# alibaba/VideoMV

Hardware: AMD Instinct MI355X
Metric: denoise-steps/sec, t2v 320x512x24 (latent 24x40x64), CFG 9.0, 50-step DDIM schedule (higher is better)
Workload: dtype fp16; 1 GPU; t2v_infer.yaml UNetSD_T2VBase 1.413B, 24 views, latent 40x64, 77 ctx tokens, 1 sample per GPU (cond+uncond batched); parallelism=replicas x1

## Files before the change

include/vmv.h:

```cpp
#ifndef VMV_H
#define VMV_H
#include <stdint.h>
#include <stddef.h>

#ifdef __cplusplus
extern "C" {
#endif

#define VMV_OK            0
#define VMV_EINVAL       -1
#define VMV_EALIGN       -2
#define VMV_ENULL        -3
#define VMV_ERANGE       -4
#define VMV_ECOMM        -5

#define VMV_ABI_VERSION   12
int vmv_abi_version(void);
#define VMV_ELEM_F16      0
#define VMV_ELEM_BF16     1
int vmv_elem_type(void);
int vmv_has_experiments(void);
int vmv_sizeof(int which);
const char* vmv_error_string(int code);

#define VMV_MAX_SEGS 24
#define VMV_SEG_LINEAR   0
#define VMV_SEG_SPATIAL  1
#define VMV_SEG_TEMPORAL 2

typedef struct {
    const void* src;
    int32_t ld;
    int32_t k;
    int32_t mode;
    int32_t d0, d1;
    int32_t _pad;
} VmvGemmSeg;

#define VMV_EPI_NONE   0
#define VMV_EPI_GEGLU  1
#define VMV_EPI_TATTN  2
#define VMV_ACT_NONE   0
#define VMV_ACT_SILU   1
#define VMV_ACT_GELU   2

typedef struct {
    int32_t M, N;
    int32_t nseg;
    int32_t ktot;
    VmvGemmSeg seg[VMV_MAX_SEGS];
    const void* W;
    const float* bias;
    const float* rowvec;
    int32_t rowvec_div, rowvec_ld;
    const void* residual;
    int32_t ldr;
    int32_t epilogue;
    int32_t act;
    int32_t out_fp32;
    void* out;
    int32_t ldo;
    int32_t OH, OW, IH, IW, stride, ups;
    int32_t F, P;
    int32_t ksplit;
    float* workspace;
    int32_t tile;
    float res_scale;
    const float* rowstat;
    const float* colsum;
    float ln_eps;
    int32_t wgroup_rows;
    int64_t wgroup_stride;
    const float* gn_table;
    int32_t gn_rows_per_stat;
    int32_t gn_silu;
    float epi_scale;
    int32_t phased;
} VmvGemmParams;

#define VMV_TILE_AUTO     0
#define VMV_TILE_128x128  1
#define VMV_TILE_128x160  2
#define VMV_TILE_128x64   3
#define VMV_TILE_64x64    4
#define VMV_TILE_256x128  5
#define VMV_TILE_256x160  6
#define VMV_TILE_G128x128 7
#define VMV_TILE_G128x160 8
#define VMV_TILE_P256x128 9
#define VMV_TILE_P256x160 10
#define VMV_TILE_PP256x128 11
#define VMV_TILE_PP256x160 12
#define VMV_TILE_Q128x128 13
#define VMV_TILE_Q96x160  14
#define VMV_TILE_S256x128 15
#define VMV_TILE_S192x160 16
#define VMV_TILE_S256x160 17
#define VMV_TILE_A128x160 18
#define VMV_TILE_A128x128 19
#define VMV_TILE_X256x320 20
#define VMV_TILE_X256x256 21
#define VMV_TILE_X256x128 22
#define VMV_TILE_RS       23
#define VMV_TILE_RS512    24
#define VMV_TILE_RS256    25
#define VMV_TILE_HALO     26
#define VMV_TILE_TFR      27

#define VMV_TILE_TQA      28
#define VMV_TILE_W256x256 29

#define VMV_TILE_X512x128 30
#define VMV_TILE_Y256x128 31

#define VMV_TILE_TRS      32

int vmv_gemm(const VmvGemmParams* p, void* stream);
int vmv_gemm_tqa_ok(const VmvGemmParams* p);
int vmv_gemm_up4_ok(const VmvGemmParams* p);
int vmv_gemm_ln_inline_ok(const VmvGemmParams* p);
int vmv_gemm_rs_ok(const VmvGemmParams* p);
int vmv_gemm_tfr_ok(const VmvGemmParams* p);
int vmv_gemm_trs_ok(const VmvGemmParams* p);
int vmv_gemm_trs_blocks(const VmvGemmParams* p, int max_blocks, void* stream);
int vmv_gemm_pick_tile(const VmvGemmParams* p);
int vmv_gemm_validate(const VmvGemmParams* p);
int vmv_gemm_served_tile(const VmvGemmParams* p);
int vmv_gemm_tile_map(int bid, int tiles_m, int tiles_n, int gm, int* tile_m, int* tile_n);
int vmv_gemm_group_m(int tiles_m, int tiles_n, int BM, int BN, int conc);

typedef struct {
    int32_t M, C;
    const void* x; int32_t ldx;
    int32_t _pad0;
    const void* w1;
    const float* b1;
    const void* w2;
    const float* b2;
    const void* residual; int32_t ldr;
    float ln_eps;
    void* out; int32_t ldo;
    int32_t _pad1;
} VmvFfParams;
int vmv_ff_fused(const VmvFfParams* p, void* stream);
int vmv_ff_fused_ok(const VmvFfParams* p);

typedef struct {
    const void* x;
    const void* x1;
    int32_t ld, ld1;
    int32_t C0, C1;
    int32_t rows, rows_per_stat;
    int32_t chunk_rows;
    float* partial;
    const float* gamma;
    const float* beta;
    float eps;
    int32_t silu;
    void* y;
    int32_t ldy;
    int32_t fold_ranks;
    int64_t* totals;
    int64_t* totals_clear;
    int32_t clear_count;
    int32_t _pad;
} VmvGroupNormParams;

#define VMV_GN_REC 8
#define VMV_GN_NREP 8
int vmv_groupnorm_stats(const VmvGroupNormParams* p, void* stream);
int vmv_groupnorm_table(const VmvGroupNormParams* p, void* stream);
int vmv_groupnorm_apply(const VmvGroupNormParams* p, void* stream);
#define VMV_GN_FUSED_BYTES 131072
int vmv_groupnorm_fused(const VmvGroupNormParams* p, int32_t cols, void* stream);

typedef struct {
    const void* x; int32_t ldx;
    void* y; int32_t ldy;
    const float* gamma; const float* beta;
    int32_t rows, C;
    float eps;
    int32_t _pad;
    float* stats_out;
} VmvLayerNormParams;
int vmv_layernorm(const VmvLayerNormParams* p, void* stream);

typedef struct {
    const float* s; int32_t lds;
    void* p; int32_t ldp;
    int32_t rows, n;
    float scale;
    int32_t _pad;
} VmvSoftmaxParams;
int vmv_softmax_rows(const VmvSoftmaxParams* p, void* stream);

typedef struct {
    int64_t s_outer, s_inner, s_row;
    int32_t inner; int32_t _pad;
} VmvSeqMap;

typedef struct {
    const void* q; const void* k; const void* v; void* o;
    VmvSeqMap qm, km, vm, om;
    int32_t n_outer;
    int32_t kv_div;
    int32_t heads;
    int32_t Nq, Nk;
    float scale;
    int32_t head_dim;
    int32_t causal;
} VmvAttnParams;
int vmv_attention(const VmvAttnParams* p, void* stream);
#define VMV_ATTN_SHORT    1
#define VMV_ATTN_WAVE     2
#define VMV_ATTN_Q128     3
#define VMV_ATTN_Q256     4
#define VMV_ATTN_CAUSAL   5
#define VMV_ATTN_D32      6
#define VMV_ATTN_D128     7
int vmv_attention_served_kernel(const VmvAttnParams* p);

int vmv_latent_to_rows(const float* x, void* rows, int nb_src, int C, int F, int H, int W, int Cpad, int nrep,
                       void* stream);
int vmv_latent_to_rows_keep(const float* x, void* rows, int nb, int C, int F, int H, int W, int ld, int nrep, void* stream);
int vmv_rows_to_nchw(const void* rows, int rows_fp32, int ld, float* out, int n, int C, int HW, void* stream);

typedef struct {
    const float* eps_rows;
    int32_t ld;
    int32_t C, F, HW;
    float guide_scale;
    float c_recip, c_recipm1;
    float c_sqrt_ac, c_sqrt_1mac;
    float a_prev;
    int32_t v_pred;
    float* xt;
    float* x0_out;
    float clamp;
    float sigma;
    const float* noise;
} VmvDdimParams;
int vmv_cfg_ddim_step(const VmvDdimParams* p, void* stream);

int vmv_posterior_sample(const float* moments_rows, int ld, const float* noise, float* z, int n, int zc, int HW, float scale,
                         void* stream);
int vmv_emb_combine_silu(const float* temb, const float* cam, void* out, int rows, int C, int rows_per_t,
                         int cam_rows, void* stream);
int vmv_sinusoidal(const float* t, void* out_elem, int n, int dim, void* stream);

int vmv_i2v_temporal_adapter(const void* in, int ld_in, void* out, int ld_out, const float* w, int F, int HW, int nrep,
                             float scale, void* stream);
int vmv_adaptive_avgpool_rows(const void* in, int ld, void* out, int ldo, int n, int C, int IH, int IW, int OH, int OW,
                              void* stream);

int vmv_lgm_x0_views(const float* eps_rows, int ld, int branch, const float* xt, int C, int F, int HW, const int32_t* idx4,
                     float c_recip, float c_recipm1, float inv_scale, float* out, void* stream);
int vmv_lgm_pack_input(const float* decoded, const float* rays, float* out, int nviews, int HW, void* stream);
int vmv_lgm_render_to_vae(const float* images, float* out, int nviews, int S_in, int S, void* stream);
int vmv_ddim_x0_step(const float* x0_cond, const float* x0_uncond, float* xt, long n, float guide, float c_recip,
                     float c_recipm1, float a_prev, float clamp, float sigma, const float* noise, void* stream);

int vmv_gaussian_activation(const float* raw, int ld, float* out, int n, float* workspace, void* stream);

typedef struct {
    const float* gaussians;
    int32_t N;
    int32_t size;
    const float* view;
    const float* view_proj;
    float tan_half_fov;
    float bg[3];
    float* depth;
    float* xy;
    float* conic_opacity;
    int32_t* rect;
    uint32_t* tiles_touched;
    uint32_t* offsets;
    void* scan_temp; size_t scan_temp_bytes;
    uint64_t* keys; uint64_t* keys_sorted;
    uint32_t* vals; uint32_t* vals_sorted;
    int32_t num_rendered; int32_t _pad;
    void* sort_temp; size_t sort_temp_bytes;
    uint32_t* ranges;
    float* out_color; float* out_alpha;
} VmvGsParams;
int vmv_gs_workspace_bytes(int n_gaussians, int n_instances, size_t* scan_bytes, size_t* sort_bytes);
int vmv_gs_preprocess(const VmvGsParams* p, void* stream);
int vmv_gs_render(const VmvGsParams* p, void* stream);

typedef struct {
    const float* gaussians;
    int32_t B, N, V, size;
    const float* views;
    const float* view_projs;
    float tan_half_fov;
    float bg[3];
    float* depth;
    float* xy;
    float* conic_opacity;
    int32_t* rect;
    uint32_t* tiles_touched;
    uint32_t* offsets;
    void* scan_temp; size_t scan_temp_bytes;
    uint64_t* keys; uint64_t* keys_sorted;
    uint32_t* vals; uint32_t* vals_sorted;
    int32_t num_rendered; int32_t _pad;
    void* sort_temp; size_t sort_temp_bytes;
    uint32_t* ranges;
    float* out_color;
    float* out_alpha;
} VmvGsBatchParams;
int vmv_gs_batch_key_bits(int n_views, int size);
int vmv_gs_batch_workspace_bytes(int n_view_gaussians, int n_instances, int key_bits, size_t* scan_bytes, size_t* sort_bytes);
int vmv_gs_batch_preprocess(const VmvGsBatchParams* p, void* stream);
int vmv_gs_batch_render(const VmvGsBatchParams* p, void* stream);

typedef struct {
    VmvGsBatchParams pass;
    float* out_depth;
    float* out_median_depth;
} VmvGsDepthParams;
int vmv_gs_batch_render_depth(const VmvGsDepthParams* p, void* stream);

typedef struct {
    VmvGsBatchParams pass;
    float* final_T;
    int32_t* n_contrib;
    const float* dL_dimage;
    float* grad2d;
    float* grad_view;
    float* grad;
} VmvGsBackwardParams;
int vmv_gs_batch_render_state(const VmvGsBackwardParams* p, void* stream);
int vmv_gs_batch_backward(const VmvGsBackwardParams* p, void* stream);
int vmv_gs_image_loss(const float* image, const float* target, long n, float* dL_dimage, float* loss, float* workspace, void* stream);
typedef struct {
    float* params;
    float* m; float* v;
    const float* grad;
    float* gaussians;
    int32_t n; int32_t step;
    float lr[5];
    float beta1, beta2, eps;
} VmvGsAdamParams;
int vmv_gs_adam_step(const VmvGsAdamParams* p, void* stream);

typedef struct {
    const float* image;
    const float* target;
    int32_t planes, height, width;
    float lambda_dssim;
    float* dL_dimage;
    float* loss;
    float* workspace;
    size_t workspace_bytes;
} VmvGsSsimLossParams;
int vmv_gs_ssim_loss_workspace_bytes(int planes, int height, int width, size_t* bytes);
int vmv_gs_ssim_loss(const VmvGsSsimLossParams* p, void* stream);

typedef struct {
    const float* depth;
    const float* colour;
    const float* views;
    int   n_views, size;
    float tan_half_fov;
    int   res;
    float origin[3];
    float voxel, trunc, z_min;
    int   carve;
    float* acc;
    long  plane_stride;
} VmvGsTsdfParams;
int vmv_gs_tsdf_integrate(const VmvGsTsdfParams* p, void* stream);

typedef struct {
    const int64_t* faces;
    int64_t  face_stride;
    int64_t  n_faces;
    int64_t  n_vertices;
    int32_t* label;
    int32_t* face_count;
    int32_t* status;
} VmvGsMeshComponentsParams;
int vmv_gs_mesh_components(const VmvGsMeshComponentsParams* p, void* stream);

typedef struct {
    const float*   verts;
    const float*   vert_colours;
    const int64_t* faces;
    int64_t  face_stride;
    int64_t  n_faces;
    int64_t  n_vertices;
    const float* depth;
    const float* colour;
    const float* views;
    int32_t  n_views, size;
    float    tan_half_fov;
    float    z_min, depth_tol;
    float    cos_min;
    int32_t  patch;
    int32_t  tex_size;
    float*   out;
    int64_t  plane_stride;
    int32_t* status;
} VmvGsMeshBakeParams;
int vmv_gs_mesh_bake(const VmvGsMeshBakeParams* p, void* stream);

typedef struct {
    const void* src;
    void* dst;
    int32_t n0, n1, n2;
    int32_t inner16;
    int64_t ss0, ss1, ss2;
} VmvCopyParams;
int vmv_permute_copy(const VmvCopyParams* p, void* stream);

#define VMV_COMM_ALL_TO_ALL 0
#define VMV_COMM_ALL_GATHER 1
#define VMV_COMM_ID_BYTES   128
typedef struct VmvComm VmvComm;
typedef struct {
    const VmvComm* comm;
    int32_t kind;
    int32_t _pad;
    const void* send;
    void* recv;
    int64_t bytes;
} VmvCommParams;
int      vmv_comm_load(const char* rccl_path);
int      vmv_comm_loaded(void);
int      vmv_comm_unique_id(void* id128);
VmvComm* vmv_comm_create(const void* id128, int world, int rank);
VmvComm* vmv_comm_create_sim(int world, int rank);
void     vmv_comm_destroy(VmvComm* comm);
int      vmv_comm_world(const VmvComm* comm);
int      vmv_comm_rank(const VmvComm* comm);
int      vmv_comm_is_sim(const VmvComm* comm);
int      vmv_comm_run(const VmvCommParams* p, void* stream);

typedef struct VmvPlan VmvPlan;
#define VMV_OP_GEMM        1
#define VMV_OP_GN_STATS    2
#define VMV_OP_GN_APPLY    3
#define VMV_OP_LAYERNORM   4
#define VMV_OP_ATTENTION   5
#define VMV_OP_SOFTMAX     6
#define VMV_OP_COPY        7
#define VMV_OP_GN_FUSED    8
#define VMV_OP_FF          9
#define VMV_OP_GN_TABLE    10
#define VMV_OP_COMM        11
VmvPlan* vmv_plan_create(void);
void     vmv_plan_destroy(VmvPlan* plan);
int      vmv_plan_add(VmvPlan* plan, int op, const void* params, size_t nbytes);
int      vmv_plan_size(const VmvPlan* plan);
int      vmv_plan_run(const VmvPlan* plan, void* stream);
int      vmv_plan_run_range(const VmvPlan* plan, int first, int last, void* stream);
typedef struct VmvGraph VmvGraph;
VmvGraph* vmv_plan_capture(const VmvPlan* plan, void* stream);
int       vmv_graph_launch(const VmvGraph* graph, void* stream);
int       vmv_graph_nodes(const VmvGraph* graph);
void      vmv_graph_destroy(VmvGraph* graph);

#ifdef __cplusplus
}
#endif
#endif
```

videomv_amd/_lib.py:

```python
import ctypes as C
import os

_HERE = os.path.dirname(os.path.abspath(__file__))
_ELEM_NAMES = {"fp16": "f16", "f16": "f16", "float16": "f16", "half": "f16", "bf16": "bf16", "bfloat16": "bf16"}
_elem = _ELEM_NAMES[os.environ.get("VMV_DTYPE", "fp16").lower()]
ELEM_F16, ELEM_BF16 = 0, 1


def set_elem(name: str):
    global _elem
    new = _ELEM_NAMES[str(name).lower()]
    if _lib is not None and new != _elem:
        raise RuntimeError(f"the {_elem} kernels are already loaded; set VMV_DTYPE / call set_elem() before first use")
    _elem = new


def elem_name() -> str:
    return "fp16" if _elem == "f16" else "bf16"


def elem():
    import torch
    return torch.float16 if _elem == "f16" else torch.bfloat16


def lib_path() -> str:
    return os.path.join(os.environ.get("VMV_LIB_DIR") or os.path.join(_HERE, "lib"), f"libvmv_hip_{_elem}.so")

VMV_MAX_SEGS = 24
SEG_LINEAR, SEG_SPATIAL, SEG_TEMPORAL = 0, 1, 2
EPI_NONE, EPI_GEGLU, EPI_TATTN = 0, 1, 2
ACT_NONE, ACT_SILU, ACT_GELU = 0, 1, 2
TILE_AUTO, TILE_128x128, TILE_128x160, TILE_128x64, TILE_64x64, TILE_256x128, TILE_256x160 = 0, 1, 2, 3, 4, 5, 6
TILE_G128x128, TILE_G128x160, TILE_P256x128, TILE_P256x160, TILE_PP256x128, TILE_PP256x160 = 7, 8, 9, 10, 11, 12
TILE_Q128x128, TILE_Q96x160 = 13, 14
TILE_S256x128, TILE_S192x160, TILE_S256x160 = 15, 16, 17
TILE_A128x160, TILE_A128x128 = 18, 19
TILE_X256x320, TILE_X256x256, TILE_X256x128 = 20, 21, 22
TILE_RS, TILE_RS512, TILE_RS256, TILE_HALO, TILE_TFR, TILE_TQA, TILE_W256x256, TILE_X512x128, TILE_Y256x128 = 23, 24, 25, 26, 27, 28, 29, 30, 31
TRS_TILE = 32
OP_GEMM, OP_GN_STATS, OP_GN_APPLY, OP_LAYERNORM, OP_ATTENTION, OP_SOFTMAX, OP_COPY, OP_GN_FUSED, OP_FF, OP_GN_TABLE, OP_COMM = 1, 2, 3, 4, 5, 6, 7, 8, 9, 10, 11
COMM_ALL_TO_ALL, COMM_ALL_GATHER, COMM_ID_BYTES = 0, 1, 128
ABI_VERSION = 12
ATTN_SHORT, ATTN_WAVE, ATTN_Q128, ATTN_Q256, ATTN_CAUSAL, ATTN_D32, ATTN_D128 = 1, 2, 3, 4, 5, 6, 7
GN_FUSED_BYTES = 131072


class GemmSeg(C.Structure):
    _fields_ = [("src", C.c_void_p), ("ld", C.c_int32), ("k", C.c_int32), ("mode", C.c_int32),
                ("d0", C.c_int32), ("d1", C.c_int32), ("_pad", C.c_int32)]


class GemmParams(C.Structure):
    _fields_ = [("M", C.c_int32), ("N", C.c_int32), ("nseg", C.c_int32), ("ktot", C.c_int32),
                ("seg", GemmSeg * VMV_MAX_SEGS),
                ("W", C.c_void_p), ("bias", C.c_void_p), ("rowvec", C.c_void_p),
                ("rowvec_div", C.c_int32), ("rowvec_ld", C.c_int32),
                ("residual", C.c_void_p), ("ldr", C.c_int32),
                ("epilogue", C.c_int32), ("act", C.c_int32), ("out_fp32", C.c_int32),
                ("out", C.c_void_p), ("ldo", C.c_int32),
                ("OH", C.c_int32), ("OW", C.c_int32), ("IH", C.c_int32), ("IW", C.c_int32),
                ("stride", C.c_int32), ("ups", C.c_int32),
                ("F", C.c_int32), ("P", C.c_int32),
                ("ksplit", C.c_int32), ("workspace", C.c_void_p),
                ("tile", C.c_int32), ("res_scale", C.c_float), ("rowstat", C.c_void_p), ("colsum", C.c_void_p),
                ("ln_eps", C.c_float), ("wgroup_rows", C.c_int32), ("wgroup_stride", C.c_int64),
                ("gn_table", C.c_void_p), ("gn_rows_per_stat", C.c_int32), ("gn_silu", C.c_int32), ("epi_scale", C.c_float),
                ("phased", C.c_int32)]


class GroupNormParams(C.Structure):
    _fields_ = [("x", C.c_void_p), ("x1", C.c_void_p), ("ld", C.c_int32), ("ld1", C.c_int32),
                ("C0", C.c_int32), ("C1", C.c_int32), ("rows", C.c_int32), ("rows_per_stat", C.c_int32),
                ("chunk_rows", C.c_int32), ("partial", C.c_void_p), ("gamma", C.c_void_p), ("beta", C.c_void_p),
                ("eps", C.c_float), ("silu", C.c_int32), ("y", C.c_void_p), ("ldy", C.c_int32), ("fold_ranks", C.c_int32),
                ("totals", C.c_void_p), ("totals_clear", C.c_void_p), ("clear_count", C.c_int32), ("_pad", C.c_int32)]


class FfParams(C.Structure):
    _fields_ = [("M", C.c_int32), ("C", C.c_int32), ("x", C.c_void_p), ("ldx", C.c_int32), ("_pad0", C.c_int32),
                ("w1", C.c_void_p), ("b1", C.c_void_p), ("w2", C.c_void_p), ("b2", C.c_void_p),
                ("residual", C.c_void_p), ("ldr", C.c_int32), ("ln_eps", C.c_float),
                ("out", C.c_void_p), ("ldo", C.c_int32), ("_pad1", C.c_int32)]


class GsParams(C.Structure):
    _fields_ = [("gaussians", C.c_void_p), ("N", C.c_int32), ("size", C.c_int32), ("view", C.c_void_p),
                ("view_proj", C.c_void_p), ("tan_half_fov", C.c_float), ("bg", C.c_float * 3),
                ("depth", C.c_void_p), ("xy", C.c_void_p), ("conic_opacity", C.c_void_p), ("rect", C.c_void_p),
                ("tiles_touched", C.c_void_p), ("offsets", C.c_void_p), ("scan_temp", C.c_void_p),
                ("scan_temp_bytes", C.c_size_t), ("keys", C.c_void_p), ("keys_sorted", C.c_void_p), ("vals", C.c_void_p),
                ("vals_sorted", C.c_void_p), ("num_rendered", C.c_int32), ("_pad", C.c_int32), ("sort_temp", C.c_void_p),
                ("sort_temp_bytes", C.c_size_t), ("ranges", C.c_void_p), ("out_color", C.c_void_p), ("out_alpha", C.c_void_p)]


class GsBatchParams(C.Structure):
    _fields_ = [("gaussians", C.c_void_p), ("B", C.c_int32), ("N", C.c_int32), ("V", C.c_int32), ("size", C.c_int32),
                ("views", C.c_void_p), ("view_projs", C.c_void_p), ("tan_half_fov", C.c_float), ("bg", C.c_float * 3),
                ("depth", C.c_void_p), ("xy", C.c_void_p), ("conic_opacity", C.c_void_p), ("rect", C.c_void_p),
                ("tiles_touched", C.c_void_p), ("offsets", C.c_void_p), ("scan_temp", C.c_void_p),
                ("scan_temp_bytes", C.c_size_t), ("keys", C.c_void_p), ("keys_sorted", C.c_void_p), ("vals", C.c_void_p),
                ("vals_sorted", C.c_void_p), ("num_rendered", C.c_int32), ("_pad", C.c_int32), ("sort_temp", C.c_void_p),
                ("sort_temp_bytes", C.c_size_t), ("ranges", C.c_void_p), ("out_color", C.c_void_p), ("out_alpha", C.c_void_p)]


class GsBackwardParams(C.Structure):
    _fields_ = [("pass_", GsBatchParams), ("final_T", C.c_void_p), ("n_contrib", C.c_void_p), ("dL_dimage", C.c_void_p),
                ("grad2d", C.c_void_p), ("grad_view", C.c_void_p), ("grad", C.c_void_p)]


class GsDepthParams(C.Structure):
    _fields_ = [("pass_", GsBatchParams), ("out_depth", C.c_void_p), ("out_median_depth", C.c_void_p)]


class GsAdamParams(C.Structure):
    _fields_ = [("params", C.c_void_p), ("m", C.c_void_p), ("v", C.c_void_p), ("grad", C.c_void_p), ("gaussians", C.c_void_p),
                ("n", C.c_int32), ("step", C.c_int32), ("lr", C.c_float * 5), ("beta1", C.c_float), ("beta2", C.c_float),
                ("eps", C.c_float)]


class GsSsimLossParams(C.Structure):
    _fields_ = [("image", C.c_void_p), ("target", C.c_void_p), ("planes", C.c_int32), ("height", C.c_int32), ("width", C.c_int32),
                ("lambda_dssim", C.c_float), ("dL_dimage", C.c_void_p), ("loss", C.c_void_p), ("workspace", C.c_void_p),
                ("workspace_bytes", C.c_size_t)]


class GsTsdfParams(C.Structure):
    _fields_ = [("depth", C.c_void_p), ("colour", C.c_void_p), ("views", C.c_void_p), ("n_views", C.c_int), ("size", C.c_int),
                ("tan_half_fov", C.c_float), ("res", C.c_int), ("origin", C.c_float * 3), ("voxel", C.c_float), ("trunc", C.c_float),
                ("z_min", C.c_float), ("carve", C.c_int), ("acc", C.c_void_p), ("plane_stride", C.c_long)]


class GsMeshComponentsParams(C.Structure):
    _fields_ = [("faces", C.c_void_p), ("face_stride", C.c_int64), ("n_faces", C.c_int64), ("n_vertices", C.c_int64),
                ("label", C.c_void_p), ("face_count", C.c_void_p), ("status", C.c_void_p)]


class GsMeshBakeParams(C.Structure):
    _fields_ = [("verts", C.c_void_p), ("vert_colours", C.c_void_p), ("faces", C.c_void_p), ("face_stride", C.c_int64),
                ("n_faces", C.c_int64), ("n_vertices", C.c_int64), ("depth", C.c_void_p), ("colour", C.c_void_p), ("views", C.c_void_p),
                ("n_views", C.c_int32), ("size", C.c_int32), ("tan_half_fov", C.c_float), ("z_min", C.c_float), ("depth_tol", C.c_float),
                ("cos_min", C.c_float), ("patch", C.c_int32), ("tex_size", C.c_int32), ("out", C.c_void_p), ("plane_stride", C.c_int64),
                ("status", C.c_void_p)]


MESH_STATUS_RANGE, MESH_STATUS_GAVE_UP = 1, 2


class CopyParams(C.Structure):
    _fields_ = [("src", C.c_void_p), ("dst", C.c_void_p), ("n0", C.c_int32), ("n1", C.c_int32), ("n2", C.c_int32),
                ("inner16", C.c_int32), ("ss0", C.c_int64), ("ss1", C.c_int64), ("ss2", C.c_int64)]


class CommParams(C.Structure):
    _fields_ = [("comm", C.c_void_p), ("kind", C.c_int32), ("_pad", C.c_int32), ("send", C.c_void_p), ("recv", C.c_void_p),
                ("bytes", C.c_int64)]


class LayerNormParams(C.Structure):
    _fields_ = [("x", C.c_void_p), ("ldx", C.c_int32), ("y", C.c_void_p), ("ldy", C.c_int32),
                ("gamma", C.c_void_p), ("beta", C.c_void_p), ("rows", C.c_int32), ("C", C.c_int32),
                ("eps", C.c_float), ("_pad", C.c_int32), ("stats_out", C.c_void_p)]


class SeqMap(C.Structure):
    _fields_ = [("s_outer", C.c_int64), ("s_inner", C.c_int64), ("s_row", C.c_int64),
                ("inner", C.c_int32), ("_pad", C.c_int32)]


class AttnParams(C.Structure):
    _fields_ = [("q", C.c_void_p), ("k", C.c_void_p), ("v", C.c_void_p), ("o", C.c_void_p),
                ("qm", SeqMap), ("km", SeqMap), ("vm", SeqMap), ("om", SeqMap),
                ("n_outer", C.c_int32), ("kv_div", C.c_int32), ("heads", C.c_int32),
                ("Nq", C.c_int32), ("Nk", C.c_int32), ("scale", C.c_float), ("head_dim", C.c_int32), ("causal", C.c_int32)]


class SoftmaxParams(C.Structure):
    _fields_ = [("s", C.c_void_p), ("lds", C.c_int32), ("p", C.c_void_p), ("ldp", C.c_int32),
                ("rows", C.c_int32), ("n", C.c_int32), ("scale", C.c_float), ("_pad", C.c_int32)]


class DdimParams(C.Structure):
    _fields_ = [("eps_rows", C.c_void_p), ("ld", C.c_int32), ("C", C.c_int32), ("F", C.c_int32), ("HW", C.c_int32),
                ("guide_scale", C.c_float), ("c_recip", C.c_float), ("c_recipm1", C.c_float),
                ("c_sqrt_ac", C.c_float), ("c_sqrt_1mac", C.c_float), ("a_prev", C.c_float),
                ("v_pred", C.c_int32), ("xt", C.c_void_p), ("x0_out", C.c_void_p),
                ("clamp", C.c_float), ("sigma", C.c_float), ("noise", C.c_void_p)]


_P = C.c_void_p
SYMBOLS = {
    "vmv_abi_version": (C.c_int, []),
    "vmv_elem_type": (C.c_int, []),
    "vmv_sizeof": (C.c_int, [C.c_int]),
    "vmv_error_string": (C.c_char_p, [C.c_int]),
    "vmv_gemm": (C.c_int, [C.POINTER(GemmParams), _P]),
    "vmv_gemm_ln_inline_ok": (C.c_int, [C.POINTER(GemmParams)]),
    "vmv_gemm_rs_ok": (C.c_int, [C.POINTER(GemmParams)]),
    "vmv_gemm_tfr_ok": (C.c_int, [C.POINTER(GemmParams)]),
    "vmv_gemm_tqa_ok": (C.c_int, [C.POINTER(GemmParams)]),
    "vmv_gemm_trs_ok": (C.c_int, [C.POINTER(GemmParams)]),
    "vmv_gemm_trs_blocks": (C.c_int, [C.POINTER(GemmParams), C.c_int, _P]),
    "vmv_gemm_up4_ok": (C.c_int, [C.POINTER(GemmParams)]),
    "vmv_has_experiments": (C.c_int, []),
    "vmv_ff_fused": (C.c_int, [C.POINTER(FfParams), _P]),
    "vmv_ff_fused_ok": (C.c_int, [C.POINTER(FfParams)]),
    "vmv_gemm_pick_tile": (C.c_int, [C.POINTER(GemmParams)]),
    "vmv_gemm_validate": (C.c_int, [C.POINTER(GemmParams)]),
    "vmv_gemm_served_tile": (C.c_int, [C.POINTER(GemmParams)]),
    "vmv_gemm_tile_map": (C.c_int, [C.c_int, C.c_int, C.c_int, C.c_int, C.POINTER(C.c_int), C.POINTER(C.c_int)]),
    "vmv_gemm_group_m": (C.c_int, [C.c_int, C.c_int, C.c_int, C.c_int, C.c_int]),
    "vmv_groupnorm_stats": (C.c_int, [C.POINTER(GroupNormParams), _P]),
    "vmv_groupnorm_apply": (C.c_int, [C.POINTER(GroupNormParams), _P]),
    "vmv_groupnorm_table": (C.c_int, [C.POINTER(GroupNormParams), _P]),
    "vmv_groupnorm_fused": (C.c_int, [C.POINTER(GroupNormParams), C.c_int32, _P]),
    "vmv_layernorm": (C.c_int, [C.POINTER(LayerNormParams), _P]),
    "vmv_attention": (C.c_int, [C.POINTER(AttnParams), _P]),
    "vmv_attention_served_kernel": (C.c_int, [C.POINTER(AttnParams)]),
    "vmv_softmax_rows": (C.c_int, [C.POINTER(SoftmaxParams), _P]),
    "vmv_permute_copy": (C.c_int, [C.POINTER(CopyParams), _P]),
    "vmv_gaussian_activation": (C.c_int, [_P, C.c_int, _P, C.c_int, _P, _P]),
    "vmv_lgm_x0_views": (C.c_int, [_P, C.c_int, C.c_int, _P, C.c_int, C.c_int, C.c_int, _P, C.c_float, C.c_float, C.c_float, _P, _P]),
    "vmv_lgm_pack_input": (C.c_int, [_P, _P, _P, C.c_int, C.c_int, _P]),
    "vmv_lgm_render_to_vae": (C.c_int, [_P, _P, C.c_int, C.c_int, C.c_int, _P]),
    "vmv_ddim_x0_step": (C.c_int, [_P, _P, _P, C.c_long, C.c_float, C.c_float, C.c_float, C.c_float, C.c_float, C.c_float, _P, _P]),
    "vmv_gs_workspace_bytes": (C.c_int, [C.c_int, C.c_int, C.POINTER(C.c_size_t), C.POINTER(C.c_size_t)]),
    "vmv_gs_preprocess": (C.c_int, [C.POINTER(GsParams), _P]),
    "vmv_gs_render": (C.c_int, [C.POINTER(GsParams), _P]),
    "vmv_gs_batch_key_bits": (C.c_int, [C.c_int, C.c_int]),
    "vmv_gs_batch_workspace_bytes": (C.c_int, [C.c_int, C.c_int, C.c_int, C.POINTER(C.c_size_t), C.POINTER(C.c_size_t)]),
    "vmv_gs_batch_preprocess": (C.c_int, [C.POINTER(GsBatchParams), _P]),
    "vmv_gs_batch_render": (C.c_int, [C.POINTER(GsBatchParams), _P]),
    "vmv_gs_batch_render_depth": (C.c_int, [C.POINTER(GsDepthParams), _P]),
    "vmv_gs_batch_render_state": (C.c_int, [C.POINTER(GsBackwardParams), _P]),
    "vmv_gs_batch_backward": (C.c_int, [C.POINTER(GsBackwardParams), _P]),
    "vmv_gs_image_loss": (C.c_int, [_P, _P, C.c_long, _P, _P, _P, _P]),
    "vmv_gs_adam_step": (C.c_int, [C.POINTER(GsAdamParams), _P]),
    "vmv_gs_ssim_loss_workspace_bytes": (C.c_int, [C.c_int, C.c_int, C.c_int, C.POINTER(C.c_size_t)]),
    "vmv_gs_ssim_loss": (C.c_int, [C.POINTER(GsSsimLossParams), _P]),
    "vmv_gs_tsdf_integrate": (C.c_int, [C.POINTER(GsTsdfParams), _P]),
    "vmv_gs_mesh_components": (C.c_int, [C.POINTER(GsMeshComponentsParams), _P]),
    "vmv_gs_mesh_bake": (C.c_int, [C.POINTER(GsMeshBakeParams), _P]),
    "vmv_latent_to_rows": (C.c_int, [_P, _P, C.c_int, C.c_int, C.c_int, C.c_int, C.c_int, C.c_int, C.c_int, _P]),
    "vmv_latent_to_rows_keep": (C.c_int, [_P, _P, C.c_int, C.c_int, C.c_int, C.c_int, C.c_int, C.c_int, C.c_int, _P]),
    "vmv_i2v_temporal_adapter": (C.c_int, [_P, C.c_int, _P, C.c_int, _P, C.c_int, C.c_int, C.c_int, C.c_float, _P]),
    "vmv_adaptive_avgpool_rows": (C.c_int, [_P, C.c_int, _P, C.c_int, C.c_int, C.c_int, C.c_int, C.c_int, C.c_int, C.c_int, _P]),
    "vmv_rows_to_nchw": (C.c_int, [_P, C.c_int, C.c_int, _P, C.c_int, C.c_int, C.c_int, _P]),
    "vmv_cfg_ddim_step": (C.c_int, [C.POINTER(DdimParams), _P]),
    "vmv_posterior_sample": (C.c_int, [_P, C.c_int, _P, _P, C.c_int, C.c_int, C.c_int, C.c_float, _P]),
    "vmv_emb_combine_silu": (C.c_int, [_P, _P, _P, C.c_int, C.c_int, C.c_int, C.c_int, _P]),
    "vmv_sinusoidal": (C.c_int, [_P, _P, C.c_int, C.c_int, _P]),
    "vmv_plan_create": (_P, []),
    "vmv_plan_destroy": (None, [_P]),
    "vmv_plan_add": (C.c_int, [_P, C.c_int, _P, C.c_size_t]),
    "vmv_plan_size": (C.c_int, [_P]),
    "vmv_plan_run": (C.c_int, [_P, _P]),
    "vmv_plan_run_range": (C.c_int, [_P, C.c_int, C.c_int, _P]),
    "vmv_plan_capture": (_P, [_P, _P]),
    "vmv_graph_launch": (C.c_int, [_P, _P]),
    "vmv_graph_nodes": (C.c_int, [_P]),
    "vmv_graph_destroy": (None, [_P]),
    "vmv_comm_load": (C.c_int, [C.c_char_p]),
    "vmv_comm_loaded": (C.c_int, []),
    "vmv_comm_unique_id": (C.c_int, [_P]),
    "vmv_comm_create": (_P, [_P, C.c_int, C.c_int]),
    "vmv_comm_create_sim": (_P, [C.c_int, C.c_int]),
    "vmv_comm_destroy": (None, [_P]),
    "vmv_comm_world": (C.c_int, [_P]),
    "vmv_comm_rank": (C.c_int, [_P]),
    "vmv_comm_is_sim": (C.c_int, [_P]),
    "vmv_comm_run": (C.c_int, [C.POINTER(CommParams), _P]),
}

_lib = None


def load():
    global _lib
    if _lib is not None:
        return _lib
    LIB_PATH = lib_path()
    if not os.path.exists(LIB_PATH):
        raise RuntimeError(
            f"{LIB_PATH} is missing: build the HIP extension first (python -c 'import __graft_entry__ as g; "
            f"g.build()' or make -C videomv_amd/csrc).  There is no CPU fallback for the hot path.")
    lib = C.CDLL(LIB_PATH)
    for name, (res, args) in SYMBOLS.items():
        fn = getattr(lib, name)
        fn.restype = res
        fn.argtypes = args
    if lib.vmv_abi_version() != ABI_VERSION:
        raise RuntimeError(f"{LIB_PATH}: ABI version mismatch")
    if lib.vmv_elem_type() != (ELEM_F16 if _elem == "f16" else ELEM_BF16):
        raise RuntimeError(f"{LIB_PATH} was built for another element type")
    for which, st in ((OP_GEMM, GemmParams), (OP_GN_STATS, GroupNormParams), (OP_LAYERNORM, LayerNormParams),
                      (OP_ATTENTION, AttnParams), (OP_SOFTMAX, SoftmaxParams), (OP_COPY, CopyParams), (OP_FF, FfParams), (OP_COMM, CommParams), (103, GsParams), (104, GsBatchParams), (105, GsBackwardParams), (106, GsAdamParams), (107, GsSsimLossParams), (108, GsDepthParams), (109, GsTsdfParams), (110, GsMeshComponentsParams), (111, GsMeshBakeParams), (100, DdimParams), (101, GemmSeg), (102, SeqMap)):
        if lib.vmv_sizeof(which) != C.sizeof(st):
            raise RuntimeError(f"struct layout drift for {st.__name__}: C {lib.vmv_sizeof(which)} vs ctypes "
                               f"{C.sizeof(st)}")
    _lib = lib
    return lib


class VmvError(RuntimeError):
    pass


def check(rc, what=""):
    if rc != 0:
        msg = load().vmv_error_string(rc)
        raise VmvError(f"{what}: rc={rc} ({msg.decode() if msg else '?'})")
```

videomv_amd/csrc/gemm.hip:

```cpp
#include "gemm_common.h"

using namespace vmvg;

int vmv_gemm_glds_launch(const VmvGemmParams& p, int total_steps, int tile, hipStream_t st);
int vmv_gemm_pglds_launch(const VmvGemmParams& p, int total_steps, int tile, hipStream_t st);
bool vmv_gemm_pglds_supported(const VmvGemmParams& p);
int vmv_gemm_xglds_launch(const VmvGemmParams& p, int total_steps, int tile, hipStream_t st);
int vmv_gemm_xglds_epi_ok(const VmvGemmParams& p, int tile);
int vmv_gemm_rs_launch(const VmvGemmParams& p, int tile, hipStream_t st);
bool vmv_gemm_rs_supported(const VmvGemmParams& p);
int vmv_conv_halo_launch(const VmvGemmParams& p, hipStream_t st);
bool vmv_conv_halo_supported(const VmvGemmParams& p);
bool vmv_gemm_rs_preferred(const VmvGemmParams& p);
int vmv_gemm_tfr_launch(const VmvGemmParams& p, hipStream_t st);
bool vmv_gemm_tfr_supported(const VmvGemmParams& p);
bool vmv_gemm_tfr_preferred(const VmvGemmParams& p);
int vmv_gemm_tqa_launch(const VmvGemmParams& p, hipStream_t st);
bool vmv_gemm_tqa_supported(const VmvGemmParams& p);
bool vmv_gemm_tqa_preferred(const VmvGemmParams& p);
int vmv_gemm_trs_launch(const VmvGemmParams& p, int max_blocks, hipStream_t st);
bool vmv_gemm_trs_supported(const VmvGemmParams& p);
bool vmv_gemm_trs_preferred(const VmvGemmParams& p);
namespace {

template <int WM, int WN>
struct GemmCfg {
    static constexpr int BM = 32 * WM;
    static constexpr int BN = 32 * WN;
    static constexpr int LDS_BYTES = 2 * (BM + BN) * BK * 2;
};

template <int WM, int WN>
__global__ __launch_bounds__(256) void gemm_kernel(const VmvGemmParams p, const int tiles_m, const int tiles_n,
                                                   const int total_steps, const int steps_per_split) {
    VMV_KERNEL_ENTER();
    using Cfg = GemmCfg<WM, WN>;
    constexpr int BM = Cfg::BM, BN = Cfg::BN;
    extern __shared__ __attribute__((aligned(16))) unsigned char smem_raw[];
    u32x4_t* const lds = reinterpret_cast<u32x4_t*>(smem_raw);
    constexpr int A_U = BM * 8, W_U = BN * 8;

    const int tid = threadIdx.x;
    const int lane = tid & 63;
    const int wave = tid >> 6;
    const int wave_m = wave >> 1, wave_n = wave & 1;

    int tile_m, tile_n;
    tile_of_block(blockIdx.x, tiles_m, tiles_n, 1, tile_m, tile_n);
    const int m0 = tile_m * BM, n0 = tile_n * BN;
    const int split = blockIdx.y;
    const int step_begin = split * steps_per_split;
    const int step_end = min(total_steps, step_begin + steps_per_split);

    const int srow = tid >> 3, sslot = tid & 7;
    const int sw_slot = sslot ^ ((srow >> 1) & 7);

    RowInfo rinfo[WM];
#pragma unroll
    for (int i = 0; i < WM; ++i) {
        const int m = m0 + srow + 32 * i;
        RowInfo r;
        r.m = (m < p.M) ? m : -1;
        r.nb = 0; r.oy = 0; r.ox = 0; r.fr = 0;
        if (p.OH > 0) {
            const int hw = p.OH * p.OW;
            const int n = m / hw, rem = m - n * hw;
            r.nb = n * p.IH * p.IW;
            r.oy = rem / p.OW;
            r.ox = rem - r.oy * p.OW;
        }
        if (p.P > 0) r.fr = (m / p.P) % p.F;
        rinfo[i] = r;
    }
    const uint16_t* wrow[WN];
    bool wvalid[WN];
#pragma unroll
    for (int j = 0; j < WN; ++j) {
        const int n = n0 + srow + 32 * j;
        wvalid[j] = n < p.N;
        wrow[j] = reinterpret_cast<const uint16_t*>(p.W) + (size_t)(wvalid[j] ? n : 0) * p.ktot + sslot * 8 +
                  (p.wgroup_rows > 0 ? (long)(m0 / p.wgroup_rows) * p.wgroup_stride : 0L);
    }

    int s = 0, kc = 0, koff = 0;
    {
        int skip = step_begin;
        while (s < p.nseg) {
            const int nch = (p.seg[s].k + BK - 1) / BK;
            if (skip < nch) { kc = skip * BK; break; }
            skip -= nch; koff += p.seg[s].k; ++s;
        }
    }
    int aoff[WM];
    auto enter_segment = [&]() {
#pragma unroll
        for (int i = 0; i < WM; ++i) aoff[i] = seg_row_offset(p, p.seg[s], rinfo[i]);
    };
    if (s < p.nseg) enter_segment();

    u32x4_t ra[WM], rw[WN];
    auto load_chunk = [&]() {
        const VmvGemmSeg& sg = p.seg[s];
        const int kk = kc + sslot * 8;
        const bool kvalid = kk < sg.k;
        const uint16_t* src = reinterpret_cast<const uint16_t*>(sg.src) + kk;
#pragma unroll
        for (int i = 0; i < WM; ++i) {
            u32x4_t v = {0u, 0u, 0u, 0u};
            if (kvalid && aoff[i] >= 0) v = *reinterpret_cast<const u32x4_t*>(src + aoff[i]);
            ra[i] = v;
        }
#pragma unroll
        for (int j = 0; j < WN; ++j) {
            u32x4_t v = {0u, 0u, 0u, 0u};
            if (kvalid && wvalid[j]) v = *reinterpret_cast<const u32x4_t*>(wrow[j] + koff + kc);
            rw[j] = v;
        }
    };
    auto advance = [&]() {
        kc += BK;
        if (kc >= p.seg[s].k) {
            koff += p.seg[s].k; ++s; kc = 0;
            if (s < p.nseg) enter_segment();
        }
    };
    auto store_chunk = [&](int buf) {
        u32x4_t* a = lds + buf * A_U;
        u32x4_t* w = lds + 2 * A_U + buf * W_U;
#pragma unroll
        for (int i = 0; i < WM; ++i) a[(srow + 32 * i) * 8 + sw_slot] = ra[i];
#pragma unroll
        for (int j = 0; j < WN; ++j) w[(srow + 32 * j) * 8 + sw_slot] = rw[j];
    };

    f32x4_t acc[WN][WM];
#pragma unroll
    for (int j = 0; j < WN; ++j)
#pragma unroll
        for (int i = 0; i < WM; ++i) acc[j][i] = f32x4_t{0.f, 0.f, 0.f, 0.f};

    const int frow = lane & 15;
    const int fgrp = lane >> 4;
    const int fswz = (frow >> 1) & 7;

    const int nsteps = step_end - step_begin;
    if (nsteps > 0) {
        load_chunk();
        advance();
        store_chunk(0);
    }
    __syncthreads();
    int cur = 0;
    for (int t = 0; t < nsteps; ++t) {
        const bool more = (t + 1) < nsteps;
        if (more) { load_chunk(); advance(); }
        const u32x4_t* a = lds + cur * A_U + (wave_m * 16 * WM + frow) * 8;
        const u32x4_t* w = lds + 2 * A_U + cur * W_U + (wave_n * 16 * WN + frow) * 8;
#pragma unroll
        for (int kk = 0; kk < 2; ++kk) {
            const int slot = (kk * 4 + fgrp) ^ fswz;
            elem8_t af[WM], wf[WN];
#pragma unroll
            for (int i = 0; i < WM; ++i) af[i] = __builtin_bit_cast(elem8_t, a[i * 16 * 8 + slot]);
#pragma unroll
            for (int j = 0; j < WN; ++j) wf[j] = __builtin_bit_cast(elem8_t, w[j * 16 * 8 + slot]);
#pragma unroll
            for (int j = 0; j < WN; ++j)
#pragma unroll
                for (int i = 0; i < WM; ++i)
                    acc[j][i] = VMV_MFMA16(wf[j], af[i], acc[j][i], 0, 0, 0);
        }
        if (more) store_chunk(cur ^ 1);
        __syncthreads();
        cur ^= 1;
    }

    const int mbase = m0 + wave_m * 16 * WM + frow;
    const int nbase = n0 + wave_n * 16 * WN + 4 * fgrp;
    if (p.ksplit > 1) {
        float* ws = p.workspace + (size_t)split * p.M * p.N;
#pragma unroll
        for (int j = 0; j < WN; ++j)
#pragma unroll
            for (int i = 0; i < WM; ++i) {
                const int m = mbase + 16 * i, n = nbase + 16 * j;
                if (m < p.M && n < p.N) *reinterpret_cast<f32x4_t*>(ws + (size_t)m * p.N + n) = acc[j][i];
            }
        return;
    }
    if (p.epilogue == VMV_EPI_GEGLU) {
        if constexpr ((WN & 1) == 0) {
#pragma unroll
            for (int j = 0; j < WN; j += 2)
#pragma unroll
                for (int i = 0; i < WM; ++i) epilogue_store(p, mbase + 16 * i, nbase + 16 * j, acc[j][i], acc[j + 1][i]);
        }
    } else {
#pragma unroll
        for (int j = 0; j < WN; ++j)
#pragma unroll
            for (int i = 0; i < WM; ++i) epilogue_store(p, mbase + 16 * i, nbase + 16 * j, acc[j][i], acc[j][i]);
    }
}

__global__ __launch_bounds__(256) void gemm_splitk_reduce(const VmvGemmParams p) {
    VMV_KERNEL_ENTER();
    const int geglu = p.epilogue == VMV_EPI_GEGLU;
    const int nq = geglu ? (p.N / 32) * 4 : p.N / 4;
    const long total = (long)p.M * nq;
    for (long idx = (long)blockIdx.x * blockDim.x + threadIdx.x; idx < total; idx += (long)gridDim.x * blockDim.x) {
        const int m = (int)(idx / nq);
        const int qi = (int)(idx - (long)m * nq);
        const int n = geglu ? (qi >> 2) * 32 + (qi & 3) * 4 : qi * 4;
        f32x4_t v = {0.f, 0.f, 0.f, 0.f}, g = {0.f, 0.f, 0.f, 0.f};
        for (int s = 0; s < p.ksplit; ++s) {
            const float* ws = p.workspace + ((size_t)s * p.M + m) * p.N + n;
            v += *reinterpret_cast<const f32x4_t*>(ws);
            if (geglu) g += *reinterpret_cast<const f32x4_t*>(ws + 16);
        }
        epilogue_store(p, m, n, v, g);
    }
}

template <int WM, int WN>
int launch_cfg(const VmvGemmParams& p, int total_steps, hipStream_t st) {
    using Cfg = GemmCfg<WM, WN>;
    const int tiles_m = (p.M + Cfg::BM - 1) / Cfg::BM;
    const int tiles_n = (p.N + Cfg::BN - 1) / Cfg::BN;
    const int ks = p.ksplit > 1 ? p.ksplit : 1;
    const int sps = (total_steps + ks - 1) / ks;
    static std::atomic<unsigned long long> attr_set{0};
    if (const int rc_attr = vmv_lds_attr_once(attr_set, reinterpret_cast<const void*>(&gemm_kernel<WM, WN>), Cfg::LDS_BYTES)) return rc_attr;
    dim3 grid(tiles_m * tiles_n, ks, 1);
    VMV_LAUNCH((gemm_kernel<WM, WN>), grid, dim3(256), Cfg::LDS_BYTES, st, p, tiles_m, tiles_n, total_steps, sps);
    return vmv_launch_status();
}

int pick_tile(const VmvGemmParams& p, int total_steps) {
    if (p.epilogue == VMV_EPI_TATTN) return VMV_TILE_TQA;
    if (p.tile != VMV_TILE_AUTO) return p.tile;
    const int geglu = p.epilogue == VMV_EPI_GEGLU;
    if (vmv_gemm_rs_preferred(p)) return VMV_TILE_RS;
    if (vmv_conv_halo_supported(p)) return VMV_TILE_HALO;
    if (vmv_gemm_tfr_preferred(p)) return VMV_TILE_TFR;
    if (vmv_gemm_trs_preferred(p)) return VMV_TILE_TRS;
    if (p.gn_table && p.nseg == 3 && p.seg[0].mode == VMV_SEG_TEMPORAL) return VMV_TILE_TFR;
    if (p.gn_table) return VMV_TILE_RS;
    if (!geglu && p.ksplit <= 1 && !p.rowstat && !vmv_gemm_ln_inline(p) && total_steps >= 12 && (p.N % 320 == 0 || p.N % 256 == 0)) {
        bool any_gather = false;
        for (int i = 0; i < p.nseg; ++i) any_gather = any_gather || p.seg[i].mode != VMV_SEG_LINEAR;
        const int bx = p.N % 320 == 0 ? 320 : 256;
        const long tm = (p.M + 255) / 256;
        const long rounds_x = (tm * (p.N / bx) + 255) / 256, rounds_g = (tm * (p.N / (bx / 2)) + 255) / 256;
        if ((any_gather || total_steps >= 32) && 20 * rounds_x <= 11 * rounds_g) return bx == 320 ? VMV_TILE_X256x320 : VMV_TILE_X256x256;
    }
    if (!geglu && p.ksplit <= 1 && !p.rowstat && !vmv_gemm_ln_inline(p) && p.N == 128 && total_steps >= 12 && p.wgroup_rows == 0 &&
        !p.out_fp32 && (long)p.M >= 2L * 256 * 512) {
        bool any_gather = false;
        for (int i = 0; i < p.nseg; ++i) any_gather = any_gather || p.seg[i].mode != VMV_SEG_LINEAR;
        if (any_gather) return VMV_TILE_X512x128;
    }
    if ((geglu || p.rowstat) && p.ksplit <= 1 && !vmv_gemm_ln_inline(p) && total_steps >= 20 && p.N % 256 == 0 && p.wgroup_rows == 0 &&
        !p.out_fp32 && !p.rowvec && vmv_gemm_xglds_epi_ok(p, VMV_TILE_X256x256)) {
        bool lin = true;
        for (int i = 0; i < p.nseg; ++i) lin = lin && p.seg[i].mode == VMV_SEG_LINEAR;
        const long tiles = (long)((p.M + 255) / 256) * (p.N / 256);
        const long rounds = (tiles + 255) / 256;
        if (lin && tiles >= 400 && (double)tiles / (double)(rounds * 256) >= 0.85) return VMV_TILE_X256x256;
    }
    auto padded = [&](int bn) { return ((p.N + bn - 1) / bn) * bn; };
    int best = VMV_TILE_128x128, best_pad = padded(128);
    if (!geglu && padded(160) <= best_pad) { best = VMV_TILE_128x160; best_pad = padded(160); }
    if (padded(64) < best_pad) { best = VMV_TILE_128x64; best_pad = padded(64); }
    if (p.M <= 64 && best == VMV_TILE_128x64) best = VMV_TILE_64x64;
    if (p.ksplit > 1 && p.M > 64 && (best == VMV_TILE_128x128 || best == VMV_TILE_128x160)) {
        const int bn = best == VMV_TILE_128x128 ? 128 : 160;
        best = best == VMV_TILE_128x128 ? VMV_TILE_G128x128 : VMV_TILE_G128x160;
        const long blocks256 = (long)((p.M + 255) / 256) * ((p.N + bn - 1) / bn) * p.ksplit;
        if (p.M >= 1024 && blocks256 >= 192 && blocks256 <= 272)
            best = bn == 128 ? VMV_TILE_256x128 : VMV_TILE_256x160;
    }
    if (p.ksplit <= 1 && (best == VMV_TILE_128x128 || best == VMV_TILE_128x160)) {
        const int bn = best == VMV_TILE_128x128 ? 128 : 160;
        const long tiles = (long)((p.M + 255) / 256) * ((p.N + bn - 1) / bn);
        const long waves = (tiles + 255) / 256;
        const bool big = tiles >= 240 && (double)tiles / (double)(waves * 256) >= 0.8;
        bool linear = true;
        for (int i = 0; i < p.nseg; ++i) linear = linear && p.seg[i].mode == VMV_SEG_LINEAR;
        const bool p160 = best == VMV_TILE_128x160;
        const long ptiles = (long)((p.M + (p160 ? 191 : 255)) / (p160 ? 192 : 256)) * ((p.N + bn - 1) / bn);
        if (linear && total_steps <= 24 && ptiles >= 2 * 256)
            best = p160 ? VMV_TILE_P256x160 : VMV_TILE_P256x128;
        else if (big)
            best = best == VMV_TILE_128x128 ? VMV_TILE_256x128 : VMV_TILE_256x160;
        else if (p.M > 64)
            best = best == VMV_TILE_128x128 ? VMV_TILE_G128x128 : VMV_TILE_G128x160;
    }
    return best;
}

bool retired_tile(int t) {
    return t == VMV_TILE_S256x128 || t == VMV_TILE_S192x160 || t == VMV_TILE_S256x160 || t == VMV_TILE_A128x160 || t == VMV_TILE_A128x128 ||
           t == VMV_TILE_W256x256 || t == VMV_TILE_Y256x128;
}

int final_tile(const VmvGemmParams& p, int total_steps) {
    int picked = pick_tile(p, total_steps);
    if (retired_tile(picked)) return VMV_EINVAL;
    if (p.phased) {
        const bool x = picked == VMV_TILE_X256x320 || picked == VMV_TILE_X256x256 || picked == VMV_TILE_X256x128;
        if (x) return picked;
        if (p.tile != VMV_TILE_AUTO) return VMV_EINVAL;
        const long tm = 4L * ((p.M / 4 + 255) / 256);
        if (p.N % 320 == 0 && tm * (p.N / 320) >= 256) return VMV_TILE_X256x320;
        if (p.N % 256 == 0 && tm * (p.N / 256) >= 256) return VMV_TILE_X256x256;
        return VMV_TILE_X256x128;
    }
    if (picked == VMV_TILE_HALO) return vmv_conv_halo_supported(p) ? picked : VMV_EINVAL;
    if (picked == VMV_TILE_TFR) return vmv_gemm_tfr_supported(p) ? picked : VMV_EINVAL;
    if (picked == VMV_TILE_TRS) return vmv_gemm_trs_supported(p) ? picked : VMV_EINVAL;
    if (picked == VMV_TILE_TQA) return vmv_gemm_tqa_supported(p) && (p.tile == VMV_TILE_AUTO || p.tile == VMV_TILE_TQA) ? picked : VMV_EINVAL;
    const bool rs_tile = picked == VMV_TILE_RS || picked == VMV_TILE_RS512 || picked == VMV_TILE_RS256;
    if (rs_tile) return vmv_gemm_rs_supported(p) ? picked : VMV_EINVAL;
    if (p.gn_table) return VMV_EINVAL;
    if (vmv_gemm_ln_inline(p) && p.tile == VMV_TILE_AUTO)
        picked = vmv_gemm_rs_supported(p) ? VMV_TILE_RS
                                          : (p.epilogue != VMV_EPI_GEGLU && p.N % 160 == 0) ? VMV_TILE_P256x160 : VMV_TILE_P256x128;
    if (picked == VMV_TILE_RS) return picked;
    if (p.wgroup_rows > 0) {
        const bool ok = picked == VMV_TILE_128x128 || picked == VMV_TILE_128x64 || picked == VMV_TILE_64x64 || picked == VMV_TILE_256x128 ||
                        picked == VMV_TILE_G128x128 || picked == VMV_TILE_P256x128;
        if (p.tile != VMV_TILE_AUTO) {
            if (!ok) return VMV_EINVAL;
        } else if (picked == VMV_TILE_P256x160 || picked == VMV_TILE_X256x320 || picked == VMV_TILE_X256x256 || picked == VMV_TILE_X512x128) picked = VMV_TILE_P256x128;
        else if (picked == VMV_TILE_256x160) picked = VMV_TILE_256x128;
        else if (!ok) picked = VMV_TILE_G128x128;
    }
    if (p.rowstat && !(picked == VMV_TILE_X256x256 && vmv_gemm_xglds_epi_ok(p, picked)) && picked != VMV_TILE_P256x128 && picked != VMV_TILE_P256x160 &&
        picked != VMV_TILE_Q128x128 && picked != VMV_TILE_Q96x160 && picked != VMV_TILE_128x128 && picked != VMV_TILE_128x160 &&
        picked != VMV_TILE_128x64 && picked != VMV_TILE_64x64)
        picked = (p.epilogue != VMV_EPI_GEGLU && p.N % 160 == 0) ? VMV_TILE_P256x160 : VMV_TILE_P256x128;
    return picked;
}

bool up4_valid(const VmvGemmParams& p) {
    if (p.phased != 1 || p.ups != 1 || p.stride != 1 || p.out_fp32 || p.nseg != 4 || p.ksplit > 1) return false;
    if (p.residual || p.rowvec || p.rowstat || p.colsum || p.gn_table || p.gn_silu || p.wgroup_rows != 0 || p.epilogue != VMV_EPI_NONE) return false;
    static const int taps[4][2] = {{-1, -1}, {-1, 0}, {0, -1}, {0, 0}};
    for (int s = 0; s < 4; ++s) {
        const VmvGemmSeg& sg = p.seg[s];
        if (sg.mode != VMV_SEG_SPATIAL || sg.src != p.seg[0].src || sg.ld != p.seg[0].ld || sg.k != p.seg[0].k) return false;
        if (sg.d0 != taps[s][0] || sg.d1 != taps[s][1]) return false;
    }
    if (p.ktot != 4 * p.seg[0].k || p.OH != 2 * p.IH || p.OW != 2 * p.IW) return false;
    const long hw = (long)p.IH * p.IW;
    if ((p.M & 3) || (p.M / 4) % hw != 0) return false;
    return true;
}

bool ln_inline_ok(const VmvGemmParams& p) {
    if (!p.W || !p.out || !p.colsum || p.nseg != 1 || p.seg[0].mode != VMV_SEG_LINEAR || p.seg[0].k != p.ktot) return false;
    if (p.ksplit > 1 || p.out_fp32 || p.rowvec || p.residual) return false;
    if (p.epilogue == VMV_EPI_TATTN) return (p.tile == VMV_TILE_AUTO || p.tile == VMV_TILE_TQA) && vmv_gemm_tqa_supported(p);
    const bool rs_forced = p.tile == VMV_TILE_RS || p.tile == VMV_TILE_RS512 || p.tile == VMV_TILE_RS256;
    if (p.tile != VMV_TILE_AUTO && p.tile != VMV_TILE_P256x128 && p.tile != VMV_TILE_P256x160 && !rs_forced) return false;
    const int n_out = p.epilogue == VMV_EPI_GEGLU ? p.N / 2 : p.N;
    if ((p.ldo & 7) || (n_out & 7) || !vmv_aligned16(p.out)) return false;
    if (rs_forced) return vmv_gemm_rs_supported(p);
    return vmv_gemm_rs_supported(p) || vmv_gemm_pglds_supported(p);
}

}

extern "C" int vmv_has_experiments(void) { return 0; }

extern "C" int vmv_gemm_ln_inline_ok(const VmvGemmParams* pp) { return pp && ln_inline_ok(*pp) ? 1 : 0; }

extern "C" int vmv_gemm_rs_ok(const VmvGemmParams* pp) {
    if (!pp || pp->tile != VMV_TILE_AUTO || pp->nseg <= 0 || pp->nseg > VMV_MAX_SEGS) return 0;
    return vmv_gemm_rs_preferred(*pp) ? 1 : 0;
}

extern "C" int vmv_gemm_tfr_ok(const VmvGemmParams* pp) {
    if (!pp || pp->tile != VMV_TILE_AUTO || pp->nseg <= 0 || pp->nseg > VMV_MAX_SEGS) return 0;
    return vmv_gemm_tfr_preferred(*pp) ? 1 : 0;
}

extern "C" int vmv_gemm_trs_ok(const VmvGemmParams* pp) {
    if (!pp || pp->tile != VMV_TILE_AUTO || pp->nseg <= 0 || pp->nseg > VMV_MAX_SEGS) return 0;
    return vmv_gemm_trs_preferred(*pp) && vmv_gemm_validate(pp) == VMV_OK ? 1 : 0;
}

extern "C" int vmv_gemm_tqa_ok(const VmvGemmParams* pp) {
    if (!pp || pp->tile != VMV_TILE_AUTO || pp->nseg <= 0 || pp->nseg > VMV_MAX_SEGS) return 0;
    return vmv_gemm_tqa_preferred(*pp) ? 1 : 0;
}

extern "C" int vmv_gemm_up4_ok(const VmvGemmParams* pp) {
    if (!pp || pp->tile != VMV_TILE_AUTO || !pp->phased) return 0;
    const char* e = getenv("VMV_UP4_MIN_ROWS");
    const long min_rows = e ? atol(e) : 769;
    if (pp->M / 4 < min_rows) return 0;
    return vmv_gemm_validate(pp) == VMV_OK ? 1 : 0;
}

extern "C" int vmv_gemm_pick_tile(const VmvGemmParams* pp) {
    if (!pp || pp->nseg <= 0 || pp->nseg > VMV_MAX_SEGS) return VMV_EINVAL;
    int total_steps = 0;
    for (int s = 0; s < pp->nseg; ++s) total_steps += (pp->seg[s].k + BK - 1) / BK;
    return final_tile(*pp, total_steps);
}

thread_local int vmv_dry_run = 0;
extern "C" int vmv_gemm_validate(const VmvGemmParams* pp) {
    vmv_dry_run = 1;
    const int rc = vmv_gemm(pp, nullptr);
    vmv_dry_run = 0;
    return rc;
}

static thread_local int vmv_served_note = 0;
static inline int served(int rc, int tile) {
    if (vmv_dry_run && rc != VMV_GLDS_UNSUPPORTED) vmv_served_note = tile;
    return rc;
}
extern "C" int vmv_gemm_served_tile(const VmvGemmParams* pp) {
    vmv_served_note = 0;
    const int rc = vmv_gemm_validate(pp);
    if (rc != VMV_OK) return rc < 0 ? rc : VMV_EINVAL;
    return vmv_served_note > 0 ? vmv_served_note : VMV_EINVAL;
}

extern "C" int vmv_gemm_trs_blocks(const VmvGemmParams* pp, int max_blocks, void* stream) {
    if (!pp || pp->tile != VMV_TILE_TRS || max_blocks < 1) return VMV_EINVAL;
    if (const int rc = vmv_gemm_validate(pp)) return rc;
    const int rc = vmv_gemm_trs_launch(*pp, max_blocks, reinterpret_cast<hipStream_t>(stream));
    return rc == VMV_GLDS_UNSUPPORTED ? VMV_EINVAL : rc;
}

extern "C" int vmv_gemm_tile_map(int bid, int tiles_m, int tiles_n, int gm, int* tile_m, int* tile_n) {
    if (!tile_m || !tile_n) return VMV_ENULL;
    if (tiles_m <= 0 || tiles_n <= 0 || gm < 1 || bid < 0 || (long)bid >= (long)tiles_m * tiles_n) return VMV_EINVAL;
    tile_of_block(bid, tiles_m, tiles_n, gm, *tile_m, *tile_n);
    return VMV_OK;
}
extern "C" int vmv_gemm_group_m(int tiles_m, int tiles_n, int BM, int BN, int conc) { return gemm_group_m(tiles_m, tiles_n, BM, BN, conc); }

extern "C" int vmv_gemm(const VmvGemmParams* pp, void* stream) {
    if (!pp) return VMV_ENULL;
    const VmvGemmParams& p = *pp;
    if (!p.W || !p.out) return VMV_ENULL;
    if (p.M <= 0 || p.N <= 0 || (p.N & 3) || p.nseg <= 0 || p.nseg > VMV_MAX_SEGS) return VMV_EINVAL;
    if (!vmv_aligned16(p.W) || !vmv_aligned16(p.out) || (p.ktot & 7)) return VMV_EALIGN;
    if (p.bias && !vmv_aligned16(p.bias)) return VMV_EALIGN;
    if (p.ldo & 3) return VMV_EALIGN;
    int ksum = 0, total_steps = 0, maxld = p.ldo;
    for (int s = 0; s < p.nseg; ++s) {
        const VmvGemmSeg& sg = p.seg[s];
        if (!sg.src) return VMV_ENULL;
        if (!vmv_aligned16(sg.src) || (sg.ld & 7) || (sg.k & 7) || sg.k <= 0) return VMV_EALIGN;
        if (sg.mode == VMV_SEG_SPATIAL && (p.OH <= 0 || p.OW <= 0 || p.IH <= 0 || p.IW <= 0 || p.stride <= 0)) return VMV_EINVAL;
        if (sg.mode == VMV_SEG_TEMPORAL && (p.F <= 0 || p.P <= 0)) return VMV_EINVAL;
        if (sg.mode < 0 || sg.mode > 2) return VMV_EINVAL;
        ksum += sg.k;
        if (sg.ld > maxld) maxld = sg.ld;
        total_steps += (sg.k + BK - 1) / BK;
    }
    if (ksum != p.ktot) return VMV_EINVAL;
    if (p.epilogue == VMV_EPI_GEGLU && (p.N & 31)) return VMV_EINVAL;
    if (p.epilogue < VMV_EPI_NONE || p.epilogue > VMV_EPI_TATTN) return VMV_EINVAL;
    if (p.epilogue == VMV_EPI_TATTN && !vmv_gemm_tqa_supported(p)) return VMV_EINVAL;
    if (p.rowvec && (p.rowvec_div <= 0 || (p.rowvec_ld & 3) || !vmv_aligned16(p.rowvec))) return VMV_EINVAL;
    if (p.residual && ((p.ldr & 3) || (((uintptr_t)p.residual) & 7))) return VMV_EALIGN;
    if (p.ksplit > 1 && (!p.workspace || !vmv_aligned16(p.workspace))) return VMV_ENULL;
    if ((long)p.M * (long)maxld >= (1L << 31) || (long)p.N * (long)p.ktot >= (1L << 31)) return VMV_ERANGE;
    if (p.phased) {
        if (!up4_valid(p)) return VMV_EINVAL;
        if (4L * p.N * (long)p.ktot >= (1L << 31)) return VMV_ERANGE;
    }
    hipStream_t st = reinterpret_cast<hipStream_t>(stream);
    int rc;
    if (p.rowstat) {
        if (!p.colsum) return VMV_ENULL;
        if ((((uintptr_t)p.rowstat) & 7) || !vmv_aligned16(p.colsum)) return VMV_EALIGN;
        if (p.ksplit > 1) return VMV_EINVAL;
        for (int s = 0; s < p.nseg; ++s) if (p.seg[s].mode != VMV_SEG_LINEAR) return VMV_EINVAL;
    }
    if (p.wgroup_rows != 0) {
        if (p.wgroup_rows < 0 || (p.wgroup_rows & 255) || p.wgroup_stride < 0 || (p.wgroup_stride & 7) || p.ksplit > 1) return VMV_EINVAL;
        const long groups = ((long)p.M + p.wgroup_rows - 1) / p.wgroup_rows;
        if (!vmv_span32(1, (groups - 1) * p.wgroup_stride + (long)p.N * p.ktot)) return VMV_ERANGE;
    }
    if (p.gn_table && !vmv_gemm_rs_supported(p) && !vmv_gemm_tfr_supported(p) && !vmv_gemm_trs_supported(p)) return VMV_EINVAL;
    if (p.gn_silu && !(p.gn_table && (vmv_gemm_tfr_supported(p) || vmv_gemm_trs_supported(p)))) return VMV_EINVAL;
    const bool ln_inline = vmv_gemm_ln_inline(p);
    if (ln_inline) {
        if (!ln_inline_ok(p)) return VMV_EINVAL;
        if (!vmv_aligned16(p.colsum)) return VMV_EALIGN;
    }
    const int picked = final_tile(p, total_steps);
    if (picked < 0) return picked;
    switch (picked) {
        case VMV_TILE_128x128: rc = served(launch_cfg<4, 4>(p, total_steps, st), VMV_TILE_128x128); break;
        case VMV_TILE_128x160:
            if (p.epilogue == VMV_EPI_GEGLU) return VMV_EINVAL;
            rc = served(launch_cfg<4, 5>(p, total_steps, st), VMV_TILE_128x160); break;
        case VMV_TILE_128x64: rc = served(launch_cfg<4, 2>(p, total_steps, st), VMV_TILE_128x64); break;
        case VMV_TILE_64x64: rc = served(launch_cfg<2, 2>(p, total_steps, st), VMV_TILE_64x64); break;
        case VMV_TILE_256x128:
            rc = served(vmv_gemm_glds_launch(p, total_steps, VMV_TILE_256x128, st), VMV_TILE_256x128);
            if (rc == VMV_GLDS_UNSUPPORTED) rc = served(launch_cfg<4, 4>(p, total_steps, st), VMV_TILE_128x128);
            break;
        case VMV_TILE_256x160:
            rc = served(vmv_gemm_glds_launch(p, total_steps, VMV_TILE_256x160, st), VMV_TILE_256x160);
            if (rc == VMV_GLDS_UNSUPPORTED) rc = served(launch_cfg<4, 5>(p, total_steps, st), VMV_TILE_128x160);
            break;
        case VMV_TILE_X256x320:
        case VMV_TILE_X256x256:
        case VMV_TILE_X256x128:
        case VMV_TILE_X512x128:
            rc = served(vmv_gemm_xglds_launch(p, total_steps, picked, st), picked);
            if (rc == VMV_GLDS_UNSUPPORTED && p.phased) return VMV_EINVAL;
            if (rc == VMV_GLDS_UNSUPPORTED && (p.rowstat || p.epilogue == VMV_EPI_GEGLU)) {
                if (p.tile != VMV_TILE_AUTO) return VMV_EINVAL;
                rc = served(vmv_gemm_pglds_launch(p, total_steps, VMV_TILE_P256x128, st), VMV_TILE_P256x128);
                if (rc == VMV_GLDS_UNSUPPORTED) rc = served(launch_cfg<4, 4>(p, total_steps, st), VMV_TILE_128x128);
                break;
            }
            if (rc == VMV_GLDS_UNSUPPORTED) {
                if (p.tile != VMV_TILE_AUTO) return VMV_EINVAL;
                rc = served(vmv_gemm_glds_launch(p, total_steps, p.N % 160 == 0 ? VMV_TILE_256x160 : VMV_TILE_256x128, st), p.N % 160 == 0 ? VMV_TILE_256x160 : VMV_TILE_256x128);
                if (rc == VMV_GLDS_UNSUPPORTED) rc = p.N % 160 == 0 ? served(launch_cfg<4, 5>(p, total_steps, st), VMV_TILE_128x160) : served(launch_cfg<4, 4>(p, total_steps, st), VMV_TILE_128x128);
            }
            break;
        case VMV_TILE_TFR:
            rc = served(vmv_gemm_tfr_launch(p, st), VMV_TILE_TFR);
            if (rc == VMV_GLDS_UNSUPPORTED) return VMV_EINVAL;
            break;
        case VMV_TILE_TRS:
            rc = served(vmv_gemm_trs_launch(p, 0, st), VMV_TILE_TRS);
            if (rc == VMV_GLDS_UNSUPPORTED) return VMV_EINVAL;
            break;
        case VMV_TILE_TQA:
            rc = served(vmv_gemm_tqa_launch(p, st), VMV_TILE_TQA);
            if (rc == VMV_GLDS_UNSUPPORTED) return VMV_EINVAL;
            break;
        case VMV_TILE_HALO:
            rc = served(vmv_conv_halo_launch(p, st), VMV_TILE_HALO);
            if (rc == VMV_GLDS_UNSUPPORTED) return VMV_EINVAL;
            break;
        case VMV_TILE_RS:
        case VMV_TILE_RS512:
        case VMV_TILE_RS256:
            rc = served(vmv_gemm_rs_launch(p, picked, st), picked);
            if (rc == VMV_GLDS_UNSUPPORTED) return VMV_EINVAL;
            break;
        case VMV_TILE_Q128x128:
            rc = served(vmv_gemm_pglds_launch(p, total_steps, VMV_TILE_Q128x128, st), VMV_TILE_Q128x128);
            if (rc == VMV_GLDS_UNSUPPORTED && !p.rowstat) rc = served(vmv_gemm_glds_launch(p, total_steps, VMV_TILE_256x128, st), VMV_TILE_256x128);
            if (rc == VMV_GLDS_UNSUPPORTED) rc = served(launch_cfg<4, 4>(p, total_steps, st), VMV_TILE_128x128);
            break;
        case VMV_TILE_Q96x160:
            rc = served(vmv_gemm_pglds_launch(p, total_steps, VMV_TILE_Q96x160, st), VMV_TILE_Q96x160);
            if (rc == VMV_GLDS_UNSUPPORTED && !p.rowstat) rc = served(vmv_gemm_glds_launch(p, total_steps, VMV_TILE_256x160, st), VMV_TILE_256x160);
            if (rc == VMV_GLDS_UNSUPPORTED) rc = served(launch_cfg<4, 5>(p, total_steps, st), VMV_TILE_128x160);
            break;
        case VMV_TILE_P256x128:
            rc = served(vmv_gemm_pglds_launch(p, total_steps, VMV_TILE_P256x128, st), VMV_TILE_P256x128);
            if (rc == VMV_GLDS_UNSUPPORTED && ln_inline) return VMV_EINVAL;
            if (rc == VMV_GLDS_UNSUPPORTED && !p.rowstat) rc = served(vmv_gemm_glds_launch(p, total_steps, VMV_TILE_256x128, st), VMV_TILE_256x128);
            if (rc == VMV_GLDS_UNSUPPORTED) rc = served(launch_cfg<4, 4>(p, total_steps, st), VMV_TILE_128x128);
            break;
        case VMV_TILE_P256x160:
            rc = served(vmv_gemm_pglds_launch(p, total_steps, VMV_TILE_P256x160, st), VMV_TILE_P256x160);
            if (rc == VMV_GLDS_UNSUPPORTED && ln_inline) return VMV_EINVAL;
            if (rc == VMV_GLDS_UNSUPPORTED && !p.rowstat) rc = served(vmv_gemm_glds_launch(p, total_steps, VMV_TILE_256x160, st), VMV_TILE_256x160);
            if (rc == VMV_GLDS_UNSUPPORTED) rc = served(launch_cfg<4, 5>(p, total_steps, st), VMV_TILE_128x160);
            break;
        case VMV_TILE_PP256x128:
            rc = served(vmv_gemm_glds_launch(p, total_steps, VMV_TILE_PP256x128, st), VMV_TILE_PP256x128);
            if (rc == VMV_GLDS_UNSUPPORTED) rc = served(launch_cfg<4, 4>(p, total_steps, st), VMV_TILE_128x128);
            break;
        case VMV_TILE_PP256x160:
            rc = served(vmv_gemm_glds_launch(p, total_steps, VMV_TILE_PP256x160, st), VMV_TILE_PP256x160);
            if (rc == VMV_GLDS_UNSUPPORTED) rc = served(launch_cfg<4, 5>(p, total_steps, st), VMV_TILE_128x160);
            break;
        case VMV_TILE_G128x128:
            rc = served(vmv_gemm_glds_launch(p, total_steps, VMV_TILE_G128x128, st), VMV_TILE_G128x128);
            if (rc == VMV_GLDS_UNSUPPORTED) rc = served(launch_cfg<4, 4>(p, total_steps, st), VMV_TILE_128x128);
            break;
        case VMV_TILE_G128x160:
            rc = served(vmv_gemm_glds_launch(p, total_steps, VMV_TILE_G128x160, st), VMV_TILE_G128x160);
            if (rc == VMV_GLDS_UNSUPPORTED) rc = served(launch_cfg<4, 5>(p, total_steps, st), VMV_TILE_128x160);
            break;
        default: return VMV_EINVAL;
    }
    if (rc != VMV_OK) return rc;
    if (p.ksplit > 1) {
        const long items = (long)p.M * (p.N / 4);
        int blocks = (int)((items + 255) / 256);
        if (blocks > 4096) blocks = 4096;
        VMV_LAUNCH(gemm_splitk_reduce, dim3(blocks), dim3(256), 0, st, p);
        rc = vmv_launch_status();
    }
    return rc;
}
```

videomv_amd/csrc/gemm_rs.hip:

```cpp
#include "gemm_rs_common.h"
#include <type_traits>

using namespace vmvg;

namespace {

template <int RT, int KS>
struct RsCfg : RsRing<KS> {
    using Ring = RsRing<KS>;
    static constexpr int BM = Ring::NW * RT * 16;
    static constexpr int MAX_COLS = 5120;
    static constexpr int TAB_BYTES = 2 * 2 * Ring::K * 4;
    static constexpr int LDS_BYTES = Ring::STAGES * Ring::CHUNK_BYTES + MAX_COLS * 4 + TAB_BYTES;
    static_assert(LDS_BYTES <= 160 * 1024, "LDS budget");
};

constexpr int RS_GEGLU = 1, RS_LN = 2, RS_RES = 4, RS_GN = 8;

template <int RT, int KS, int MODE>
__global__ __launch_bounds__(512, 1) void gemm_rs_kernel(const VmvGemmParams p, const int tiles_m, const int nsplit, const int cols_per_split) {
    VMV_KERNEL_ENTER();
    using Cfg = RsCfg<RT, KS>;
    constexpr bool GEGLU = (MODE & RS_GEGLU) != 0, LN = (MODE & RS_LN) != 0, RES = (MODE & RS_RES) != 0, GN = (MODE & RS_GN) != 0;
    constexpr int RB = Cfg::RB, G = Cfg::G, P = Cfg::PIECES;
    extern __shared__ __attribute__((aligned(16))) unsigned char smem[];

    const int tid = threadIdx.x;
    const int lane = tid & 63;
    const int wave = __builtin_amdgcn_readfirstlane(tid >> 6);
    const int frow = lane & 15, fgrp = lane >> 4;

    const int nblk = tiles_m * nsplit;
    const int logical = xcd_logical(blockIdx.x, nblk);
    const int mt = logical / nsplit, ns = logical - mt * nsplit;
    const int m_wave = mt * Cfg::BM + wave * (16 * RT);
    const int n_begin = ns * cols_per_split;
    const int ncols = (p.N - n_begin) < cols_per_split ? (p.N - n_begin) : cols_per_split;
    const int NC = ncols / Cfg::CROWS;

    const VmvGemmSeg& sg = p.seg[0];
    const __amdgpu_buffer_rsrc_t a_rsrc = __builtin_amdgcn_make_buffer_rsrc(const_cast<void*>(sg.src), 0, (uint32_t)p.M * (uint32_t)sg.ld * 2u, SRD_FLAGS);
    u32x4_t a[RT][KS];
#pragma unroll
    for (int i = 0; i < RT; ++i) {
        const uint32_t vo = (uint32_t)((m_wave + 16 * i + frow) * sg.ld + 8 * fgrp) * 2u;
#pragma unroll
        for (int kk = 0; kk < KS; ++kk) a[i][kk] = __builtin_amdgcn_raw_buffer_load_b128(a_rsrc, vo + (uint32_t)(kk * 64), 0, 0);
    }

    float* bias_lds = reinterpret_cast<float*>(smem + Cfg::STAGES * Cfg::CHUNK_BYTES);
    {
        const __amdgpu_buffer_rsrc_t b_rsrc = __builtin_amdgcn_make_buffer_rsrc(const_cast<float*>(p.bias), 0, p.bias ? (uint32_t)p.N * 4u : 0u, SRD_FLAGS);
        for (int q = wave; q * 256 < ncols; q += Cfg::NW)
            blds16(b_rsrc, reinterpret_cast<unsigned char*>(bias_lds) + q * 1024, (uint32_t)(n_begin + q * 256 + 4 * lane) * 4u, 0);
    }
    float* tab_lds = bias_lds + Cfg::MAX_COLS;
    int gn_first = 0;
    if constexpr (GN) {
        gn_first = (mt * Cfg::BM) / p.gn_rows_per_stat;
        const uint32_t nstat = (uint32_t)((p.M + p.gn_rows_per_stat - 1) / p.gn_rows_per_stat);
        const __amdgpu_buffer_rsrc_t t_rsrc = __builtin_amdgcn_make_buffer_rsrc(const_cast<float*>(p.gn_table), 0, nstat * (uint32_t)(2 * Cfg::K * 4), SRD_FLAGS);
        for (int q = wave; q * 1024 < Cfg::TAB_BYTES; q += Cfg::NW)
            blds16(t_rsrc, reinterpret_cast<unsigned char*>(tab_lds) + q * 1024, (uint32_t)(gn_first * 2 * Cfg::K * 4 + q * 1024 + 16 * lane), 0);
    }
    const __amdgpu_buffer_rsrc_t w_rsrc = __builtin_amdgcn_make_buffer_rsrc(const_cast<void*>(p.W), 0, (uint32_t)p.N * (uint32_t)p.ktot * 2u, SRD_FLAGS);
    auto issue_chunk = [&](int c, int slot) {
        unsigned char* base = Cfg::wave_base(smem + slot * Cfg::CHUNK_BYTES, wave);
        const uint32_t so = (uint32_t)((n_begin + c * Cfg::CROWS) * p.ktot) * 2u;
        rs_issue_rows<Cfg>(w_rsrc, base, wave, lane, so, [&](const int r) { return r * p.ktot; });
    };
    const int pro = NC < Cfg::STAGES ? NC : Cfg::STAGES;
    for (int c = 0; c < pro; ++c) issue_chunk(c, c);

    if constexpr (GN) {
        wait_vmcnt_rt(pro * P);
        __syncthreads();
        const float* tbase[RT];
#pragma unroll
        for (int i = 0; i < RT; ++i) {
            const int l = __builtin_amdgcn_readfirstlane((m_wave + 16 * i) / p.gn_rows_per_stat - gn_first);
            tbase[i] = tab_lds + (l ? 2 * Cfg::K : 0) + 8 * fgrp;
        }
        constexpr int GPF = 1, GNB = GPF + 1;
        f32x4_t tv[GNB][4];
        int chain = 0;
        auto rd = [&](int idx, f32x4_t (&t)[4]) {
            const float* tb = tbase[idx / KS] + (idx % KS) * 32 + chain;
            t[0] = *reinterpret_cast<const f32x4_t*>(tb); t[1] = *reinterpret_cast<const f32x4_t*>(tb + 4);
            t[2] = *reinterpret_cast<const f32x4_t*>(tb + Cfg::K); t[3] = *reinterpret_cast<const f32x4_t*>(tb + Cfg::K + 4);
        };
#pragma unroll
        for (int idx = 0; idx < GPF; ++idx) rd(idx, tv[idx % GNB]);
#pragma unroll
        for (int idx = 0; idx < RT * KS; ++idx) {
            if (idx + GPF < RT * KS) rd(idx + GPF, tv[(idx + GPF) % GNB]);
            __builtin_amdgcn_sched_barrier(0);
            const f32x4_t sc0 = tv[idx % GNB][0], sc1 = tv[idx % GNB][1], sh0 = tv[idx % GNB][2], sh1 = tv[idx % GNB][3];
            u32x4_t v = a[idx / KS][idx % KS];
            v.x = pack_elem2(fmaf(elem_lo(v.x), sc0.x, sh0.x), fmaf(elem_hi(v.x), sc0.y, sh0.y));
            v.y = pack_elem2(fmaf(elem_lo(v.y), sc0.z, sh0.z), fmaf(elem_hi(v.y), sc0.w, sh0.w));
            v.z = pack_elem2(fmaf(elem_lo(v.z), sc1.x, sh1.x), fmaf(elem_hi(v.z), sc1.y, sh1.y));
            v.w = pack_elem2(fmaf(elem_lo(v.w), sc1.z, sh1.z), fmaf(elem_hi(v.w), sc1.w, sh1.w));
            a[idx / KS][idx % KS] = v;
            asm volatile("" : "+v"(chain) : "v"(v.x), "v"(v.y), "v"(v.z), "v"(v.w));
            __builtin_amdgcn_sched_barrier(0);
        }
    }

    if constexpr (LN) rs_layernorm_rows(a, p.ln_eps);

    const int lanecol = (fgrp & 1) * 16 + (fgrp >> 1) * 8;
    const __amdgpu_buffer_rsrc_t out_rsrc = __builtin_amdgcn_make_buffer_rsrc(p.out, 0, SRD_RECORDS, SRD_FLAGS);
    const __amdgpu_buffer_rsrc_t res_rsrc = __builtin_amdgcn_make_buffer_rsrc(const_cast<void*>(p.residual), 0, SRD_RECORDS, SRD_FLAGS);
    const uint32_t ovo = (uint32_t)(frow * p.ldo + lanecol) * 2u;
    const uint32_t ovo_g = (uint32_t)((frow + 16 * (fgrp & 1)) * p.ldo + (fgrp >> 1) * 8) * 2u;
    const uint32_t rvo = (uint32_t)(frow * p.ldr + lanecol) * 2u;
    const float rs = p.res_scale != 0.f ? p.res_scale : 1.f;
    auto row_ok = [&](int i) { return m_wave + 16 * i + frow < p.M; };

    if (pro >= 3) wait_vmcnt_rt(2 * P); else if (pro == 2) wait_vmcnt_rt(P); else wait_vmcnt_rt(0);
    __builtin_amdgcn_s_barrier();
    asm volatile("" ::: "memory");

    const int fsw = KS == 10 ? ((frow >> 1) & 7) : frow;
    constexpr int NB = KS == 10 ? 2 : 4;
    int foff[Cfg::NB];
#pragma unroll
    for (int r = 0; r < NB; ++r) foff[r] = frow * RB + (fgrp ^ (fsw & 3)) * 16 + ((r ^ (fsw >> 2)) - r) * 64;
    constexpr int PFD = (RES && RT == 4) ? 0 : 1;
    auto mma_pair = [&](const unsigned char* sbase, const int q, f32x4_t (&c0)[RT], f32x4_t (&c1)[RT]) {
        rs_mma_pair<false, PFD, Cfg>(a, sbase, q, foff, c0, c1);
    };
    auto load_res = [&](const int ocol, u32x4_t (&rv)[RT]) {
#pragma unroll
        for (int i = 0; i < RT; ++i)
            rv[i] = __builtin_amdgcn_raw_buffer_load_b128(res_rsrc, row_ok(i) ? rvo : OOB, (uint32_t)((m_wave + 16 * i) * p.ldr + ocol) * 2u, 0);
    };
    auto store_pair = [&](const int ocol, const int i, u32x4_t o) {
        rs_store16(rs_swap16(o), out_rsrc, row_ok(i) ? ovo : OOB, (uint32_t)((m_wave + 16 * i) * p.ldo + ocol) * 2u);
    };

    const int nbody = ncols / 64;
    int c = 0, slot = 0;
    auto chunk_end = [&](const int stores) { rs_ring_step<Cfg>(c, slot, NC, stores, issue_chunk); };
    for (int b = 0; b < nbody; ++b) {
#pragma unroll
        for (int h = 0; h < 2; ++h) {
            const unsigned char* sbase = smem + slot * Cfg::CHUNK_BYTES;
            const int q = G == 4 ? h : 0;
            const int nrel = 64 * b + 32 * h;
            const int ocol = GEGLU ? (n_begin + nrel) / 2 : n_begin + nrel;
            f32x4_t c0[RT], c1[RT];
            u32x4_t rv[RT];
            if constexpr (RES) load_res(ocol, rv);
            mma_pair(sbase, q, c0, c1);
            const bool cend = G == 2 || h == 1;
            constexpr int SP = GEGLU ? RT / 2 : RT;
            const f32x4_t b0 = *reinterpret_cast<const f32x4_t*>(bias_lds + nrel + 4 * fgrp);
            const f32x4_t b1 = *reinterpret_cast<const f32x4_t*>(bias_lds + nrel + 16 + 4 * fgrp);
            if constexpr (GEGLU) {
                u32x2_t hp[RT];
#pragma unroll
                for (int i = 0; i < RT; ++i) {
                    f32x4_t v = c0[i] + b0;
                    const f32x4_t gt = c1[i] + b1;
                    v.x *= gelu_erf_f(gt.x); v.y *= gelu_erf_f(gt.y); v.z *= gelu_erf_f(gt.z); v.w *= gelu_erf_f(gt.w);
                    hp[i].x = pack_elem2(v.x, v.y); hp[i].y = pack_elem2(v.z, v.w);
                    if (i & 1) {
                        const u32x4_t o = rs_swap16(u32x4_t{hp[i - 1].x, hp[i - 1].y, hp[i].x, hp[i].y});
                        const bool ok = m_wave + 16 * (i - 1 + (fgrp & 1)) + frow < p.M;
                        rs_store16(o, out_rsrc, ok ? ovo_g : OOB, (uint32_t)((m_wave + 16 * (i - 1)) * p.ldo + ocol) * 2u);
                    }
                    __builtin_amdgcn_sched_barrier(0);
                }
            } else {
#pragma unroll
                for (int i = 0; i < RT; ++i) {
                    f32x4_t v0 = c0[i] + b0, v1 = c1[i] + b1;
                    if constexpr (RES) {
                        const u32x4_t r = rs_swap16(rv[i]);
                        v0.x += rs * elem_lo(r.x); v0.y += rs * elem_hi(r.x); v0.z += rs * elem_lo(r.y); v0.w += rs * elem_hi(r.y);
                        v1.x += rs * elem_lo(r.z); v1.y += rs * elem_hi(r.z); v1.z += rs * elem_lo(r.w); v1.w += rs * elem_hi(r.w);
                    }
                    u32x4_t o;
                    o.x = pack_elem2(v0.x, v0.y); o.y = pack_elem2(v0.z, v0.w);
                    o.z = pack_elem2(v1.x, v1.y); o.w = pack_elem2(v1.z, v1.w);
                    store_pair(ocol, i, o);
                }
            }
            if (cend) chunk_end(c == 0 ? SP * (G / 2) : 2 * SP * (G / 2));
        }
    }
}

struct RsPlan { int rt, nsplit, cols; };

bool rs_plan(const VmvGemmParams& p, int force_rt, RsPlan& best, int ncu) {
    const int K = p.ktot;
    bool found = false;
    double best_cost = 0;
    for (int rt = 4; rt >= 2; rt -= 2) {
        if (force_rt && rt != force_rt) continue;
        if ((K == 640 || K == 512) && rt != 2) continue;
        const int bm = 128 * rt;
        const long tm = (p.M + bm - 1) / bm;
        for (int ns = 1; ns <= 8; ns *= 2) {
            if (p.N % (64 * ns)) continue;
            const int cols = p.N / ns;
            if (cols > 5120) continue;
            const long blocks = tm * ns;
            const long rounds = (blocks + ncu - 1) / ncu;
            const double cost = (double)rounds * ((double)bm * cols + 24.0 * bm * K / 32.0);
            if (!found || cost < best_cost * 0.999) { found = true; best_cost = cost; best = RsPlan{rt, ns, cols}; }
        }
    }
    return found;
}

template <int RT, int KS, int MODE>
int launch_rs(const VmvGemmParams& p, const RsPlan& pl, hipStream_t st) {
    using Cfg = RsCfg<RT, KS>;
    const int tiles_m = (p.M + Cfg::BM - 1) / Cfg::BM;
    static std::atomic<unsigned long long> attr{0};
    if (const int rc_attr = vmv_lds_attr_once(attr, reinterpret_cast<const void*>(&gemm_rs_kernel<RT, KS, MODE>), Cfg::LDS_BYTES)) return rc_attr;
    VMV_LAUNCH((gemm_rs_kernel<RT, KS, MODE>), dim3(tiles_m * pl.nsplit), dim3(Cfg::NT), Cfg::LDS_BYTES, st, p, tiles_m, pl.nsplit, pl.cols);
    return vmv_launch_status();
}

template <int RT, int KS>
int launch_rs_mode(const VmvGemmParams& p, const RsPlan& pl, int mode, hipStream_t st) {
    switch (mode) {
        case 0: return launch_rs<RT, KS, 0>(p, pl, st);
        case RS_GEGLU: return launch_rs<RT, KS, RS_GEGLU>(p, pl, st);
        case RS_LN: return launch_rs<RT, KS, RS_LN>(p, pl, st);
        case RS_LN | RS_GEGLU: return launch_rs<RT, KS, RS_LN | RS_GEGLU>(p, pl, st);
        case RS_RES: return launch_rs<RT, KS, RS_RES>(p, pl, st);
        case RS_GN: return launch_rs<RT, KS, RS_GN>(p, pl, st);
        default: return VMV_GLDS_UNSUPPORTED;
    }
}

}

bool vmv_gemm_rs_supported(const VmvGemmParams& p) {
    if (p.nseg != 1 || p.seg[0].mode != VMV_SEG_LINEAR || p.seg[0].k != p.ktot) return false;
    if (p.ktot != 320 && p.ktot != 640 && p.ktot != 512) return false;
    if (p.ksplit > 1 || p.out_fp32 || p.rowvec || p.act != VMV_ACT_NONE || p.wgroup_rows != 0) return false;
    if (p.N % 64) return false;
    const bool geglu = p.epilogue == VMV_EPI_GEGLU;
    const bool ln = p.colsum != nullptr;
    if (ln && !(p.ln_eps > 0.f)) return false;
    if (ln && p.residual) return false;
    if (geglu && p.residual) return false;
    if (p.gn_table) {
        if (ln || geglu || p.residual) return false;
        if (p.gn_rows_per_stat < 512 || (p.gn_rows_per_stat & 15) || (((uintptr_t)p.gn_table) & 15)) return false;
    }
    const int n_out = geglu ? p.N / 2 : p.N;
    if ((p.ldo & 7) || (n_out & 7) || !vmv_aligned16(p.out)) return false;
    if (p.residual && ((p.ldr & 7) || !vmv_aligned16(p.residual))) return false;
    if (!vmv_gemm_spans32(p, p.M + 512, 0, p.M + 512, p.M + 512)) return false;
    RsPlan pl;
    return rs_plan(p, 0, pl, 256);
}

bool vmv_gemm_rs_preferred(const VmvGemmParams& p) {
    if (!vmv_gemm_rs_supported(p)) return false;
    RsPlan pl;
    if (!rs_plan(p, 0, pl, 256)) return false;
    const long blocks = (long)((p.M + 128 * pl.rt - 1) / (128 * pl.rt)) * pl.nsplit;
    return blocks >= 160;
}

int vmv_gemm_rs_launch(const VmvGemmParams& p, int tile, hipStream_t st) {
    if (!vmv_gemm_rs_supported(p)) return VMV_GLDS_UNSUPPORTED;
    RsPlan pl;
    const int force_rt = tile == VMV_TILE_RS512 ? 4 : tile == VMV_TILE_RS256 ? 2 : 0;
    if (!rs_plan(p, force_rt, pl, rs_ncu_whole_xcds())) return VMV_GLDS_UNSUPPORTED;
    const int mode = (p.epilogue == VMV_EPI_GEGLU ? RS_GEGLU : 0) | (p.colsum ? RS_LN : 0) | (p.residual ? RS_RES : 0) | (p.gn_table ? RS_GN : 0);
    if (p.ktot == 320) return pl.rt == 4 ? launch_rs_mode<4, 10>(p, pl, mode, st) : launch_rs_mode<2, 10>(p, pl, mode, st);
    if (p.ktot == 512) return launch_rs_mode<2, 16>(p, pl, mode, st);
    return launch_rs_mode<2, 20>(p, pl, mode, st);
}
```

videomv_amd/csrc/gemm_trs.hip:

```cpp
#include "gemm_rs_common.h"
#include <cstdlib>
#include <type_traits>

using namespace vmvg;

bool vmv_gemm_tfr_preferred(const VmvGemmParams& p);

namespace {

using TrRing = RsRing<10>;
constexpr int TR_RT = 3, TR_KS = TrRing::KS, TR_K = TrRing::K;
constexpr int TR_ROWS = 16 * TR_RT;
constexpr int TR_RB = TrRing::RB, TR_CHUNK = TrRing::CHUNK_BYTES, TR_STAGES = TrRing::STAGES;
constexpr int TR_MAXCOLS = 1280;
constexpr int TR_MAXSAMP = 8;
constexpr int TR_TAB = TR_MAXSAMP * 2 * TR_K * 4;
constexpr int TR_OFF_BIAS = TR_STAGES * TR_CHUNK, TR_OFF_TAB = TR_OFF_BIAS + TR_MAXCOLS * 4;
constexpr int TR_LDS = TR_OFF_TAB + TR_TAB;
static_assert(TrRing::CROWS == 64 && (TR_TAB % 1024) == 0 && TR_LDS <= 160 * 1024, "chunk geometry");

constexpr int DPP_ROW_SHL = 0x100, DPP_ROW_SHR = 0x110, DPP_ROW_ROR = 0x120;
template <int CTRL>
VMV_DEV float tr_dpp(float old, float v) {
#if defined(__HIP_DEVICE_COMPILE__)
    return __builtin_bit_cast(float, __builtin_amdgcn_update_dpp(__builtin_bit_cast(int, old), __builtin_bit_cast(int, v), CTRL, 0xf, 0xf, false));
#else
    return old + v;
#endif
}
template <int S>
VMV_DEV void tr_shift_down(const f32x4_t (&y)[TR_RT], f32x4_t (&o)[TR_RT]) {
#pragma unroll
    for (int i = 0; i < TR_RT; ++i)
#pragma unroll
        for (int r = 0; r < 4; ++r) {
            const float carry = i > 0 ? tr_dpp<DPP_ROW_ROR + S>(0.f, y[i - 1][r]) : 0.f;
            o[i][r] = tr_dpp<DPP_ROW_SHR + S>(carry, y[i][r]);
        }
}
template <int S>
VMV_DEV void tr_shift_up_add(const f32x4_t (&y)[TR_RT], f32x4_t (&o)[TR_RT]) {
#pragma unroll
    for (int i = 0; i < TR_RT; ++i)
#pragma unroll
        for (int r = 0; r < 4; ++r) {
            const float carry = i + 1 < TR_RT ? tr_dpp<DPP_ROW_ROR + 16 - S>(0.f, y[i + 1][r]) : 0.f;
            o[i][r] += tr_dpp<DPP_ROW_SHL + S>(carry, y[i][r]);
        }
}

template <bool GN, bool RES, int S>
__global__ __launch_bounds__(512, 1) void gemm_trs_kernel(const VmvGemmParams p, const int ntiles, const int ngroups, const int npix) {
    VMV_KERNEL_ENTER();
    constexpr int RT = TR_RT, KS = TR_KS, RB = TR_RB, P = TrRing::PIECES, PPW = S, F = TR_ROWS / S;
    extern __shared__ __attribute__((aligned(16))) unsigned char smem[];
    const int tid = threadIdx.x;
    const int lane = tid & 63;
    const int wave = __builtin_amdgcn_readfirstlane(tid >> 6);
    const int frow = lane & 15, fgrp = lane >> 4;
    const int PX = p.P;

    const int nblk = gridDim.x;
    const int logical = xcd_logical(blockIdx.x, nblk);
    const long nitems = (long)ntiles * ngroups;
    const int i0 = (int)(((long)logical * nitems) / nblk), i1 = (int)(((long)(logical + 1) * nitems) / nblk);
    const int nit = i1 - i0;

    const VmvGemmSeg& sg = p.seg[0];
    const int lanecol = (fgrp & 1) * 16 + (fgrp >> 1) * 8;
    int mrow[RT];
    uint32_t tabo[RT];
    const __amdgpu_buffer_rsrc_t a_rsrc = __builtin_amdgcn_make_buffer_rsrc(const_cast<void*>(sg.src), 0, (uint32_t)p.M * (uint32_t)sg.ld * 2u, SRD_FLAGS);
    u32x4_t a[RT][KS];
    auto load_tile = [&](const int tile) __attribute__((always_inline)) {
        const int gp0 = (tile * TrRing::NW + wave) * PPW;
        rs_load_rows(a, a_rsrc, sg.ld, gp0, frow, fgrp, F, PX, npix, [&](const int tr, int& f, int& px) { f = tr / PPW; px = tr - f * PPW; },
                     [&](const int i, const bool ok, const int b, const long m, const int) {
                         mrow[i] = ok ? (int)m : -1;
                         tabo[i] = (uint32_t)(TR_OFF_TAB + ((ok ? b : 0) * 2 * TR_K + 8 * fgrp) * 4);
                     });
    };
    int cur_tile = i0 / ngroups;
    load_tile(cur_tile);

    float* bias_lds = reinterpret_cast<float*>(smem + TR_OFF_BIAS);
    {
        const __amdgpu_buffer_rsrc_t b_rsrc = __builtin_amdgcn_make_buffer_rsrc(const_cast<float*>(p.bias), 0, p.bias ? (uint32_t)p.N * 4u : 0u, SRD_FLAGS);
        for (int q = wave; q * 256 < TR_MAXCOLS; q += TrRing::NW)
            blds16(b_rsrc, reinterpret_cast<unsigned char*>(bias_lds) + q * 1024, (uint32_t)(q * 256 + 4 * lane) * 4u, 0);
    }
    if constexpr (GN) {
        const uint32_t tbytes = (uint32_t)(p.M / (F * PX)) * (uint32_t)(2 * TR_K * 4);
        const __amdgpu_buffer_rsrc_t t_rsrc = __builtin_amdgcn_make_buffer_rsrc(const_cast<float*>(p.gn_table), 0, tbytes, SRD_FLAGS);
        for (int q = wave; q * 1024 < (int)tbytes; q += TrRing::NW)
            blds16(t_rsrc, smem + TR_OFF_TAB + q * 1024, (uint32_t)(q * 1024 + 16 * lane), 0);
    }
    const __amdgpu_buffer_rsrc_t w_rsrc = __builtin_amdgcn_make_buffer_rsrc(const_cast<void*>(p.W), 0, (uint32_t)p.N * (uint32_t)p.ktot * 2u, SRD_FLAGS);
    auto issue_chunk = [&](int c, int slot) {
        unsigned char* base = TrRing::wave_base(smem + slot * TR_CHUNK, wave);
        const int it = c / 3, cc = c - 3 * it;
        const int n0 = 64 * ((i0 + it) % ngroups);
        rs_issue_rows<TrRing>(w_rsrc, base, wave, lane, 0, [&](const int r) {
            const int hh = 2 * cc + (r >> 5);
            const int pr = hh >= 3 ? 1 : 0, tp = hh - 3 * pr;
            const int n = n0 + 32 * pr + (r & 31);
            return n * p.ktot + tp * TR_K;
        });
    };
    const int NC = 3 * nit;
    for (int c = 0; c < TR_STAGES; ++c) issue_chunk(c, c);

    const bool silu = p.gn_silu != 0;
    auto fold_rows = [&]() __attribute__((always_inline)) {
        if constexpr (GN) {
            f32x4_t tv[2][4];
            int chain = 0;
            auto rd = [&](int idx, f32x4_t (&t)[4]) {
                const float* tb = reinterpret_cast<const float*>(smem + tabo[idx / KS]) + (idx % KS) * 32 + chain;
                t[0] = *reinterpret_cast<const f32x4_t*>(tb); t[1] = *reinterpret_cast<const f32x4_t*>(tb + 4);
                t[2] = *reinterpret_cast<const f32x4_t*>(tb + TR_K); t[3] = *reinterpret_cast<const f32x4_t*>(tb + TR_K + 4);
            };
            rd(0, tv[0]);
#pragma unroll
            for (int idx = 0; idx < RT * KS; ++idx) {
                if (idx + 1 < RT * KS) rd(idx + 1, tv[(idx + 1) & 1]);
                __builtin_amdgcn_sched_barrier(0);
                const f32x4_t sc0 = tv[idx & 1][0], sc1 = tv[idx & 1][1], sh0 = tv[idx & 1][2], sh1 = tv[idx & 1][3];
                u32x4_t v = a[idx / KS][idx % KS];
                float x0 = fmaf(elem_lo(v.x), sc0.x, sh0.x), x1 = fmaf(elem_hi(v.x), sc0.y, sh0.y);
                float x2 = fmaf(elem_lo(v.y), sc0.z, sh0.z), x3 = fmaf(elem_hi(v.y), sc0.w, sh0.w);
                float x4 = fmaf(elem_lo(v.z), sc1.x, sh1.x), x5 = fmaf(elem_hi(v.z), sc1.y, sh1.y);
                float x6 = fmaf(elem_lo(v.w), sc1.z, sh1.z), x7 = fmaf(elem_hi(v.w), sc1.w, sh1.w);
                if (silu) {
                    x0 = silu_f(x0); x1 = silu_f(x1); x2 = silu_f(x2); x3 = silu_f(x3);
                    x4 = silu_f(x4); x5 = silu_f(x5); x6 = silu_f(x6); x7 = silu_f(x7);
                }
                v.x = pack_elem2(x0, x1); v.y = pack_elem2(x2, x3); v.z = pack_elem2(x4, x5); v.w = pack_elem2(x6, x7);
                a[idx / KS][idx % KS] = v;
                asm volatile("" : "+v"(chain) : "v"(v.x), "v"(v.y), "v"(v.z), "v"(v.w));
                __builtin_amdgcn_sched_barrier(0);
            }
        }
    };
    if constexpr (GN) {
        wait_vmcnt_rt(TR_STAGES * P);
        __syncthreads();
    }
    fold_rows();

    const __amdgpu_buffer_rsrc_t out_rsrc = __builtin_amdgcn_make_buffer_rsrc(p.out, 0, SRD_RECORDS, SRD_FLAGS);
    const __amdgpu_buffer_rsrc_t res_rsrc = __builtin_amdgcn_make_buffer_rsrc(const_cast<void*>(p.residual), 0, SRD_RECORDS, SRD_FLAGS);
    const float rs = p.res_scale != 0.f ? p.res_scale : 1.f;

    wait_vmcnt_rt(2 * P);
    __builtin_amdgcn_s_barrier();
    asm volatile("" ::: "memory");

    const int fsw = (frow >> 1) & 7;
    int foff[2];
#pragma unroll
    for (int r = 0; r < 2; ++r) foff[r] = frow * RB + (fgrp ^ (fsw & 3)) * 16 + ((r ^ (fsw >> 2)) - r) * 64;
    auto mma_pair = [&](const unsigned char* sbase, const int q, f32x4_t (&c0)[RT], f32x4_t (&c1)[RT]) {
        rs_mma_pair<false, 1, TrRing>(a, sbase, q, foff, c0, c1);
    };

    int c = 0, slot = 0;
    auto chunk_end = [&](const int extra) { rs_ring_step<TrRing>(c, slot, NC, extra, issue_chunk); };
    constexpr int NVM = RES ? 2 * RT : RT;

    for (int it = 0; it < nit; ++it) {
        const int tile = (i0 + it) / ngroups, g = (i0 + it) - tile * ngroups;
        if (tile != cur_tile) {
            cur_tile = tile;
            load_tile(tile);
            fold_rows();
        }
        f32x4_t o0[RT], o1[RT];
#pragma unroll
        for (int h = 0; h < 6; ++h) {
            const int pr = h / 3, tap = h - 3 * pr;
            const int ocol = 64 * g + 32 * pr;
            const unsigned char* sbase = smem + slot * TR_CHUNK;
            const bool col_ok = ocol < p.N;
            u32x4_t rv[RT];
            if constexpr (RES) {
                if (tap == 2) {
#pragma unroll
                    for (int i = 0; i < RT; ++i)
                        rv[i] = __builtin_amdgcn_raw_buffer_load_b128(res_rsrc, col_ok && mrow[i] >= 0 ? (uint32_t)(mrow[i] * p.ldr + lanecol) * 2u : OOB, (uint32_t)ocol * 2u, 0);
                }
            }
            f32x4_t c0[RT], c1[RT];
            mma_pair(sbase, h & 1, c0, c1);
            if (tap == 0) {
                tr_shift_down<S>(c0, o0); tr_shift_down<S>(c1, o1);
            } else if (tap == 1) {
#pragma unroll
                for (int i = 0; i < RT; ++i) { o0[i] += c0[i]; o1[i] += c1[i]; }
            } else {
                tr_shift_up_add<S>(c0, o0); tr_shift_up_add<S>(c1, o1);
                const f32x4_t b0 = *reinterpret_cast<const f32x4_t*>(bias_lds + ocol + 4 * fgrp);
                const f32x4_t b1 = *reinterpret_cast<const f32x4_t*>(bias_lds + ocol + 16 + 4 * fgrp);
#pragma unroll
                for (int i = 0; i < RT; ++i) {
                    f32x4_t v0 = o0[i] + b0, v1 = o1[i] + b1;
                    act_apply(v0, p.act); act_apply(v1, p.act);
                    if constexpr (RES) {
                        const u32x4_t r = rs_swap16(rv[i]);
                        v0.x += rs * elem_lo(r.x); v0.y += rs * elem_hi(r.x); v0.z += rs * elem_lo(r.y); v0.w += rs * elem_hi(r.y);
                        v1.x += rs * elem_lo(r.z); v1.y += rs * elem_hi(r.z); v1.z += rs * elem_lo(r.w); v1.w += rs * elem_hi(r.w);
                    }
                    const u32x4_t ov = u32x4_t{pack_elem2(v0.x, v0.y), pack_elem2(v0.z, v0.w), pack_elem2(v1.x, v1.y), pack_elem2(v1.z, v1.w)};
                    rs_store16(rs_swap16(ov), out_rsrc, col_ok && mrow[i] >= 0 ? (uint32_t)(mrow[i] * p.ldo + lanecol) * 2u : OOB, (uint32_t)ocol * 2u);
                    __builtin_amdgcn_sched_barrier(0);
                }
            }
            if (h == 1) chunk_end(it > 0 ? NVM : 0);
            else if (h == 3) chunk_end(NVM);
            else if (h == 5) chunk_end(2 * NVM);
        }
    }
}

long trs_items(const VmvGemmParams& p) {
    return (long)rs_pixel_tiles(p, TR_ROWS).ntiles * ((p.N + 63) / 64);
}

}

bool vmv_gemm_trs_supported(const VmvGemmParams& p) {
    if (p.nseg != 3 || (p.F != 12 && p.F != 16 && p.F != 24) || p.P <= 0) return false;
    const VmvGemmSeg& s0 = p.seg[0];
    for (int i = 0; i < 3; ++i) {
        const VmvGemmSeg& sg = p.seg[i];
        if (sg.mode != VMV_SEG_TEMPORAL || sg.d0 != i - 1 || sg.src != s0.src || sg.ld != s0.ld || sg.k != s0.k) return false;
    }
    if (s0.k != TR_K || p.ktot != 3 * TR_K || (p.N % 32) || p.N > TR_MAXCOLS) return false;
    if ((long)p.M % ((long)p.F * p.P)) return false;
    if (p.epilogue != VMV_EPI_NONE || p.rowvec || p.rowstat || p.colsum || p.ln_eps > 0.f || p.wgroup_rows || p.ksplit > 1 || p.out_fp32 || p.phased) return false;
    if ((p.ldo & 7) || !vmv_aligned16(p.out) || (p.residual && ((p.ldr & 7) || !vmv_aligned16(p.residual)))) return false;
    if (p.gn_table && (p.gn_rows_per_stat != p.F * p.P || !vmv_aligned16(p.gn_table) || p.M / ((long)p.F * p.P) > TR_MAXSAMP)) return false;
    if (p.gn_silu && !p.gn_table) return false;
    if (!vmv_gemm_spans32(p, p.M, 64, p.M, p.M)) return false;
    return true;
}

bool vmv_gemm_trs_preferred(const VmvGemmParams& p) {
    if (!p.gn_table || !vmv_gemm_trs_supported(p) || vmv_gemm_tfr_preferred(p)) return false;
    const char* e = getenv("VMV_TRS_MIN_ITEMS");
    return trs_items(p) >= (e ? atol(e) : 128);
}

int vmv_gemm_trs_launch(const VmvGemmParams& p, int max_blocks, hipStream_t st) {
    if (!vmv_gemm_trs_supported(p)) return VMV_GLDS_UNSUPPORTED;
    const int npix = rs_pixel_tiles(p, TR_ROWS).npix, ntiles = rs_pixel_tiles(p, TR_ROWS).ntiles;
    const int ngroups = (p.N + 63) / 64;
    const long nitems = trs_items(p);
    int nblk = (int)(nitems < rs_ncu_whole_xcds() ? nitems : rs_ncu_whole_xcds());
    if (max_blocks > 0 && nblk > max_blocks) nblk = max_blocks;
    const bool gn = p.gn_table != nullptr, res = p.residual != nullptr;
#define TR_LAUNCH1(GNV, RESV, SV)                                                                                                               \
    do {                                                                                                                                 \
        static std::atomic<unsigned long long> attr{0};                                                                                  \
        if (const int rc = vmv_lds_attr_once(attr, reinterpret_cast<const void*>(&gemm_trs_kernel<GNV, RESV, SV>), TR_LDS)) return rc;         \
        VMV_LAUNCH((gemm_trs_kernel<GNV, RESV, SV>), dim3(nblk), dim3(TrRing::NT), TR_LDS, st, p, ntiles, ngroups, npix);                           \
    } while (0)
#define TR_LAUNCH(SV)                                                                                                                    \
    do {                                                                                                                                 \
        if (gn) { if (res) TR_LAUNCH1(true, true, SV); else TR_LAUNCH1(true, false, SV); }                                               \
        else { if (res) TR_LAUNCH1(false, true, SV); else TR_LAUNCH1(false, false, SV); }                                                \
    } while (0)
    if (p.F == 24) TR_LAUNCH(2); else if (p.F == 16) TR_LAUNCH(3); else TR_LAUNCH(4);
#undef TR_LAUNCH
#undef TR_LAUNCH1
    return vmv_launch_status();
}
```

videomv_amd/csrc/norm.hip:

```cpp
#include "common.h"
#include <type_traits>

namespace {

constexpr float GN_LO = 1099511627776.0f;

VMV_DEV void gn_add2(unsigned long long* rec, int which, float v) {
    const float fl = floorf(v);
    atomicAdd(rec + which, (unsigned long long)(long long)fl);
    atomicAdd(rec + 2 + which, (unsigned long long)(long long)((v - fl) * GN_LO));
}

struct GnSlots {
    int TPR, RPP;
    __host__ __device__ explicit GnSlots(int slots) : TPR(slots < 256 ? slots : 256), RPP(256 / TPR) {}
};
struct GnLane : GnSlots {
    int rl, cl;
    bool active;
    __device__ explicit GnLane(int slots) : GnSlots(slots), rl((int)threadIdx.x / TPR), cl((int)threadIdx.x - rl * TPR), active(rl < RPP) {}
};
struct GnSrc { const uint16_t* base; long ld; };
VMV_DEV GnSrc gn_src(const VmvGroupNormParams& p, int c) {
    const bool first = c < p.C0;
    return {first ? reinterpret_cast<const uint16_t*>(p.x) + c : reinterpret_cast<const uint16_t*>(p.x1) + (c - p.C0),
            first ? p.ld : p.ld1};
}
VMV_DEV float gn_pilot(const VmvGroupNormParams& p, long row, int c) {
    const GnSrc s = gn_src(p, c);
    return elem_to_f32(s.base[row * s.ld]);
}
template <int U, typename F>
VMV_DEV void gn_walk(const uint16_t* base, long ld, long& r, long row_end, int RPP, F f) {
    for (; r + (long)(U - 1) * RPP < row_end; r += (long)U * RPP) {
        u32x4_t v[U];
#pragma unroll
        for (int k = 0; k < U; ++k) v[k] = *reinterpret_cast<const u32x4_t*>(base + (r + (long)k * RPP) * ld);
#pragma unroll
        for (int k = 0; k < U; ++k) f(v[k], r + (long)k * RPP);
    }
}
VMV_DEV void gn_scale_shift(float* scale, float* shift, const float* s_mean, const float* s_rstd, const VmvGroupNormParams& p,
                            int c0, int n, int cpg) {
    for (int c = threadIdx.x; c < n; c += 256) {
        const int g = c / cpg;
        const float sc = s_rstd[g] * p.gamma[c0 + c];
        scale[c] = sc;
        shift[c] = p.beta[c0 + c] - s_mean[g] * sc;
    }
}
struct GnAffine {
    float a[8], b[8];
    VMV_DEV GnAffine(const float* scale, const float* shift) {
#pragma unroll
        for (int e = 0; e < 8; ++e) { a[e] = scale[e]; b[e] = shift[e]; }
    }
    template <bool SILU>
    VMV_DEV u32x4_t apply(const u32x4_t& v) const {
        float f[8];
        unpack8(v, f);
#pragma unroll
        for (int e = 0; e < 8; ++e) {
            f[e] = f[e] * a[e] + b[e];
            if constexpr (SILU) f[e] = silu_f(f[e]);
        }
        return pack8(f);
    }
};

__global__ __launch_bounds__(256) void gn_stats_kernel(const VmvGroupNormParams p, const int nchunk) {
    VMV_KERNEL_ENTER();
    extern __shared__ __attribute__((aligned(16))) float sh[];
    const int C = p.C0 + p.C1;
    const int CS = C >> 3;
    const GnLane L(CS);
    const int RPP = L.RPP, rl = L.rl;
    const int tid = threadIdx.x;
    const int stat = blockIdx.y, chunk = blockIdx.x;
    const long row0 = (long)stat * p.rows_per_stat + (long)chunk * p.chunk_rows;
    long row_end = row0 + p.chunk_rows;
    const long stat_end = (long)(stat + 1) * p.rows_per_stat;
    if (row_end > stat_end) row_end = stat_end;
    float* lsum = sh;
    float* lsq = sh + RPP * C;
    float* pil = sh + 2 * RPP * C;
    const int cpg_ = C >> 5;
    if (tid < 32) pil[tid] = gn_pilot(p, (long)stat * p.rows_per_stat, tid * cpg_);
    __syncthreads();
    for (int cs = L.cl; cs < CS; cs += L.TPR) {
        float s[8], q[8], pl[8];
#pragma unroll
        for (int e = 0; e < 8; ++e) { s[e] = 0.f; q[e] = 0.f; pl[e] = pil[(cs * 8 + e) / cpg_]; }
        if (L.active) {
            const GnSrc src = gn_src(p, cs * 8);
            auto add = [&](const u32x4_t& v, long) {
                float f[8];
                unpack8(v, f);
#pragma unroll
                for (int e = 0; e < 8; ++e) { const float d = f[e] - pl[e]; s[e] += d; q[e] += d * d; }
            };
            long r = row0 + rl;
            gn_walk<8>(src.base, src.ld, r, row_end, RPP, add);
            gn_walk<4>(src.base, src.ld, r, row_end, RPP, add);
            gn_walk<1>(src.base, src.ld, r, row_end, RPP, add);
#pragma unroll
            for (int e = 0; e < 8; ++e) { lsum[rl * C + cs * 8 + e] = s[e]; lsq[rl * C + cs * 8 + e] = q[e]; }
        }
    }
    __syncthreads();
    if (tid < 32) {
        const int cpg = C >> 5;
        float s = 0.f, q = 0.f;
        for (int r = 0; r < RPP; ++r)
            for (int c = tid * cpg; c < (tid + 1) * cpg; ++c) { s += lsum[r * C + c]; q += lsq[r * C + c]; }
        if (p.totals) {
            unsigned long long* rec = reinterpret_cast<unsigned long long*>(p.totals) +
                                      (((long)stat * 32 + tid) * VMV_GN_NREP + (chunk & (VMV_GN_NREP - 1))) * VMV_GN_REC;
            gn_add2(rec, 0, s);
            gn_add2(rec, 1, q);
            if (chunk == 0) rec[4] = (unsigned long long)__float_as_uint(pil[tid]);
        } else {
            float* out = p.partial + (((long)stat * nchunk + chunk) * 32 + tid) * 2;
            out[0] = s; out[1] = q;
        }
    }
}

__global__ __launch_bounds__(256) void gn_apply_kernel(const VmvGroupNormParams p, const int nchunk,
                                                       const int apply_rows, const int nstat, float* const table) {
    VMV_KERNEL_ENTER();
    extern __shared__ __attribute__((aligned(16))) float sh[];
    const int C = p.C0 + p.C1;
    const int CS = C >> 3;
    const int cpg = C >> 5;
    const int tid = threadIdx.x;
    const int stat = blockIdx.y;
    float* scale = sh;
    float* shift = sh + C;
    float* s_mean = sh + 2 * C;
    float* s_rstd = s_mean + 32;
    {
        const int g = tid >> 3, sub = tid & 7;
        float s = 0.f, q = 0.f;
        const int R = p.fold_ranks > 1 ? p.fold_ranks : 1;
        if (p.totals) {
            static_assert(VMV_GN_NREP == 8, "one replica per sub-lane");
            const double nr = (double)p.rows_per_stat * (double)cpg;
            double S = 0.0, Q = 0.0, P0 = 0.0;
            for (int r = 0; r < R; ++r) {
                const long long* rec = reinterpret_cast<const long long*>(p.totals) +
                                       ((((long)r * nstat + stat) * 32 + g) * VMV_GN_NREP + sub) * VMV_GN_REC;
                long long l0 = rec[0], l1 = rec[1], l2 = rec[2], l3 = rec[3];
                const long long pb = __shfl(rec[4], tid & 56, 64);
#pragma unroll
                for (int o = 1; o < 8; o <<= 1) {
                    l0 += __shfl_xor(l0, o, 64); l1 += __shfl_xor(l1, o, 64);
                    l2 += __shfl_xor(l2, o, 64); l3 += __shfl_xor(l3, o, 64);
                }
                const double sr = (double)l0 + (double)l2 * (1.0 / (double)GN_LO);
                const double qr = (double)l1 + (double)l3 * (1.0 / (double)GN_LO);
                const double P = (double)__uint_as_float((uint32_t)pb);
                if (r == 0) P0 = P;
                const double d = P - P0;
                S += sr + nr * d;
                Q += qr + 2.0 * d * sr + nr * d * d;
            }
            if (sub == 0) {
                const double n = nr * (double)R;
                const double m = S / n;
                double var = Q / n - m * m;
                var = var < 0.0 ? 0.0 : var;
                s_mean[g] = (float)(P0 + m);
                s_rstd[g] = (float)(1.0 / sqrt(var + (double)p.eps));
            }
        } else {
            const float* pp = p.partial + ((long)stat * nchunk * 32 + g) * 2;
            for (int c = sub; c < nchunk; c += 8) { s += pp[(long)c * 64]; q += pp[(long)c * 64 + 1]; }
#pragma unroll
            for (int o = 1; o < 8; o <<= 1) { s += __shfl_xor(s, o, 64); q += __shfl_xor(q, o, 64); }
            if (sub == 0) {
                const float n = (float)p.rows_per_stat * (float)cpg;
                const float m = s / n;
                float var = q / n - m * m;
                var = var < 0.f ? 0.f : var;
                s_mean[g] = gn_pilot(p, (long)stat * p.rows_per_stat, g * cpg) + m;
                s_rstd[g] = rsqrtf(var + p.eps);
            }
        }
    }
    __syncthreads();
    if (p.totals_clear && blockIdx.x == 0 && blockIdx.y == 0)
        for (int i = tid; i < p.clear_count; i += 256) p.totals_clear[i] = 0;
    gn_scale_shift(scale, shift, s_mean, s_rstd, p, 0, C, cpg);
    __syncthreads();
    if (table) {
        for (int c = tid; c < C; c += 256) {
            table[((long)stat * 2 + 0) * C + c] = scale[c];
            table[((long)stat * 2 + 1) * C + c] = shift[c];
        }
        return;
    }
    const long row0 = (long)stat * p.rows_per_stat + (long)blockIdx.x * apply_rows;
    long row_end = row0 + apply_rows;
    const long stat_end = (long)(stat + 1) * p.rows_per_stat;
    if (row_end > stat_end) row_end = stat_end;
    const GnLane L(CS);
    uint16_t* y = reinterpret_cast<uint16_t*>(p.y);
    if (L.active) {
        for (int cs = L.cl; cs < CS; cs += L.TPR) {
            const int c = cs * 8;
            const GnAffine af(scale + c, shift + c);
            const GnSrc src = gn_src(p, c);
            uint16_t* dst = y + c;
            auto stream = [&](auto silu_tag) {
                auto put = [&](const u32x4_t& v, long row) {
                    *reinterpret_cast<u32x4_t*>(dst + row * p.ldy) = af.apply<decltype(silu_tag)::value>(v);
                };
                long r = row0 + L.rl;
                gn_walk<4>(src.base, src.ld, r, row_end, L.RPP, put);
                gn_walk<1>(src.base, src.ld, r, row_end, L.RPP, put);
            };
            if (p.silu) stream(std::true_type{}); else stream(std::false_type{});
        }
    }
}

constexpr int GNF_UNR = 4;
__global__ __launch_bounds__(256) void gn_fused_kernel(const VmvGroupNormParams p, const int CW) {
    VMV_KERNEL_ENTER();
    extern __shared__ __attribute__((aligned(16))) float sh[];
    const int C = p.C0 + p.C1;
    const int cpg = C >> 5;
    const int G = CW / cpg;
    const int SW = CW >> 3;
    const GnLane L(SW);
    const int TPR = L.TPR, RPP = L.RPP, rl = L.rl, cl = L.cl;
    const bool active = L.active;
    const int tid = threadIdx.x;
    const int stat = blockIdx.y, c0 = blockIdx.x * CW;
    const int rows = p.rows_per_stat;
    const long row0 = (long)stat * rows;
    u32x4_t* stage = reinterpret_cast<u32x4_t*>(sh);
    float* red = sh + (size_t)rows * SW * 4;
    float* scale = red + RPP * CW;
    float* shift = scale + CW;
    float* s_mean = shift + CW;
    float* s_rstd = s_mean + 32;
    for (int cs = cl; cs < SW; cs += TPR) {
        float s[8];
#pragma unroll
        for (int e = 0; e < 8; ++e) s[e] = 0.f;
        if (active) {
            const GnSrc src = gn_src(p, c0 + cs * 8);
            const uint16_t* base = src.base;
            const long ld = src.ld;
            int r = rl;
            for (; r + (GNF_UNR - 1) * RPP < rows; r += GNF_UNR * RPP) {
                u32x4_t v[GNF_UNR];
#pragma unroll
                for (int k = 0; k < GNF_UNR; ++k) v[k] = *reinterpret_cast<const u32x4_t*>(base + (row0 + r + k * RPP) * ld);
#pragma unroll
                for (int k = 0; k < GNF_UNR; ++k) {
                    stage[(size_t)(r + k * RPP) * SW + cs] = v[k];
                    float f[8];
                    unpack8(v[k], f);
#pragma unroll
                    for (int e = 0; e < 8; ++e) s[e] += f[e];
                }
            }
            for (; r < rows; r += RPP) {
                const u32x4_t v = *reinterpret_cast<const u32x4_t*>(base + (row0 + r) * ld);
                stage[(size_t)r * SW + cs] = v;
                float f[8];
                unpack8(v, f);
#pragma unroll
                for (int e = 0; e < 8; ++e) s[e] += f[e];
            }
#pragma unroll
            for (int e = 0; e < 8; ++e) red[rl * CW + cs * 8 + e] = s[e];
        }
    }
    __syncthreads();
    const float n = (float)rows * (float)cpg;
    auto group_totals = [&](float* dst, auto finish) {
        float cs = 0.f;
        if (tid < CW)
            for (int r = 0; r < RPP; ++r) cs += red[r * CW + tid];
        __syncthreads();
        if (tid < CW) red[tid] = cs;
        __syncthreads();
        const int wv = tid >> 6, ln = tid & 63;
        for (int g = wv; g < G; g += 4) {
            float s = 0.f;
            for (int c = ln; c < cpg; c += 64) s += red[g * cpg + c];
            s = wave_sum(s);
            if (ln == 0) dst[g] = finish(s);
        }
        __syncthreads();
    };
    group_totals(s_mean, [&](float s) { return s / n; });
    for (int cs = cl; cs < SW; cs += TPR) {
        if (active) {
            float mu[8], q[8];
#pragma unroll
            for (int e = 0; e < 8; ++e) { mu[e] = s_mean[(cs * 8 + e) / cpg]; q[e] = 0.f; }
            for (int r = rl; r < rows; r += RPP) {
                float f[8];
                unpack8(stage[(size_t)r * SW + cs], f);
#pragma unroll
                for (int e = 0; e < 8; ++e) { const float d = f[e] - mu[e]; q[e] += d * d; }
            }
#pragma unroll
            for (int e = 0; e < 8; ++e) red[rl * CW + cs * 8 + e] = q[e];
        }
    }
    __syncthreads();
    group_totals(s_rstd, [&](float q) { return rsqrtf(q / n + p.eps); });
    gn_scale_shift(scale, shift, s_mean, s_rstd, p, c0, CW, cpg);
    __syncthreads();
    uint16_t* y = reinterpret_cast<uint16_t*>(p.y);
    if (active) {
        for (int cs = cl; cs < SW; cs += TPR) {
            const GnAffine af(scale + cs * 8, shift + cs * 8);
            uint16_t* dst = y + c0 + cs * 8;
            auto run = [&](auto silu_tag) {
                for (int r = rl; r < rows; r += RPP)
                    *reinterpret_cast<u32x4_t*>(dst + (row0 + r) * p.ldy) = af.apply<decltype(silu_tag)::value>(stage[(size_t)r * SW + cs]);
            };
            if (p.silu) run(std::true_type{}); else run(std::false_type{});
        }
    }
}

constexpr int LN_MAX_IT = 5;
template <int LPR>
__global__ __launch_bounds__(256) void layernorm_kernel(const VmvLayerNormParams p) {
    VMV_KERNEL_ENTER();
    constexpr int RPW = 64 / LPR;
    const int lane = threadIdx.x & 63;
    const int sub = lane % LPR;
    const long row = ((long)blockIdx.x * 4 + (threadIdx.x >> 6)) * RPW + lane / LPR;
    const bool live = row < p.rows;
    const int CS = p.C >> 3;
    const uint16_t* x = reinterpret_cast<const uint16_t*>(p.x) + (live ? row : 0) * p.ldx;
    float f[LN_MAX_IT][8];
    float s = 0.f;
#pragma unroll
    for (int it = 0; it < LN_MAX_IT; ++it) {
        const int cs = sub + it * LPR;
        if (cs < CS) {
            unpack8(*reinterpret_cast<const u32x4_t*>(x + cs * 8), f[it]);
#pragma unroll
            for (int e = 0; e < 8; ++e) s += f[it][e];
        }
    }
#pragma unroll
    for (int o = LPR / 2; o > 0; o >>= 1) s += __shfl_xor(s, o, 64);
    const float mean = s / (float)p.C;
    float q = 0.f;
#pragma unroll
    for (int it = 0; it < LN_MAX_IT; ++it) {
        const int cs = sub + it * LPR;
        if (cs < CS) {
#pragma unroll
            for (int e = 0; e < 8; ++e) { const float d = f[it][e] - mean; q += d * d; }
        }
    }
#pragma unroll
    for (int o = LPR / 2; o > 0; o >>= 1) q += __shfl_xor(q, o, 64);
    const float rstd = rsqrtf(q / (float)p.C + p.eps);
    if (!live) return;
    if (p.stats_out) {
        if (sub == 0) *reinterpret_cast<float2*>(p.stats_out + row * 2) = make_float2(mean, rstd);
        return;
    }
    uint16_t* y = reinterpret_cast<uint16_t*>(p.y) + row * p.ldy;
#pragma unroll
    for (int it = 0; it < LN_MAX_IT; ++it) {
        const int cs = sub + it * LPR;
        if (cs < CS) {
            const int c = cs * 8;
            const f32x4_t g0 = *reinterpret_cast<const f32x4_t*>(p.gamma + c);
            const f32x4_t g1 = *reinterpret_cast<const f32x4_t*>(p.gamma + c + 4);
            const f32x4_t b0 = *reinterpret_cast<const f32x4_t*>(p.beta + c);
            const f32x4_t b1 = *reinterpret_cast<const f32x4_t*>(p.beta + c + 4);
            float o[8];
            o[0] = (f[it][0] - mean) * rstd * g0.x + b0.x; o[1] = (f[it][1] - mean) * rstd * g0.y + b0.y;
            o[2] = (f[it][2] - mean) * rstd * g0.z + b0.z; o[3] = (f[it][3] - mean) * rstd * g0.w + b0.w;
            o[4] = (f[it][4] - mean) * rstd * g1.x + b1.x; o[5] = (f[it][5] - mean) * rstd * g1.y + b1.y;
            o[6] = (f[it][6] - mean) * rstd * g1.z + b1.z; o[7] = (f[it][7] - mean) * rstd * g1.w + b1.w;
            *reinterpret_cast<u32x4_t*>(y + c) = pack8(o);
        }
    }
}

__global__ __launch_bounds__(256) void softmax_rows_kernel(const VmvSoftmaxParams p) {
    VMV_KERNEL_ENTER();
    const int lane = threadIdx.x & 63;
    const long row = (long)blockIdx.x * 4 + (threadIdx.x >> 6);
    if (row >= p.rows) return;
    const float* s = p.s + row * p.lds;
    const float sc = p.scale * 1.44269504088896341f;
    const int n4 = p.n >> 2;
    float mx = -3.0e38f;
    for (int i = lane; i < n4; i += 64) {
        const f32x4_t v = *reinterpret_cast<const f32x4_t*>(s + 4 * i);
        mx = fmaxf(fmaxf(fmaxf(mx, v.x), fmaxf(v.y, v.z)), v.w);
    }
#pragma unroll
    for (int o = 32; o > 0; o >>= 1) mx = fmaxf(mx, __shfl_xor(mx, o, 64));
    const float m2 = mx * sc;
    float sum = 0.f;
    for (int i = lane; i < n4; i += 64) {
        const f32x4_t v = *reinterpret_cast<const f32x4_t*>(s + 4 * i);
        sum += __builtin_amdgcn_exp2f(v.x * sc - m2) + __builtin_amdgcn_exp2f(v.y * sc - m2) +
               __builtin_amdgcn_exp2f(v.z * sc - m2) + __builtin_amdgcn_exp2f(v.w * sc - m2);
    }
    const float inv = 1.0f / wave_sum(sum);
    uint16_t* out = reinterpret_cast<uint16_t*>(p.p) + row * p.ldp;
    for (int i = lane; i < n4; i += 64) {
        const f32x4_t v = *reinterpret_cast<const f32x4_t*>(s + 4 * i);
        u32x2_t w;
        w.x = pack_elem2(__builtin_amdgcn_exp2f(v.x * sc - m2) * inv, __builtin_amdgcn_exp2f(v.y * sc - m2) * inv);
        w.y = pack_elem2(__builtin_amdgcn_exp2f(v.z * sc - m2) * inv, __builtin_amdgcn_exp2f(v.w * sc - m2) * inv);
        *reinterpret_cast<u32x2_t*>(out + 4 * i) = w;
    }
}

int gn_check(const VmvGroupNormParams& p, bool ws) {
    if (!p.x || (ws && !p.partial && !p.totals)) return VMV_ENULL;
    const int C = p.C0 + p.C1;
    if (C <= 0 || (C & 31) || (p.C0 & 7) || (p.C1 & 7)) return VMV_EINVAL;
    if (p.C1 > 0 && !p.x1) return VMV_ENULL;
    if (p.rows <= 0 || p.rows_per_stat <= 0 || (p.rows % p.rows_per_stat) || (ws && p.chunk_rows <= 0)) return VMV_EINVAL;
    if (!vmv_aligned16(p.x) || (p.ld & 7) || (p.C1 > 0 && (!vmv_aligned16(p.x1) || (p.ld1 & 7)))) return VMV_EALIGN;
    if (C > 4096) return VMV_ERANGE;
    return VMV_OK;
}
int gn_check_out(const VmvGroupNormParams& p, bool table) {
    if (!p.y || !p.gamma || !p.beta) return VMV_ENULL;
    if (table && p.silu) return VMV_EINVAL;
    if (!vmv_aligned16(p.y) || (!table && (p.ldy & 7)) || !vmv_aligned16(p.gamma) || !vmv_aligned16(p.beta)) return VMV_EALIGN;
    return VMV_OK;
}
struct GnGrid { int nstat, nchunk; };
GnGrid gn_grid(const VmvGroupNormParams& p) { return {p.rows / p.rows_per_stat, (p.rows_per_stat + p.chunk_rows - 1) / p.chunk_rows}; }

int gn_apply_launch(const VmvGroupNormParams* pp, void* stream, bool table) {
    if (!pp) return VMV_ENULL;
    const VmvGroupNormParams& p = *pp;
    if (const int rc = gn_check(p, true)) return rc;
    if (const int rc = gn_check_out(p, table)) return rc;
    if (p.fold_ranks > 1 && !p.totals) return VMV_EINVAL;
    const int C = p.C0 + p.C1;
    const GnGrid g = gn_grid(p);
    int apply_rows = (65536 / (C * 2));
    if (apply_rows < 1 || table) apply_rows = 1;
    const int nblk = table ? 1 : (p.rows_per_stat + apply_rows - 1) / apply_rows;
    hipLaunchKernelGGL(gn_apply_kernel, dim3(nblk, g.nstat), dim3(256), (size_t)(2 * C + 64) * sizeof(float),
                       reinterpret_cast<hipStream_t>(stream), p, g.nchunk, apply_rows, g.nstat, table ? reinterpret_cast<float*>(p.y) : nullptr);
    return vmv_launch_status();
}

}

extern "C" int vmv_groupnorm_stats(const VmvGroupNormParams* pp, void* stream) {
    if (!pp) return VMV_ENULL;
    const VmvGroupNormParams& p = *pp;
    if (const int rc = gn_check(p, true)) return rc;
    const int C = p.C0 + p.C1;
    const GnGrid g = gn_grid(p);
    const size_t shbytes = ((size_t)2 * GnSlots(C >> 3).RPP * C + 32) * sizeof(float);
    if (p.totals && (((uintptr_t)p.totals) & 7)) return VMV_EALIGN;
    hipLaunchKernelGGL(gn_stats_kernel, dim3(g.nchunk, g.nstat), dim3(256), shbytes, reinterpret_cast<hipStream_t>(stream), p, g.nchunk);
    return vmv_launch_status();
}

extern "C" int vmv_groupnorm_apply(const VmvGroupNormParams* pp, void* stream) { return gn_apply_launch(pp, stream, false); }
extern "C" int vmv_groupnorm_table(const VmvGroupNormParams* pp, void* stream) { return gn_apply_launch(pp, stream, true); }

extern "C" int vmv_groupnorm_fused(const VmvGroupNormParams* pp, int32_t cols, void* stream) {
    if (!pp) return VMV_ENULL;
    const VmvGroupNormParams& p = *pp;
    if (const int rc = gn_check(p, false)) return rc;
    if (const int rc = gn_check_out(p, false)) return rc;
    const int C = p.C0 + p.C1, cpg = C >> 5;
    if (cols <= 0 || (cols & 7) || (cols % cpg) || (C % cols)) return VMV_EINVAL;
    if (cols > 256) return VMV_ERANGE;
    if (p.fold_ranks > 1) return VMV_EINVAL;
    if ((long)p.rows_per_stat * cols * 2 > VMV_GN_FUSED_BYTES) return VMV_ERANGE;
    const size_t shbytes = (size_t)p.rows_per_stat * cols * 2 + (size_t)(GnSlots(cols >> 3).RPP * cols + 2 * cols + 64) * sizeof(float);
    if (shbytes > 160 * 1024) return VMV_ERANGE;
    static std::atomic<unsigned long long> attr{0};
    if (const int rc_attr = vmv_lds_attr_once(attr, reinterpret_cast<const void*>(&gn_fused_kernel), 160 * 1024)) return rc_attr;
    hipLaunchKernelGGL(gn_fused_kernel, dim3(C / cols, p.rows / p.rows_per_stat), dim3(256), shbytes,
                       reinterpret_cast<hipStream_t>(stream), p, cols);
    return vmv_launch_status();
}

extern "C" int vmv_layernorm(const VmvLayerNormParams* pp, void* stream) {
    if (!pp) return VMV_ENULL;
    const VmvLayerNormParams& p = *pp;
    if (!p.x) return VMV_ENULL;
    if (!p.stats_out && (!p.y || !p.gamma || !p.beta)) return VMV_ENULL;
    if (p.rows <= 0 || p.C <= 0 || (p.C & 7)) return VMV_EINVAL;
    if (p.C > LN_MAX_IT * 64 * 8) return VMV_ERANGE;
    if (!vmv_aligned16(p.x) || (p.ldx & 7)) return VMV_EALIGN;
    if (p.stats_out) { if (((uintptr_t)p.stats_out) & 7) return VMV_EALIGN; }
    else if (!vmv_aligned16(p.y) || (p.ldy & 7) || !vmv_aligned16(p.gamma) || !vmv_aligned16(p.beta)) return VMV_EALIGN;
    const int CS = p.C >> 3;
    hipStream_t st = reinterpret_cast<hipStream_t>(stream);
    auto go = [&](auto lpr_tag) {
        constexpr int LPR = decltype(lpr_tag)::value;
        const int rows_per_block = 4 * (64 / LPR);
        const int blocks = (p.rows + rows_per_block - 1) / rows_per_block;
        hipLaunchKernelGGL(layernorm_kernel<LPR>, dim3(blocks), dim3(256), 0, st, p);
    };
    if (CS <= 8 * LN_MAX_IT) go(std::integral_constant<int, 8>{});
    else if (CS <= 16 * LN_MAX_IT) go(std::integral_constant<int, 16>{});
    else if (CS <= 32 * LN_MAX_IT) go(std::integral_constant<int, 32>{});
    else go(std::integral_constant<int, 64>{});
    return vmv_launch_status();
}

extern "C" int vmv_softmax_rows(const VmvSoftmaxParams* pp, void* stream) {
    if (!pp) return VMV_ENULL;
    const VmvSoftmaxParams& p = *pp;
    if (!p.s || !p.p) return VMV_ENULL;
    if (p.rows <= 0 || p.n <= 0 || (p.n & 3) || p.scale <= 0.f) return VMV_EINVAL;
    if (!vmv_aligned16(p.s) || (p.lds & 3) || (((uintptr_t)p.p) & 7) || (p.ldp & 3)) return VMV_EALIGN;
    hipLaunchKernelGGL(softmax_rows_kernel, dim3((p.rows + 3) / 4), dim3(256), 0, reinterpret_cast<hipStream_t>(stream), p);
    return vmv_launch_status();
}
```

videomv_amd/csrc/plan.hip:

```cpp
#include "common.h"
#include <vector>
#include <cstring>
#include <new>

struct VmvPlan {
    struct Op { int op; std::vector<unsigned char> args; };
    std::vector<Op> ops;
};

namespace {
int run_op(const VmvPlan::Op& o, void* stream) {
    switch (o.op) {
        case VMV_OP_GEMM: return vmv_gemm(reinterpret_cast<const VmvGemmParams*>(o.args.data()), stream);
        case VMV_OP_GN_STATS: return vmv_groupnorm_stats(reinterpret_cast<const VmvGroupNormParams*>(o.args.data()), stream);
        case VMV_OP_GN_APPLY: return vmv_groupnorm_apply(reinterpret_cast<const VmvGroupNormParams*>(o.args.data()), stream);
        case VMV_OP_LAYERNORM: return vmv_layernorm(reinterpret_cast<const VmvLayerNormParams*>(o.args.data()), stream);
        case VMV_OP_ATTENTION: return vmv_attention(reinterpret_cast<const VmvAttnParams*>(o.args.data()), stream);
        case VMV_OP_SOFTMAX: return vmv_softmax_rows(reinterpret_cast<const VmvSoftmaxParams*>(o.args.data()), stream);
        case VMV_OP_COPY: return vmv_permute_copy(reinterpret_cast<const VmvCopyParams*>(o.args.data()), stream);
        case VMV_OP_FF: return vmv_ff_fused(reinterpret_cast<const VmvFfParams*>(o.args.data()), stream);
        case VMV_OP_GN_TABLE: return vmv_groupnorm_table(reinterpret_cast<const VmvGroupNormParams*>(o.args.data()), stream);
        case VMV_OP_COMM: return vmv_comm_run(reinterpret_cast<const VmvCommParams*>(o.args.data()), stream);
        case VMV_OP_GN_FUSED: {
            const VmvGroupNormParams* g = reinterpret_cast<const VmvGroupNormParams*>(o.args.data());
            return vmv_groupnorm_fused(g, g->chunk_rows, stream);
        }
        default: return VMV_EINVAL;
    }
}
size_t op_size(int op) {
    switch (op) {
        case VMV_OP_GEMM: return sizeof(VmvGemmParams);
        case VMV_OP_GN_STATS: case VMV_OP_GN_APPLY: case VMV_OP_GN_FUSED: case VMV_OP_GN_TABLE: return sizeof(VmvGroupNormParams);
        case VMV_OP_LAYERNORM: return sizeof(VmvLayerNormParams);
        case VMV_OP_ATTENTION: return sizeof(VmvAttnParams);
        case VMV_OP_SOFTMAX: return sizeof(VmvSoftmaxParams);
        case VMV_OP_COPY: return sizeof(VmvCopyParams);
        case VMV_OP_FF: return sizeof(VmvFfParams);
        case VMV_OP_COMM: return sizeof(VmvCommParams);
        default: return 0;
    }
}
}

extern "C" int vmv_abi_version(void) { return VMV_ABI_VERSION; }
extern "C" int vmv_elem_type(void) { return VMV_ELEM_TYPE; }
extern "C" int vmv_sizeof(int which) {
    switch (which) {
        case 100: return (int)sizeof(VmvDdimParams);
        case 101: return (int)sizeof(VmvGemmSeg);
        case 102: return (int)sizeof(VmvSeqMap);
        case 103: return (int)sizeof(VmvGsParams);
        case 104: return (int)sizeof(VmvGsBatchParams);
        case 105: return (int)sizeof(VmvGsBackwardParams);
        case 106: return (int)sizeof(VmvGsAdamParams);
        case 107: return (int)sizeof(VmvGsSsimLossParams);
        case 108: return (int)sizeof(VmvGsDepthParams);
        case 109: return (int)sizeof(VmvGsTsdfParams);
        case 110: return (int)sizeof(VmvGsMeshComponentsParams);
        case 111: return (int)sizeof(VmvGsMeshBakeParams);
        default: return (int)op_size(which);
    }
}

extern "C" const char* vmv_error_string(int code) {
    switch (code) {
        case VMV_OK: return "ok";
        case VMV_EINVAL: return "VMV_EINVAL: bad dimension or flag combination";
        case VMV_EALIGN: return "VMV_EALIGN: pointer or leading dimension not suitably aligned";
        case VMV_ENULL: return "VMV_ENULL: required pointer is NULL";
        case VMV_ERANGE: return "VMV_ERANGE: size outside what the kernel supports";
        case VMV_ECOMM: return "VMV_ECOMM: an RCCL call failed (vmv_comm_*)";
        default: return code > 0 ? hipGetErrorString((hipError_t)code) : "unknown vmv error";
    }
}

extern "C" VmvPlan* vmv_plan_create(void) { return new (std::nothrow) VmvPlan(); }
extern "C" void vmv_plan_destroy(VmvPlan* plan) { delete plan; }
extern "C" int vmv_plan_add(VmvPlan* plan, int op, const void* params, size_t nbytes) {
    if (!plan || !params) return VMV_ENULL;
    const size_t want = op_size(op);
    if (want == 0 || nbytes != want) return VMV_EINVAL;
    VmvPlan::Op o;
    o.op = op;
    o.args.resize(nbytes);
    std::memcpy(o.args.data(), params, nbytes);
    plan->ops.push_back(std::move(o));
    return (int)plan->ops.size() - 1;
}
extern "C" int vmv_plan_size(const VmvPlan* plan) { return plan ? (int)plan->ops.size() : VMV_ENULL; }
extern "C" int vmv_plan_run_range(const VmvPlan* plan, int first, int last, void* stream) {
    if (!plan) return VMV_ENULL;
    if (first < 0 || last > (int)plan->ops.size() || first > last) return VMV_EINVAL;
    for (int i = first; i < last; ++i) {
        const int rc = run_op(plan->ops[i], stream);
        if (rc != VMV_OK) return rc;
    }
    return VMV_OK;
}
extern "C" int vmv_plan_run(const VmvPlan* plan, void* stream) {
    if (!plan) return VMV_ENULL;
    return vmv_plan_run_range(plan, 0, (int)plan->ops.size(), stream);
}

struct VmvGraph {
    hipGraph_t graph = nullptr;
    hipGraphExec_t exec = nullptr;
    int nodes = 0;
};
extern "C" VmvGraph* vmv_plan_capture(const VmvPlan* plan, void* stream) {
    if (!plan || plan->ops.empty()) return nullptr;
    hipStream_t s = reinterpret_cast<hipStream_t>(stream);
    VmvGraph* g = new (std::nothrow) VmvGraph();
    if (!g) return nullptr;
    if (hipStreamBeginCapture(s, hipStreamCaptureModeThreadLocal) != hipSuccess) { delete g; return nullptr; }
    int rc = VMV_OK;
    for (size_t i = 0; i < plan->ops.size() && rc == VMV_OK; ++i) rc = run_op(plan->ops[i], stream);
    const hipError_t e = hipStreamEndCapture(s, &g->graph);
    if (rc != VMV_OK || e != hipSuccess || !g->graph) { vmv_graph_destroy(g); return nullptr; }
    size_t n = 0;
    if (hipGraphGetNodes(g->graph, nullptr, &n) == hipSuccess) g->nodes = (int)n;
    if (hipGraphInstantiate(&g->exec, g->graph, nullptr, nullptr, 0) != hipSuccess) { vmv_graph_destroy(g); return nullptr; }
    return g;
}
extern "C" int vmv_graph_launch(const VmvGraph* g, void* stream) {
    if (!g || !g->exec) return VMV_ENULL;
    const hipError_t e = hipGraphLaunch(g->exec, reinterpret_cast<hipStream_t>(stream));
    return e == hipSuccess ? VMV_OK : (int)e;
}
extern "C" int vmv_graph_nodes(const VmvGraph* g) { return g ? g->nodes : VMV_ENULL; }
extern "C" void vmv_graph_destroy(VmvGraph* g) {
    if (!g) return;
    if (g->exec) (void)hipGraphExecDestroy(g->exec);
    if (g->graph) (void)hipGraphDestroy(g->graph);
    delete g;
}
```

Baseline: 21.75 denoise-steps/s.

## Fuse GroupNorm table computation into the following RS/TRS GEMM prologue

Adds a fused path in which the RS and TRS GEMM kernels compute the GroupNorm scale/shift table themselves, folding the partial statistics in their prologue while the A-tile loads are in flight. The plan replay now detects GN_TABLE followed by a GEMM that consumes that table and runs them as a single launch, both in direct runs and in graph capture. This removes one kernel launch and the global round trip of the table per fused pair. In exchange the GEMM prologue does more work and every block recomputes the fold, and blocks still write the table and clear the totals for later consumers.

```diff
diff --git a/include/vmv.h b/include/vmv.h
--- a/include/vmv.h
+++ b/include/vmv.h
@@ -13,6 +13,7 @@
 #define VMV_ENULL        -3
 #define VMV_ERANGE       -4
 #define VMV_ECOMM        -5
+#define VMV_ENOTSERVED   -6
 
 #define VMV_ABI_VERSION   12
 int vmv_abi_version(void);
@@ -171,6 +172,9 @@
 int vmv_groupnorm_stats(const VmvGroupNormParams* p, void* stream);
 int vmv_groupnorm_table(const VmvGroupNormParams* p, void* stream);
 int vmv_groupnorm_apply(const VmvGroupNormParams* p, void* stream);
+int vmv_gemm_gn_table(const VmvGemmParams* p, const VmvGroupNormParams* gn, void* stream);
+int vmv_gemm_gn_table_ok(const VmvGemmParams* p, const VmvGroupNormParams* gn);
+int vmv_gemm_gn_table_trs_blocks(const VmvGemmParams* p, const VmvGroupNormParams* gn, int max_blocks, void* stream);
 #define VMV_GN_FUSED_BYTES 131072
 int vmv_groupnorm_fused(const VmvGroupNormParams* p, int32_t cols, void* stream);
 
@@ -456,6 +460,8 @@
 int      vmv_plan_size(const VmvPlan* plan);
 int      vmv_plan_run(const VmvPlan* plan, void* stream);
 int      vmv_plan_run_range(const VmvPlan* plan, int first, int last, void* stream);
+int      vmv_plan_fused_pairs(const VmvPlan* plan);
+int      vmv_plan_fused_pairs_range(const VmvPlan* plan, int first, int last);
 typedef struct VmvGraph VmvGraph;
 VmvGraph* vmv_plan_capture(const VmvPlan* plan, void* stream);
 int       vmv_graph_launch(const VmvGraph* graph, void* stream);
diff --git a/videomv_amd/_lib.py b/videomv_amd/_lib.py
--- a/videomv_amd/_lib.py
+++ b/videomv_amd/_lib.py
@@ -39,6 +39,7 @@
 TILE_X256x320, TILE_X256x256, TILE_X256x128 = 20, 21, 22
 TILE_RS, TILE_RS512, TILE_RS256, TILE_HALO, TILE_TFR, TILE_TQA, TILE_W256x256, TILE_X512x128, TILE_Y256x128 = 23, 24, 25, 26, 27, 28, 29, 30, 31
 TRS_TILE = 32
+ENOTSERVED = -6
 OP_GEMM, OP_GN_STATS, OP_GN_APPLY, OP_LAYERNORM, OP_ATTENTION, OP_SOFTMAX, OP_COPY, OP_GN_FUSED, OP_FF, OP_GN_TABLE, OP_COMM = 1, 2, 3, 4, 5, 6, 7, 8, 9, 10, 11
 COMM_ALL_TO_ALL, COMM_ALL_GATHER, COMM_ID_BYTES = 0, 1, 128
 ABI_VERSION = 12
@@ -214,6 +215,9 @@
     "vmv_groupnorm_apply": (C.c_int, [C.POINTER(GroupNormParams), _P]),
     "vmv_groupnorm_table": (C.c_int, [C.POINTER(GroupNormParams), _P]),
     "vmv_groupnorm_fused": (C.c_int, [C.POINTER(GroupNormParams), C.c_int32, _P]),
+    "vmv_gemm_gn_table": (C.c_int, [C.POINTER(GemmParams), C.POINTER(GroupNormParams), _P]),
+    "vmv_gemm_gn_table_ok": (C.c_int, [C.POINTER(GemmParams), C.POINTER(GroupNormParams)]),
+    "vmv_gemm_gn_table_trs_blocks": (C.c_int, [C.POINTER(GemmParams), C.POINTER(GroupNormParams), C.c_int, _P]),
     "vmv_layernorm": (C.c_int, [C.POINTER(LayerNormParams), _P]),
     "vmv_attention": (C.c_int, [C.POINTER(AttnParams), _P]),
     "vmv_attention_served_kernel": (C.c_int, [C.POINTER(AttnParams)]),
@@ -256,6 +260,8 @@
     "vmv_plan_size": (C.c_int, [_P]),
     "vmv_plan_run": (C.c_int, [_P, _P]),
     "vmv_plan_run_range": (C.c_int, [_P, C.c_int, C.c_int, _P]),
+    "vmv_plan_fused_pairs": (C.c_int, [_P]),
+    "vmv_plan_fused_pairs_range": (C.c_int, [_P, C.c_int, C.c_int]),
     "vmv_plan_capture": (_P, [_P, _P]),
     "vmv_graph_launch": (C.c_int, [_P, _P]),
     "vmv_graph_nodes": (C.c_int, [_P]),
diff --git a/videomv_amd/csrc/gemm.hip b/videomv_amd/csrc/gemm.hip
--- a/videomv_amd/csrc/gemm.hip
+++ b/videomv_amd/csrc/gemm.hip
@@ -7,7 +7,7 @@
 bool vmv_gemm_pglds_supported(const VmvGemmParams& p);
 int vmv_gemm_xglds_launch(const VmvGemmParams& p, int total_steps, int tile, hipStream_t st);
 int vmv_gemm_xglds_epi_ok(const VmvGemmParams& p, int tile);
-int vmv_gemm_rs_launch(const VmvGemmParams& p, int tile, hipStream_t st);
+int vmv_gemm_rs_launch(const VmvGemmParams& p, int tile, hipStream_t st, const VmvGroupNormParams* gn = nullptr);
 bool vmv_gemm_rs_supported(const VmvGemmParams& p);
 int vmv_conv_halo_launch(const VmvGemmParams& p, hipStream_t st);
 bool vmv_conv_halo_supported(const VmvGemmParams& p);
@@ -18,7 +18,8 @@
 int vmv_gemm_tqa_launch(const VmvGemmParams& p, hipStream_t st);
 bool vmv_gemm_tqa_supported(const VmvGemmParams& p);
 bool vmv_gemm_tqa_preferred(const VmvGemmParams& p);
-int vmv_gemm_trs_launch(const VmvGemmParams& p, int max_blocks, hipStream_t st);
+int vmv_gemm_trs_launch(const VmvGemmParams& p, int max_blocks, hipStream_t st, const VmvGroupNormParams* gn = nullptr);
+int vmv_gn_table_check(const VmvGroupNormParams& p);
 bool vmv_gemm_trs_supported(const VmvGemmParams& p);
 bool vmv_gemm_trs_preferred(const VmvGemmParams& p);
 namespace {
@@ -438,6 +439,27 @@
     return rc == VMV_GLDS_UNSUPPORTED ? VMV_EINVAL : rc;
 }
 
+static int gemm_gn_table(const VmvGemmParams* pp, const VmvGroupNormParams* gn, int max_blocks, void* stream, bool dry) {
+    if (!pp || !gn) return VMV_ENULL;
+    if (const int rc = vmv_gn_table_check(*gn)) return rc;
+    if (gn->fold_ranks > 1 || !pp->gn_table || reinterpret_cast<const void*>(pp->gn_table) != gn->y) return VMV_ENOTSERVED;
+    const int tile = vmv_gemm_served_tile(pp);
+    if (tile < 0) return tile;
+    hipStream_t st = reinterpret_cast<hipStream_t>(stream);
+    int rc = VMV_GLDS_UNSUPPORTED;
+    vmv_dry_run = dry ? 1 : 0;
+    if (tile == VMV_TILE_TRS) rc = vmv_gemm_trs_launch(*pp, max_blocks, st, gn);
+    else if (max_blocks == 0 && (tile == VMV_TILE_RS || tile == VMV_TILE_RS512 || tile == VMV_TILE_RS256)) rc = vmv_gemm_rs_launch(*pp, tile, st, gn);
+    vmv_dry_run = 0;
+    return rc == VMV_GLDS_UNSUPPORTED ? VMV_ENOTSERVED : rc;
+}
+extern "C" int vmv_gemm_gn_table(const VmvGemmParams* pp, const VmvGroupNormParams* gn, void* stream) { return gemm_gn_table(pp, gn, 0, stream, false); }
+extern "C" int vmv_gemm_gn_table_ok(const VmvGemmParams* pp, const VmvGroupNormParams* gn) { return gemm_gn_table(pp, gn, 0, nullptr, true) == VMV_OK ? 1 : 0; }
+extern "C" int vmv_gemm_gn_table_trs_blocks(const VmvGemmParams* pp, const VmvGroupNormParams* gn, int max_blocks, void* stream) {
+    if (!pp || pp->tile != VMV_TILE_TRS || max_blocks < 1) return VMV_EINVAL;
+    return gemm_gn_table(pp, gn, max_blocks, stream, false);
+}
+
 extern "C" int vmv_gemm_tile_map(int bid, int tiles_m, int tiles_n, int gm, int* tile_m, int* tile_n) {
     if (!tile_m || !tile_n) return VMV_ENULL;
     if (tiles_m <= 0 || tiles_n <= 0 || gm < 1 || bid < 0 || (long)bid >= (long)tiles_m * tiles_n) return VMV_EINVAL;
diff --git a/videomv_amd/csrc/gemm_rs.hip b/videomv_amd/csrc/gemm_rs.hip
--- a/videomv_amd/csrc/gemm_rs.hip
+++ b/videomv_amd/csrc/gemm_rs.hip
@@ -1,4 +1,5 @@
 #include "gemm_rs_common.h"
+#include "gn_table.h"
 #include <type_traits>
 
 using namespace vmvg;
@@ -15,13 +16,15 @@
     static_assert(LDS_BYTES <= 160 * 1024, "LDS budget");
 };
 
-constexpr int RS_GEGLU = 1, RS_LN = 2, RS_RES = 4, RS_GN = 8;
+constexpr int RS_GEGLU = 1, RS_LN = 2, RS_RES = 4, RS_GN = 8, RS_GNC = 16;
 
 template <int RT, int KS, int MODE>
-__global__ __launch_bounds__(512, 1) void gemm_rs_kernel(const VmvGemmParams p, const int tiles_m, const int nsplit, const int cols_per_split) {
+__global__ __launch_bounds__(512, 1) void gemm_rs_kernel(const VmvGemmParams p, const int tiles_m, const int nsplit, const int cols_per_split,
+                                                         const VmvGroupNormParams gn, const int gn_nchunk) {
     VMV_KERNEL_ENTER();
     using Cfg = RsCfg<RT, KS>;
-    constexpr bool GEGLU = (MODE & RS_GEGLU) != 0, LN = (MODE & RS_LN) != 0, RES = (MODE & RS_RES) != 0, GN = (MODE & RS_GN) != 0;
+    constexpr bool GEGLU = (MODE & RS_GEGLU) != 0, LN = (MODE & RS_LN) != 0, RES = (MODE & RS_RES) != 0, GN = (MODE & RS_GN) != 0, GNC = (MODE & RS_GNC) != 0;
+    static_assert(GN || !GNC, "computed tables belong to the folded form");
     constexpr int RB = Cfg::RB, G = Cfg::G, P = Cfg::PIECES;
     extern __shared__ __attribute__((aligned(16))) unsigned char smem[];
 
@@ -40,6 +43,10 @@
 
     const VmvGemmSeg& sg = p.seg[0];
     const __amdgpu_buffer_rsrc_t a_rsrc = __builtin_amdgcn_make_buffer_rsrc(const_cast<void*>(sg.src), 0, (uint32_t)p.M * (uint32_t)sg.ld * 2u, SRD_FLAGS);
+    const int gn_nstat = GN ? (p.M + p.gn_rows_per_stat - 1) / p.gn_rows_per_stat : 0;
+    const int gn_mine = GN ? (mt * Cfg::BM) / p.gn_rows_per_stat + (wave >> 2) : 0;
+    GnTablePrologue<Cfg::K> gnp;
+    if constexpr (GNC) gnp.load(gn, gn_nchunk, gn_nstat, gn_mine < gn_nstat ? gn_mine : gn_nstat - 1, tid & 255);
     u32x4_t a[RT][KS];
 #pragma unroll
     for (int i = 0; i < RT; ++i) {
@@ -47,6 +54,8 @@
 #pragma unroll
         for (int kk = 0; kk < KS; ++kk) a[i][kk] = __builtin_amdgcn_raw_buffer_load_b128(a_rsrc, vo + (uint32_t)(kk * 64), 0, 0);
     }
+    if constexpr (GNC)
+        gnp.template finish<RT * KS>(gn, gn_nchunk, tid & 255, gn_mine < gn_nstat, reinterpret_cast<float*>(smem + Cfg::STAGES * Cfg::CHUNK_BYTES) + Cfg::MAX_COLS + (wave >> 2) * 2 * Cfg::K);
 
     float* bias_lds = reinterpret_cast<float*>(smem + Cfg::STAGES * Cfg::CHUNK_BYTES);
     {
@@ -56,8 +65,8 @@
     }
     float* tab_lds = bias_lds + Cfg::MAX_COLS;
     int gn_first = 0;
-    if constexpr (GN) {
-        gn_first = (mt * Cfg::BM) / p.gn_rows_per_stat;
+    if constexpr (GN) gn_first = (mt * Cfg::BM) / p.gn_rows_per_stat;
+    if constexpr (GN && !GNC) {
         const uint32_t nstat = (uint32_t)((p.M + p.gn_rows_per_stat - 1) / p.gn_rows_per_stat);
         const __amdgpu_buffer_rsrc_t t_rsrc = __builtin_amdgcn_make_buffer_rsrc(const_cast<float*>(p.gn_table), 0, nstat * (uint32_t)(2 * Cfg::K * 4), SRD_FLAGS);
         for (int q = wave; q * 1024 < Cfg::TAB_BYTES; q += Cfg::NW)
@@ -75,6 +84,17 @@
     if constexpr (GN) {
         wait_vmcnt_rt(pro * P);
         __syncthreads();
+        if constexpr (GNC) {
+            for (int j = 0; j < 2; ++j) {
+                const long r0 = (long)(gn_first + j) * p.gn_rows_per_stat;
+                if (ns == 0 && gn_first + j < gn_nstat && r0 >= (long)mt * Cfg::BM && r0 < (long)(mt + 1) * Cfg::BM) {
+                    float* const gt = reinterpret_cast<float*>(gn.y) + (long)(gn_first + j) * 2 * Cfg::K;
+                    for (int i = tid; i < 2 * Cfg::K; i += Cfg::NT) gt[i] = tab_lds[j * 2 * Cfg::K + i];
+                }
+            }
+            if (gn.totals_clear && blockIdx.x == 0)
+                for (int i = tid; i < gn.clear_count; i += Cfg::NT) gn.totals_clear[i] = 0;
+        }
         const float* tbase[RT];
 #pragma unroll
         for (int i = 0; i < RT; ++i) {
@@ -218,24 +238,27 @@
 }
 
 template <int RT, int KS, int MODE>
-int launch_rs(const VmvGemmParams& p, const RsPlan& pl, hipStream_t st) {
+int launch_rs(const VmvGemmParams& p, const RsPlan& pl, hipStream_t st, const VmvGroupNormParams* gn) {
     using Cfg = RsCfg<RT, KS>;
     const int tiles_m = (p.M + Cfg::BM - 1) / Cfg::BM;
     static std::atomic<unsigned long long> attr{0};
     if (const int rc_attr = vmv_lds_attr_once(attr, reinterpret_cast<const void*>(&gemm_rs_kernel<RT, KS, MODE>), Cfg::LDS_BYTES)) return rc_attr;
-    VMV_LAUNCH((gemm_rs_kernel<RT, KS, MODE>), dim3(tiles_m * pl.nsplit), dim3(Cfg::NT), Cfg::LDS_BYTES, st, p, tiles_m, pl.nsplit, pl.cols);
+    const VmvGroupNormParams gnv = gn ? *gn : VmvGroupNormParams{};
+    const int gn_nchunk = gn ? (gn->rows_per_stat + gn->chunk_rows - 1) / gn->chunk_rows : 0;
+    VMV_LAUNCH((gemm_rs_kernel<RT, KS, MODE>), dim3(tiles_m * pl.nsplit), dim3(Cfg::NT), Cfg::LDS_BYTES, st, p, tiles_m, pl.nsplit, pl.cols, gnv, gn_nchunk);
     return vmv_launch_status();
 }
 
 template <int RT, int KS>
-int launch_rs_mode(const VmvGemmParams& p, const RsPlan& pl, int mode, hipStream_t st) {
+int launch_rs_mode(const VmvGemmParams& p, const RsPlan& pl, int mode, hipStream_t st, const VmvGroupNormParams* gn) {
     switch (mode) {
-        case 0: return launch_rs<RT, KS, 0>(p, pl, st);
-        case RS_GEGLU: return launch_rs<RT, KS, RS_GEGLU>(p, pl, st);
-        case RS_LN: return launch_rs<RT, KS, RS_LN>(p, pl, st);
-        case RS_LN | RS_GEGLU: return launch_rs<RT, KS, RS_LN | RS_GEGLU>(p, pl, st);
-        case RS_RES: return launch_rs<RT, KS, RS_RES>(p, pl, st);
-        case RS_GN: return launch_rs<RT, KS, RS_GN>(p, pl, st);
+        case 0: return launch_rs<RT, KS, 0>(p, pl, st, gn);
+        case RS_GEGLU: return launch_rs<RT, KS, RS_GEGLU>(p, pl, st, gn);
+        case RS_LN: return launch_rs<RT, KS, RS_LN>(p, pl, st, gn);
+        case RS_LN | RS_GEGLU: return launch_rs<RT, KS, RS_LN | RS_GEGLU>(p, pl, st, gn);
+        case RS_RES: return launch_rs<RT, KS, RS_RES>(p, pl, st, gn);
+        case RS_GN: return launch_rs<RT, KS, RS_GN>(p, pl, st, gn);
+        case RS_GN | RS_GNC: return launch_rs<RT, KS, RS_GN | RS_GNC>(p, pl, st, gn);
         default: return VMV_GLDS_UNSUPPORTED;
     }
 }
@@ -272,13 +295,14 @@
     return blocks >= 160;
 }
 
-int vmv_gemm_rs_launch(const VmvGemmParams& p, int tile, hipStream_t st) {
+int vmv_gemm_rs_launch(const VmvGemmParams& p, int tile, hipStream_t st, const VmvGroupNormParams* gn) {
     if (!vmv_gemm_rs_supported(p)) return VMV_GLDS_UNSUPPORTED;
+    if (gn && (!p.gn_table || gn->C0 + gn->C1 != p.ktot || gn->rows != p.M || gn->rows_per_stat != p.gn_rows_per_stat || gn->fold_ranks > 1)) return VMV_GLDS_UNSUPPORTED;
     RsPlan pl;
     const int force_rt = tile == VMV_TILE_RS512 ? 4 : tile == VMV_TILE_RS256 ? 2 : 0;
     if (!rs_plan(p, force_rt, pl, rs_ncu_whole_xcds())) return VMV_GLDS_UNSUPPORTED;
-    const int mode = (p.epilogue == VMV_EPI_GEGLU ? RS_GEGLU : 0) | (p.colsum ? RS_LN : 0) | (p.residual ? RS_RES : 0) | (p.gn_table ? RS_GN : 0);
-    if (p.ktot == 320) return pl.rt == 4 ? launch_rs_mode<4, 10>(p, pl, mode, st) : launch_rs_mode<2, 10>(p, pl, mode, st);
-    if (p.ktot == 512) return launch_rs_mode<2, 16>(p, pl, mode, st);
-    return launch_rs_mode<2, 20>(p, pl, mode, st);
-}
+    const int mode = (p.epilogue == VMV_EPI_GEGLU ? RS_GEGLU : 0) | (p.colsum ? RS_LN : 0) | (p.residual ? RS_RES : 0) | (p.gn_table ? RS_GN : 0) | (gn ? RS_GNC : 0);
+    if (p.ktot == 320) return pl.rt == 4 ? launch_rs_mode<4, 10>(p, pl, mode, st, gn) : launch_rs_mode<2, 10>(p, pl, mode, st, gn);
+    if (p.ktot == 512) return launch_rs_mode<2, 16>(p, pl, mode, st, gn);
+    return launch_rs_mode<2, 20>(p, pl, mode, st, gn);
+}
diff --git a/videomv_amd/csrc/gemm_trs.hip b/videomv_amd/csrc/gemm_trs.hip
--- a/videomv_amd/csrc/gemm_trs.hip
+++ b/videomv_amd/csrc/gemm_trs.hip
@@ -1,4 +1,5 @@
 #include "gemm_rs_common.h"
+#include "gn_table.h"
 #include <cstdlib>
 #include <type_traits>
 
@@ -14,6 +15,7 @@
 constexpr int TR_RB = TrRing::RB, TR_CHUNK = TrRing::CHUNK_BYTES, TR_STAGES = TrRing::STAGES;
 constexpr int TR_MAXCOLS = 1280;
 constexpr int TR_MAXSAMP = 8;
+constexpr int TR_GN_SAMP = 2;
 constexpr int TR_TAB = TR_MAXSAMP * 2 * TR_K * 4;
 constexpr int TR_OFF_BIAS = TR_STAGES * TR_CHUNK, TR_OFF_TAB = TR_OFF_BIAS + TR_MAXCOLS * 4;
 constexpr int TR_LDS = TR_OFF_TAB + TR_TAB;
@@ -50,7 +52,8 @@
 }
 
 template <bool GN, bool RES, int S>
-__global__ __launch_bounds__(512, 1) void gemm_trs_kernel(const VmvGemmParams p, const int ntiles, const int ngroups, const int npix) {
+__global__ __launch_bounds__(512, 1) void gemm_trs_kernel(const VmvGemmParams p, const int ntiles, const int ngroups, const int npix,
+                                                          const VmvGroupNormParams gn, const int gn_nchunk) {
     VMV_KERNEL_ENTER();
     constexpr int RT = TR_RT, KS = TR_KS, RB = TR_RB, P = TrRing::PIECES, PPW = S, F = TR_ROWS / S;
     extern __shared__ __attribute__((aligned(16))) unsigned char smem[];
@@ -81,7 +84,17 @@
                      });
     };
     int cur_tile = i0 / ngroups;
+    const bool gn_compute = GN && gn.x != nullptr;
+    const int nsamp = GN ? p.M / (F * PX) : 0;
+    float* const tab_lds = reinterpret_cast<float*>(smem + TR_OFF_TAB);
+    GnTablePrologue<TR_K> gnp;
+    if constexpr (GN) {
+        if (gn_compute && (wave >> 2) < nsamp) gnp.load(gn, gn_nchunk, nsamp, wave >> 2, tid & 255);
+    }
     load_tile(cur_tile);
+    if constexpr (GN) {
+        if (gn_compute && (wave >> 2) < nsamp) gnp.template finish<RT * KS>(gn, gn_nchunk, tid & 255, true, tab_lds + (wave >> 2) * 2 * TR_K);
+    }
 
     float* bias_lds = reinterpret_cast<float*>(smem + TR_OFF_BIAS);
     {
@@ -89,7 +102,7 @@
         for (int q = wave; q * 256 < TR_MAXCOLS; q += TrRing::NW)
             blds16(b_rsrc, reinterpret_cast<unsigned char*>(bias_lds) + q * 1024, (uint32_t)(q * 256 + 4 * lane) * 4u, 0);
     }
-    if constexpr (GN) {
+    if (GN && !gn_compute) {
         const uint32_t tbytes = (uint32_t)(p.M / (F * PX)) * (uint32_t)(2 * TR_K * 4);
         const __amdgpu_buffer_rsrc_t t_rsrc = __builtin_amdgcn_make_buffer_rsrc(const_cast<float*>(p.gn_table), 0, tbytes, SRD_FLAGS);
         for (int q = wave; q * 1024 < (int)tbytes; q += TrRing::NW)
@@ -145,6 +158,12 @@
     if constexpr (GN) {
         wait_vmcnt_rt(TR_STAGES * P);
         __syncthreads();
+        if (gn_compute && blockIdx.x == 0) {
+            float* const gt = reinterpret_cast<float*>(gn.y);
+            for (int i = tid; i < nsamp * 2 * TR_K; i += TrRing::NT) gt[i] = tab_lds[i];
+            if (gn.totals_clear)
+                for (int i = tid; i < gn.clear_count; i += TrRing::NT) gn.totals_clear[i] = 0;
+        }
     }
     fold_rows();
 
@@ -251,23 +270,27 @@
     return trs_items(p) >= (e ? atol(e) : 128);
 }
 
-int vmv_gemm_trs_launch(const VmvGemmParams& p, int max_blocks, hipStream_t st) {
+int vmv_gemm_trs_launch(const VmvGemmParams& p, int max_blocks, hipStream_t st, const VmvGroupNormParams* gn) {
     if (!vmv_gemm_trs_supported(p)) return VMV_GLDS_UNSUPPORTED;
+    if (gn && (!p.gn_table || gn->C0 + gn->C1 != TR_K || gn->rows != p.M || gn->rows_per_stat != p.gn_rows_per_stat || gn->fold_ranks > 1 ||
+               p.M / ((long)p.F * p.P) > TR_GN_SAMP)) return VMV_GLDS_UNSUPPORTED;
+    const VmvGroupNormParams gnv = gn ? *gn : VmvGroupNormParams{};
+    const int gn_nchunk = gn ? (gn->rows_per_stat + gn->chunk_rows - 1) / gn->chunk_rows : 0;
     const int npix = rs_pixel_tiles(p, TR_ROWS).npix, ntiles = rs_pixel_tiles(p, TR_ROWS).ntiles;
     const int ngroups = (p.N + 63) / 64;
     const long nitems = trs_items(p);
     int nblk = (int)(nitems < rs_ncu_whole_xcds() ? nitems : rs_ncu_whole_xcds());
     if (max_blocks > 0 && nblk > max_blocks) nblk = max_blocks;
-    const bool gn = p.gn_table != nullptr, res = p.residual != nullptr;
+    const bool fold = p.gn_table != nullptr, res = p.residual != nullptr;
 #define TR_LAUNCH1(GNV, RESV, SV)                                                                                                               \
     do {                                                                                                                                 \
         static std::atomic<unsigned long long> attr{0};                                                                                  \
         if (const int rc = vmv_lds_attr_once(attr, reinterpret_cast<const void*>(&gemm_trs_kernel<GNV, RESV, SV>), TR_LDS)) return rc;         \
-        VMV_LAUNCH((gemm_trs_kernel<GNV, RESV, SV>), dim3(nblk), dim3(TrRing::NT), TR_LDS, st, p, ntiles, ngroups, npix);                           \
+        VMV_LAUNCH((gemm_trs_kernel<GNV, RESV, SV>), dim3(nblk), dim3(TrRing::NT), TR_LDS, st, p, ntiles, ngroups, npix, gnv, gn_nchunk);                           \
     } while (0)
 #define TR_LAUNCH(SV)                                                                                                                    \
     do {                                                                                                                                 \
-        if (gn) { if (res) TR_LAUNCH1(true, true, SV); else TR_LAUNCH1(true, false, SV); }                                               \
+        if (fold) { if (res) TR_LAUNCH1(true, true, SV); else TR_LAUNCH1(true, false, SV); }                                               \
         else { if (res) TR_LAUNCH1(false, true, SV); else TR_LAUNCH1(false, false, SV); }                                                \
     } while (0)
     if (p.F == 24) TR_LAUNCH(2); else if (p.F == 16) TR_LAUNCH(3); else TR_LAUNCH(4);
diff --git a/videomv_amd/csrc/gn_table.h b/videomv_amd/csrc/gn_table.h
--- /dev/null
+++ b/videomv_amd/csrc/gn_table.h
@@ -0,0 +1,155 @@
+#pragma once
+#include "common.h"
+
+constexpr float GN_LO = 1099511627776.0f;
+
+struct GnSrc { const uint16_t* base; long ld; };
+VMV_DEV GnSrc gn_src(const VmvGroupNormParams& p, int c) {
+    const bool first = c < p.C0;
+    return {first ? reinterpret_cast<const uint16_t*>(p.x) + c : reinterpret_cast<const uint16_t*>(p.x1) + (c - p.C0),
+            first ? p.ld : p.ld1};
+}
+VMV_DEV float gn_pilot(const VmvGroupNormParams& p, long row, int c) {
+    const GnSrc s = gn_src(p, c);
+    return elem_to_f32(s.base[row * s.ld]);
+}
+VMV_DEV void gn_affine(const float mean, const float rstd, const float gamma, const float beta, float& scale, float& shift) {
+    const float sc = rstd * gamma;
+    scale = sc;
+    shift = beta - mean * sc;
+}
+VMV_DEV void gn_scale_shift(float* scale, float* shift, const float* s_mean, const float* s_rstd, const VmvGroupNormParams& p,
+                            int c0, int n, int cpg) {
+    for (int c = threadIdx.x; c < n; c += 256) gn_affine(s_mean[c / cpg], s_rstd[c / cpg], p.gamma[c0 + c], p.beta[c0 + c], scale[c], shift[c]);
+}
+
+struct GnRec { long long l0, l1, l2, l3; uint32_t pb; };
+VMV_DEV GnRec gn_rec_load(const VmvGroupNormParams& p, const int nstat, const int r, const int stat, const int t) {
+    static_assert(VMV_GN_NREP == 8, "one replica per sub-lane");
+    const long long* rec = reinterpret_cast<const long long*>(p.totals) + (((long)r * nstat + stat) * 32 * VMV_GN_NREP + t) * VMV_GN_REC;
+    return GnRec{rec[0], rec[1], rec[2], rec[3], *reinterpret_cast<const uint32_t*>(rec + 4)};
+}
+VMV_DEV void gn_rec_add(const GnRec& rc, const double nr, const bool first, double& S, double& Q, double& P0) {
+    long long l0 = rc.l0, l1 = rc.l1, l2 = rc.l2, l3 = rc.l3;
+    const uint32_t pb = (uint32_t)__shfl((int)rc.pb, (int)threadIdx.x & 56, 64);
+#pragma unroll
+    for (int o = 1; o < 8; o <<= 1) {
+        l0 += __shfl_xor(l0, o, 64); l1 += __shfl_xor(l1, o, 64);
+        l2 += __shfl_xor(l2, o, 64); l3 += __shfl_xor(l3, o, 64);
+    }
+    const double sr = (double)l0 + (double)l2 * (1.0 / (double)GN_LO);
+    const double qr = (double)l1 + (double)l3 * (1.0 / (double)GN_LO);
+    const double P = (double)__uint_as_float(pb);
+    if (first) P0 = P;
+    const double d = P - P0;
+    S += sr + nr * d;
+    Q += qr + 2.0 * d * sr + nr * d * d;
+}
+VMV_DEV void gn_totals_finish(const double S, const double Q, const double P0, const double n, const float eps, float& mean, float& rstd) {
+    const double m = S / n;
+    double var = Q / n - m * m;
+    var = var < 0.0 ? 0.0 : var;
+    mean = (float)(P0 + m);
+    rstd = (float)(1.0 / sqrt(var + (double)eps));
+}
+VMV_DEV void gn_partial_load(const VmvGroupNormParams& p, const int nchunk, const int stat, const int t, float& s, float& q) {
+    const float* pp = p.partial + ((long)stat * nchunk * 32 + (t >> 3)) * 2;
+    s = 0.f; q = 0.f;
+    for (int c = t & 7; c < nchunk; c += 8) { s += pp[(long)c * 64]; q += pp[(long)c * 64 + 1]; }
+}
+VMV_DEV void gn_partial_finish(float s, float q, const float n, const float pilot, const float eps, float& mean, float& rstd) {
+#pragma unroll
+    for (int o = 1; o < 8; o <<= 1) { s += __shfl_xor(s, o, 64); q += __shfl_xor(q, o, 64); }
+    const float m = s / n;
+    float var = q / n - m * m;
+    var = var < 0.f ? 0.f : var;
+    mean = pilot + m;
+    rstd = rsqrtf(var + eps);
+}
+
+VMV_DEV void gn_fold(const VmvGroupNormParams& p, const int nchunk, const int nstat, const int stat, const int t, float& mean, float& rstd) {
+    const int cpg = (p.C0 + p.C1) >> 5;
+    if (p.totals) {
+        const int R = p.fold_ranks > 1 ? p.fold_ranks : 1;
+        const double nr = (double)p.rows_per_stat * (double)cpg;
+        double S = 0.0, Q = 0.0, P0 = 0.0;
+        for (int r = 0; r < R; ++r) gn_rec_add(gn_rec_load(p, nstat, r, stat, t), nr, r == 0, S, Q, P0);
+        gn_totals_finish(S, Q, P0, nr * (double)R, p.eps, mean, rstd);
+    } else {
+        float s, q;
+        gn_partial_load(p, nchunk, stat, t, s, q);
+        gn_partial_finish(s, q, (float)p.rows_per_stat * (float)cpg, gn_pilot(p, (long)stat * p.rows_per_stat, (t >> 3) * cpg), p.eps, mean, rstd);
+    }
+}
+struct GnChan { int c, src; bool live; };
+VMV_DEV GnChan gn_chan(const int C, const int t, const int k) {
+    const int CQ = C >> 2, cpg = C >> 5;
+    const int c = (t & 63) + 64 * k;
+    const int cl = c < CQ ? c : CQ - 1;
+    return GnChan{(t >> 6) * CQ + cl, (cl / cpg) * 8, c < CQ};
+}
+VMV_DEV void gn_table_row(const VmvGroupNormParams& p, const int C, const int t, const float mean, const float rstd, float* dst) {
+    for (int k = 0; 64 * k < (C >> 2); ++k) {
+        const GnChan ch = gn_chan(C, t, k);
+        const float m = __shfl(mean, ch.src, 64), r = __shfl(rstd, ch.src, 64);
+        if (ch.live) gn_affine(m, r, p.gamma[ch.c], p.beta[ch.c], dst[ch.c], dst[C + ch.c]);
+    }
+}
+
+template <int C>
+struct GnTablePrologue {
+    static constexpr int CPT = (C / 4 + 63) / 64, NPRE = 4;
+    GnRec rec;
+    float s, q, ps[NPRE], pq[NPRE], gam[CPT], bet[CPT];
+    uint16_t pil;
+    VMV_DEV void pre_sum(const int nchunk, const int t) {
+        s = 0.f; q = 0.f;
+#pragma unroll
+        for (int k = 0; k < NPRE; ++k)
+            if ((t & 7) + 8 * k < nchunk) { s += ps[k]; q += pq[k]; }
+    }
+    VMV_DEV void load(const VmvGroupNormParams& p, const int nchunk, const int nstat, const int stat, const int t) {
+#pragma unroll
+        for (int k = 0; k < CPT; ++k) { const GnChan ch = gn_chan(C, t, k); gam[k] = p.gamma[ch.c]; bet[k] = p.beta[ch.c]; }
+        if (p.totals) rec = gn_rec_load(p, nstat, 0, stat, t);
+        else {
+            const GnSrc ps0 = gn_src(p, (t >> 3) * (C >> 5));
+            pil = ps0.base[(long)stat * p.rows_per_stat * ps0.ld];
+            const float* pp = p.partial + ((long)stat * nchunk * 32 + (t >> 3)) * 2;
+#pragma unroll
+            for (int k = 0; k < NPRE; ++k) {
+                const int c = (t & 7) + 8 * k, cl = c < nchunk ? c : nchunk - 1;
+                ps[k] = pp[(long)cl * 64]; pq[k] = pp[(long)cl * 64 + 1];
+            }
+            if (nchunk > 8 * NPRE) {
+                pre_sum(nchunk, t);
+                for (int c = (t & 7) + 8 * NPRE; c < nchunk; c += 8) { s += pp[(long)c * 64]; q += pp[(long)c * 64 + 1]; }
+            }
+        }
+    }
+    template <int AFTER>
+    VMV_DEV void finish(const VmvGroupNormParams& p, const int nchunk, const int t, const bool valid, float* dst) {
+        static_assert(AFTER >= 0 && AFTER < 64, "vmcnt is 6 bits");
+        __builtin_amdgcn_s_waitcnt((((AFTER >> 4) & 3) << 14) | 0x0f70 | (AFTER & 15));
+        const double nr = (double)p.rows_per_stat * (double)(C >> 5);
+        float mean, rstd;
+        if (p.totals) {
+            double S = 0.0, Q = 0.0, P0 = 0.0;
+            gn_rec_add(rec, nr, true, S, Q, P0);
+            gn_totals_finish(S, Q, P0, nr * 1.0, p.eps, mean, rstd);
+        } else {
+            if (nchunk <= 8 * NPRE) pre_sum(nchunk, t);
+            gn_partial_finish(s, q, (float)p.rows_per_stat * (float)(C >> 5), elem_to_f32(pil), p.eps, mean, rstd);
+        }
+#pragma unroll
+        for (int k = 0; k < CPT; ++k) {
+            const GnChan ch = gn_chan(C, t, k);
+            const float m = __shfl(mean, ch.src, 64), r = __shfl(rstd, ch.src, 64);
+            float sc, sh;
+            gn_affine(m, r, gam[k], bet[k], sc, sh);
+            if (ch.live) { dst[ch.c] = valid ? sc : 0.f; dst[C + ch.c] = valid ? sh : 0.f; }
+        }
+    }
+};
+
+int vmv_gn_table_check(const VmvGroupNormParams& p);
diff --git a/videomv_amd/csrc/norm.hip b/videomv_amd/csrc/norm.hip
--- a/videomv_amd/csrc/norm.hip
+++ b/videomv_amd/csrc/norm.hip
@@ -1,9 +1,7 @@
-#include "common.h"
+#include "gn_table.h"
 #include <type_traits>
 
 namespace {
-
-constexpr float GN_LO = 1099511627776.0f;
 
 VMV_DEV void gn_add2(unsigned long long* rec, int which, float v) {
     const float fl = floorf(v);
@@ -20,16 +18,6 @@
     bool active;
     __device__ explicit GnLane(int slots) : GnSlots(slots), rl((int)threadIdx.x / TPR), cl((int)threadIdx.x - rl * TPR), active(rl < RPP) {}
 };
-struct GnSrc { const uint16_t* base; long ld; };
-VMV_DEV GnSrc gn_src(const VmvGroupNormParams& p, int c) {
-    const bool first = c < p.C0;
-    return {first ? reinterpret_cast<const uint16_t*>(p.x) + c : reinterpret_cast<const uint16_t*>(p.x1) + (c - p.C0),
-            first ? p.ld : p.ld1};
-}
-VMV_DEV float gn_pilot(const VmvGroupNormParams& p, long row, int c) {
-    const GnSrc s = gn_src(p, c);
-    return elem_to_f32(s.base[row * s.ld]);
-}
 template <int U, typename F>
 VMV_DEV void gn_walk(const uint16_t* base, long ld, long& r, long row_end, int RPP, F f) {
     for (; r + (long)(U - 1) * RPP < row_end; r += (long)U * RPP) {
@@ -38,15 +26,6 @@
         for (int k = 0; k < U; ++k) v[k] = *reinterpret_cast<const u32x4_t*>(base + (r + (long)k * RPP) * ld);
 #pragma unroll
         for (int k = 0; k < U; ++k) f(v[k], r + (long)k * RPP);
-    }
-}
-VMV_DEV void gn_scale_shift(float* scale, float* shift, const float* s_mean, const float* s_rstd, const VmvGroupNormParams& p,
-                            int c0, int n, int cpg) {
-    for (int c = threadIdx.x; c < n; c += 256) {
-        const int g = c / cpg;
-        const float sc = s_rstd[g] * p.gamma[c0 + c];
-        scale[c] = sc;
-        shift[c] = p.beta[c0 + c] - s_mean[g] * sc;
     }
 }
 struct GnAffine {
@@ -132,66 +111,15 @@
     extern __shared__ __attribute__((aligned(16))) float sh[];
     const int C = p.C0 + p.C1;
     const int CS = C >> 3;
-    const int cpg = C >> 5;
     const int tid = threadIdx.x;
     const int stat = blockIdx.y;
     float* scale = sh;
     float* shift = sh + C;
-    float* s_mean = sh + 2 * C;
-    float* s_rstd = s_mean + 32;
-    {
-        const int g = tid >> 3, sub = tid & 7;
-        float s = 0.f, q = 0.f;
-        const int R = p.fold_ranks > 1 ? p.fold_ranks : 1;
-        if (p.totals) {
-            static_assert(VMV_GN_NREP == 8, "one replica per sub-lane");
-            const double nr = (double)p.rows_per_stat * (double)cpg;
-            double S = 0.0, Q = 0.0, P0 = 0.0;
-            for (int r = 0; r < R; ++r) {
-                const long long* rec = reinterpret_cast<const long long*>(p.totals) +
-                                       ((((long)r * nstat + stat) * 32 + g) * VMV_GN_NREP + sub) * VMV_GN_REC;
-                long long l0 = rec[0], l1 = rec[1], l2 = rec[2], l3 = rec[3];
-                const long long pb = __shfl(rec[4], tid & 56, 64);
-#pragma unroll
-                for (int o = 1; o < 8; o <<= 1) {
-                    l0 += __shfl_xor(l0, o, 64); l1 += __shfl_xor(l1, o, 64);
-                    l2 += __shfl_xor(l2, o, 64); l3 += __shfl_xor(l3, o, 64);
-                }
-                const double sr = (double)l0 + (double)l2 * (1.0 / (double)GN_LO);
-                const double qr = (double)l1 + (double)l3 * (1.0 / (double)GN_LO);
-                const double P = (double)__uint_as_float((uint32_t)pb);
-                if (r == 0) P0 = P;
-                const double d = P - P0;
-                S += sr + nr * d;
-                Q += qr + 2.0 * d * sr + nr * d * d;
-            }
-            if (sub == 0) {
-                const double n = nr * (double)R;
-                const double m = S / n;
-                double var = Q / n - m * m;
-                var = var < 0.0 ? 0.0 : var;
-                s_mean[g] = (float)(P0 + m);
-                s_rstd[g] = (float)(1.0 / sqrt(var + (double)p.eps));
-            }
-        } else {
-            const float* pp = p.partial + ((long)stat * nchunk * 32 + g) * 2;
-            for (int c = sub; c < nchunk; c += 8) { s += pp[(long)c * 64]; q += pp[(long)c * 64 + 1]; }
-#pragma unroll
-            for (int o = 1; o < 8; o <<= 1) { s += __shfl_xor(s, o, 64); q += __shfl_xor(q, o, 64); }
-            if (sub == 0) {
-                const float n = (float)p.rows_per_stat * (float)cpg;
-                const float m = s / n;
-                float var = q / n - m * m;
-                var = var < 0.f ? 0.f : var;
-                s_mean[g] = gn_pilot(p, (long)stat * p.rows_per_stat, g * cpg) + m;
-                s_rstd[g] = rsqrtf(var + p.eps);
-            }
-        }
-    }
-    __syncthreads();
+    float mean, rstd;
+    gn_fold(p, nchunk, nstat, stat, tid, mean, rstd);
     if (p.totals_clear && blockIdx.x == 0 && blockIdx.y == 0)
         for (int i = tid; i < p.clear_count; i += 256) p.totals_clear[i] = 0;
-    gn_scale_shift(scale, shift, s_mean, s_rstd, p, 0, C, cpg);
+    gn_table_row(p, C, tid, mean, rstd, sh);
     __syncthreads();
     if (table) {
         for (int c = tid; c < C; c += 256) {
@@ -462,6 +390,13 @@
     return vmv_launch_status();
 }
 
+}
+
+int vmv_gn_table_check(const VmvGroupNormParams& p) {
+    if (const int rc = gn_check(p, true)) return rc;
+    if (const int rc = gn_check_out(p, true)) return rc;
+    if (p.totals && (((uintptr_t)p.totals) & 7)) return VMV_EALIGN;
+    return VMV_OK;
 }
 
 extern "C" int vmv_groupnorm_stats(const VmvGroupNormParams* pp, void* stream) {
diff --git a/videomv_amd/csrc/plan.hip b/videomv_amd/csrc/plan.hip
--- a/videomv_amd/csrc/plan.hip
+++ b/videomv_amd/csrc/plan.hip
@@ -71,6 +71,7 @@
         case VMV_ENULL: return "VMV_ENULL: required pointer is NULL";
         case VMV_ERANGE: return "VMV_ERANGE: size outside what the kernel supports";
         case VMV_ECOMM: return "VMV_ECOMM: an RCCL call failed (vmv_comm_*)";
+        case VMV_ENOTSERVED: return "VMV_ENOTSERVED: the fused form does not exist for these arguments (nothing launched)";
         default: return code > 0 ? hipGetErrorString((hipError_t)code) : "unknown vmv error";
     }
 }
@@ -89,15 +90,42 @@
     return (int)plan->ops.size() - 1;
 }
 extern "C" int vmv_plan_size(const VmvPlan* plan) { return plan ? (int)plan->ops.size() : VMV_ENULL; }
+
+namespace {
+bool fusable_pair(const VmvPlan& plan, int i, int last) {
+    if (i + 1 >= last || plan.ops[i].op != VMV_OP_GN_TABLE || plan.ops[i + 1].op != VMV_OP_GEMM) return false;
+    const VmvGroupNormParams* gn = reinterpret_cast<const VmvGroupNormParams*>(plan.ops[i].args.data());
+    const VmvGemmParams* gp = reinterpret_cast<const VmvGemmParams*>(plan.ops[i + 1].args.data());
+    return gp->gn_table && reinterpret_cast<const void*>(gp->gn_table) == gn->y && gn->fold_ranks <= 1 && vmv_gemm_gn_table_ok(gp, gn) == 1;
+}
+int replay(const VmvPlan& plan, int first, int last, void* stream, bool count_only, int* fused) {
+    int n = 0, rc = VMV_OK;
+    for (int i = first; i < last && rc == VMV_OK; ++i) {
+        if (fusable_pair(plan, i, last)) {
+            if (!count_only)
+                rc = vmv_gemm_gn_table(reinterpret_cast<const VmvGemmParams*>(plan.ops[i + 1].args.data()),
+                                       reinterpret_cast<const VmvGroupNormParams*>(plan.ops[i].args.data()), stream);
+            ++n; ++i;
+        } else if (!count_only) rc = run_op(plan.ops[i], stream);
+    }
+    if (fused) *fused = n;
+    return rc;
+}
+}
+
 extern "C" int vmv_plan_run_range(const VmvPlan* plan, int first, int last, void* stream) {
     if (!plan) return VMV_ENULL;
     if (first < 0 || last > (int)plan->ops.size() || first > last) return VMV_EINVAL;
-    for (int i = first; i < last; ++i) {
-        const int rc = run_op(plan->ops[i], stream);
-        if (rc != VMV_OK) return rc;
-    }
-    return VMV_OK;
+    return replay(*plan, first, last, stream, false, nullptr);
 }
+extern "C" int vmv_plan_fused_pairs_range(const VmvPlan* plan, int first, int last) {
+    if (!plan) return VMV_ENULL;
+    if (first < 0 || last > (int)plan->ops.size() || first > last) return VMV_EINVAL;
+    int n = 0;
+    replay(*plan, first, last, nullptr, true, &n);
+    return n;
+}
+extern "C" int vmv_plan_fused_pairs(const VmvPlan* plan) { return plan ? vmv_plan_fused_pairs_range(plan, 0, (int)plan->ops.size()) : VMV_ENULL; }
 extern "C" int vmv_plan_run(const VmvPlan* plan, void* stream) {
     if (!plan) return VMV_ENULL;
     return vmv_plan_run_range(plan, 0, (int)plan->ops.size(), stream);
@@ -114,8 +142,7 @@
     VmvGraph* g = new (std::nothrow) VmvGraph();
     if (!g) return nullptr;
     if (hipStreamBeginCapture(s, hipStreamCaptureModeThreadLocal) != hipSuccess) { delete g; return nullptr; }
-    int rc = VMV_OK;
-    for (size_t i = 0; i < plan->ops.size() && rc == VMV_OK; ++i) rc = run_op(plan->ops[i], stream);
+    const int rc = replay(*plan, 0, (int)plan->ops.size(), stream, false, nullptr);
     const hipError_t e = hipStreamEndCapture(s, &g->graph);
     if (rc != VMV_OK || e != hipSuccess || !g->graph) { vmv_graph_destroy(g); return nullptr; }
     size_t n = 0;
```

Result: no change. 21.83 denoise-steps/s, median of 6 (+0.3%).
